# heat1q/libldpc

Hardware: AMD Instinct MI355X
Metric: decoded frames/s (n=1024 code, 50 BP iters, AWGN) (higher is better)
Workload: dtype f64

## Files before the change

include/ldpc_amd.h:

```cpp
#ifndef LDPC_AMD_H
#define LDPC_AMD_H

#include <stdbool.h>
#include <stdint.h>

#ifdef __cplusplus
extern "C" {
#endif

#if defined(__GNUC__)
#pragma GCC visibility push(default)
#endif

typedef struct
{
    bool earlyTerm;
    uint32_t iterations;
    const char *type;
} decoder_param;

typedef struct
{
    uint64_t seed;
    double xRange[3];
    const char *type;
} channel_param;

typedef struct
{
    uint32_t threads;
    uint64_t maxFrames;
    uint64_t fec;
    const char *resultFile;
} simulation_param;

typedef struct
{
    double *fer;
    double *ber;
    double *avg_iter;
    double *time;
    uint64_t *fec;
    uint64_t *frames;
} sim_results_t;

void ldpc_setup(const char *pcFile, const char *genFile, int *n, int *m, int *nct, int *mct);
void simulate(decoder_param decoderParams, channel_param channelParam, simulation_param simParam,
              sim_results_t *results, bool *stopFlag);
int calculate_rank(void);
void encode(uint8_t *infoWord, uint8_t *codeWord);
int decode(decoder_param decoderParams, double *llr, double *llrOut);
void syndrome(uint8_t *word, uint8_t *syndrome);

typedef struct ldpc_hip_ctx ldpc_hip_ctx;

enum
{
    LDPC_HIP_AWGN = 1,
    LDPC_HIP_BSC = 2,
    LDPC_HIP_BEC = 3
};

typedef struct
{
    uint32_t *iters;
    uint32_t *bit_errors;
    uint8_t *hard;
    double *llr_out;
    double *llr_in;
    uint8_t *codeword;
} ldpc_hip_out;

int ldpc_hip_device_count(void);
const char *ldpc_hip_last_error(void);

ldpc_hip_ctx *ldpc_hip_create(const char *pcFile, const char *genFile, int device);
void ldpc_hip_destroy(ldpc_hip_ctx *ctx);
void ldpc_hip_code_info(const ldpc_hip_ctx *ctx, int64_t info[10]);
const char *ldpc_hip_describe(ldpc_hip_ctx *ctx);
void ldpc_hip_set_bec_compat(ldpc_hip_ctx *ctx, int compat);
void ldpc_hip_set_fast_mode(ldpc_hip_ctx *ctx, int mode);

enum
{
    LDPC_HIP_NOISE_REFERENCE = 0,
    LDPC_HIP_NOISE_COUNTER = 1
};
int ldpc_hip_set_noise(ldpc_hip_ctx *ctx, int mode);
int ldpc_hip_philox(ldpc_hip_ctx *ctx, uint64_t seed, uint32_t tag, uint64_t frame, uint32_t first_block, uint64_t n_blocks,
                    uint32_t *out, void *hip_stream);

int ldpc_hip_set_min_sum_correction(ldpc_hip_ctx *ctx, double scale, double offset);

int ldpc_hip_decode_batch(ldpc_hip_ctx *ctx, decoder_param dec, uint64_t n, const double *llr_in,
                          const ldpc_hip_out *out, void *hip_stream);

int ldpc_hip_stream_begin(ldpc_hip_ctx *ctx, int channel, uint64_t seed, double x);
int ldpc_hip_stream_skip(ldpc_hip_ctx *ctx, uint64_t n, void *hip_stream);
int ldpc_hip_stream_decode(ldpc_hip_ctx *ctx, decoder_param dec, uint64_t n, const ldpc_hip_out *out,
                           void *hip_stream);
int ldpc_hip_batch_counters(ldpc_hip_ctx *ctx, const uint32_t *iters, const uint32_t *bit_errors, uint64_t n,
                            uint32_t max_iters, int early_term, int64_t *counters, void *hip_stream);
uint64_t ldpc_hip_stream_frame(const ldpc_hip_ctx *ctx);
uint64_t ldpc_hip_stream_raw_draws(const ldpc_hip_ctx *ctx);
int ldpc_hip_synchronize(ldpc_hip_ctx *ctx, void *hip_stream);

void ldpc_hip_set_profiling(ldpc_hip_ctx *ctx, int on);
float ldpc_hip_last_ms(ldpc_hip_ctx *ctx, int which);

int ldpc_hip_mt64(ldpc_hip_ctx *ctx, uint64_t seed, uint64_t first, uint64_t n, uint64_t *out, void *hip_stream);

int ldpc_hip_selftest_division(ldpc_hip_ctx *ctx, uint64_t n, uint64_t seed, uint64_t *mismatches);

int ldpc_hip_selftest_math(ldpc_hip_ctx *ctx, int fn, uint64_t n, const double *a, const double *b, double *out);

uint64_t ldpc_hip_selftest_chunk_table(uint64_t first_chunk, uint64_t chunks_per_request, uint64_t n_requests, uint64_t gap);
uint64_t ldpc_hip_selftest_shard_table(int world, int rank, uint32_t piece_chunks, uint64_t steps, uint64_t *launches);
uint64_t ldpc_hip_jump_tasks(const ldpc_hip_ctx *ctx);

int ldpc_hip_simulate(ldpc_hip_ctx *ctx, decoder_param dec, channel_param ch, simulation_param sim,
                      sim_results_t *results, uint64_t *totals, bool *stopFlag, int cli_output);

typedef struct ldpc_hip_comm ldpc_hip_comm;

int ldpc_hip_comm_unique_id(uint8_t id[128]);
ldpc_hip_comm *ldpc_hip_comm_create(int rank, int world, int device, const uint8_t id[128]);
ldpc_hip_comm *ldpc_hip_comm_create_shm(int rank, int world, const char *name);
ldpc_hip_comm *ldpc_hip_comm_create_echo(int rank, int world);
void ldpc_hip_comm_destroy(ldpc_hip_comm *comm);
int ldpc_hip_comm_allgather(ldpc_hip_comm *comm, const void *send, void *recv, uint64_t bytes);
void ldpc_hip_fused_plan_info(const ldpc_hip_ctx *ctx, int64_t info[8]);
int ldpc_hip_decode_stages(const ldpc_hip_ctx *ctx, decoder_param dec, int32_t stages[3]);
int ldpc_hip_selftest_layer_plan(ldpc_hip_ctx *ctx, int32_t *step_of_row);
int ldpc_hip_selftest_place(ldpc_hip_comm *comm, uint64_t nct, uint64_t pairs_before, uint64_t frame_pos, uint64_t cap,
                            uint64_t piece_pairs, uint64_t pairs_with_margin, uint64_t status, uint64_t out[5]);
void ldpc_hip_comm_stats(ldpc_hip_comm *comm, double out[4], int reset);
const char *ldpc_hip_comm_describe(ldpc_hip_comm *comm);

uint64_t ldpc_hip_shard_capacity(const ldpc_hip_ctx *ctx, uint64_t target_frames, int world);
int ldpc_hip_stream_decode_sharded(ldpc_hip_ctx *ctx, ldpc_hip_comm *comm, decoder_param dec, uint64_t target_frames,
                                   const ldpc_hip_out *out, uint64_t step[4], void *hip_stream);
int ldpc_hip_simulate_sharded(ldpc_hip_ctx *ctx, ldpc_hip_comm *comm, decoder_param dec, channel_param ch,
                              simulation_param sim, sim_results_t *results, uint64_t *totals, bool *stopFlag,
                              int cli_output);

#if defined(__GNUC__)
#pragma GCC visibility pop
#endif

#ifdef __cplusplus
}
#endif
#endif
```

libldpc_amd/binding.py:

```python
import ctypes as ct
import os

import numpy as np

PKG = os.path.dirname(os.path.abspath(__file__))
LIB_PATH = os.environ.get("LDPC_AMD_LIB") or os.path.join(PKG, "libldpc.so")

AWGN, BSC, BEC = 1, 2, 3
CHANNELS = {"AWGN": AWGN, "BSC": BSC, "BEC": BEC}


class decoder_param(ct.Structure):
    _fields_ = [("earlyTerm", ct.c_bool), ("iterations", ct.c_uint32), ("type", ct.c_char_p)]


class channel_param(ct.Structure):
    _fields_ = [("seed", ct.c_uint64), ("xRange", ct.c_double * 3), ("type", ct.c_char_p)]


class simulation_param(ct.Structure):
    _fields_ = [("threads", ct.c_uint32), ("maxFrames", ct.c_uint64), ("fec", ct.c_uint64),
                ("resultFile", ct.c_char_p)]


class sim_results_t(ct.Structure):
    _fields_ = [("fer", ct.POINTER(ct.c_double)), ("ber", ct.POINTER(ct.c_double)),
                ("avg_iter", ct.POINTER(ct.c_double)), ("time", ct.POINTER(ct.c_double)),
                ("fec", ct.POINTER(ct.c_uint64)), ("frames", ct.POINTER(ct.c_uint64))]


class ldpc_hip_out(ct.Structure):
    _fields_ = [("iters", ct.c_void_p), ("bit_errors", ct.c_void_p), ("hard", ct.c_void_p),
                ("llr_out", ct.c_void_p), ("llr_in", ct.c_void_p), ("codeword", ct.c_void_p)]


_lib = None


def load_library(path=LIB_PATH):
    global _lib
    if _lib is not None and path == LIB_PATH:
        return _lib
    if not os.path.exists(path):
        raise OSError(f"{path} is missing: build the HIP extension first (python -m libldpc_amd.build); "
                      "there is no CPU fallback")
    L = ct.CDLL(path)
    vp, u64, i32 = ct.c_void_p, ct.c_uint64, ct.c_int
    L.ldpc_hip_device_count.restype = i32
    L.ldpc_hip_last_error.restype = ct.c_char_p
    L.ldpc_hip_create.restype = vp
    L.ldpc_hip_create.argtypes = [ct.c_char_p, ct.c_char_p, i32]
    L.ldpc_hip_destroy.argtypes = [vp]
    L.ldpc_hip_code_info.argtypes = [vp, ct.POINTER(ct.c_int64)]
    L.ldpc_hip_set_bec_compat.argtypes = [vp, i32]
    L.ldpc_hip_set_fast_mode.argtypes = [vp, i32]
    L.ldpc_hip_set_noise.restype = i32
    L.ldpc_hip_set_noise.argtypes = [vp, i32]
    L.ldpc_hip_set_min_sum_correction.restype = i32
    L.ldpc_hip_set_min_sum_correction.argtypes = [vp, ct.c_double, ct.c_double]
    L.ldpc_hip_philox.restype = i32
    L.ldpc_hip_philox.argtypes = [vp, u64, ct.c_uint32, u64, ct.c_uint32, u64, vp, vp]
    L.ldpc_hip_decode_batch.restype = i32
    L.ldpc_hip_decode_batch.argtypes = [vp, decoder_param, u64, vp, ct.POINTER(ldpc_hip_out), vp]
    L.ldpc_hip_stream_begin.restype = i32
    L.ldpc_hip_stream_begin.argtypes = [vp, i32, u64, ct.c_double]
    L.ldpc_hip_stream_skip.restype = i32
    L.ldpc_hip_stream_skip.argtypes = [vp, u64, vp]
    L.ldpc_hip_stream_decode.restype = i32
    L.ldpc_hip_stream_decode.argtypes = [vp, decoder_param, u64, ct.POINTER(ldpc_hip_out), vp]
    L.ldpc_hip_stream_frame.restype = u64
    L.ldpc_hip_stream_frame.argtypes = [vp]
    L.ldpc_hip_stream_raw_draws.restype = u64
    L.ldpc_hip_stream_raw_draws.argtypes = [vp]
    L.ldpc_hip_synchronize.restype = i32
    L.ldpc_hip_synchronize.argtypes = [vp, vp]
    L.ldpc_hip_batch_counters.restype = i32
    L.ldpc_hip_batch_counters.argtypes = [vp, vp, vp, u64, ct.c_uint32, i32, vp, vp]
    L.ldpc_hip_selftest_division.restype = i32
    L.ldpc_hip_selftest_division.argtypes = [vp, u64, u64, vp]
    L.ldpc_hip_mt64.restype = i32
    L.ldpc_hip_mt64.argtypes = [vp, u64, u64, u64, vp, vp]
    L.ldpc_hip_set_profiling.argtypes = [vp, i32]
    L.ldpc_hip_last_ms.restype = ct.c_float
    L.ldpc_hip_last_ms.argtypes = [vp, i32]
    L.ldpc_hip_comm_unique_id.restype = i32
    L.ldpc_hip_comm_unique_id.argtypes = [vp]
    L.ldpc_hip_comm_create.restype = vp
    L.ldpc_hip_comm_create.argtypes = [i32, i32, i32, vp]
    L.ldpc_hip_comm_create_shm.restype = vp
    L.ldpc_hip_comm_create_shm.argtypes = [i32, i32, ct.c_char_p]
    L.ldpc_hip_comm_create_echo.restype = vp
    L.ldpc_hip_comm_create_echo.argtypes = [i32, i32]
    L.ldpc_hip_comm_destroy.argtypes = [vp]
    L.ldpc_hip_comm_allgather.restype = i32
    L.ldpc_hip_comm_allgather.argtypes = [vp, vp, vp, u64]
    L.ldpc_hip_fused_plan_info.restype = None
    L.ldpc_hip_fused_plan_info.argtypes = [vp, vp]
    L.ldpc_hip_decode_stages.restype = i32
    L.ldpc_hip_decode_stages.argtypes = [vp, decoder_param, vp]
    L.ldpc_hip_selftest_layer_plan.restype = i32
    L.ldpc_hip_selftest_layer_plan.argtypes = [vp, vp]
    L.ldpc_hip_selftest_place.restype = i32
    L.ldpc_hip_selftest_place.argtypes = [vp, u64, u64, u64, u64, u64, u64, u64, vp]
    L.ldpc_hip_comm_stats.restype = None
    L.ldpc_hip_comm_stats.argtypes = [vp, vp, i32]
    L.ldpc_hip_comm_describe.restype = ct.c_char_p
    L.ldpc_hip_comm_describe.argtypes = [vp]
    L.ldpc_hip_shard_capacity.restype = u64
    L.ldpc_hip_shard_capacity.argtypes = [vp, u64, i32]
    L.ldpc_hip_stream_decode_sharded.restype = i32
    L.ldpc_hip_stream_decode_sharded.argtypes = [vp, vp, decoder_param, u64, ct.POINTER(ldpc_hip_out), vp, vp]
    L.ldpc_hip_simulate_sharded.restype = i32
    L.ldpc_hip_simulate_sharded.argtypes = [vp, vp, decoder_param, channel_param, simulation_param, ct.POINTER(sim_results_t),
                                            vp, ct.POINTER(ct.c_bool), i32]
    L.ldpc_hip_selftest_math.restype = i32
    L.ldpc_hip_selftest_math.argtypes = [vp, i32, u64, vp, vp, vp]
    L.ldpc_hip_selftest_chunk_table.restype = u64
    L.ldpc_hip_selftest_chunk_table.argtypes = [u64, u64, u64, u64]
    L.ldpc_hip_selftest_shard_table.restype = u64
    L.ldpc_hip_selftest_shard_table.argtypes = [i32, i32, ct.c_uint32, u64, vp]
    L.ldpc_hip_jump_tasks.restype = u64
    L.ldpc_hip_jump_tasks.argtypes = [vp]
    L.ldpc_hip_simulate.restype = i32
    L.ldpc_hip_simulate.argtypes = [vp, decoder_param, channel_param, simulation_param, ct.POINTER(sim_results_t),
                                    vp, ct.POINTER(ct.c_bool), i32]
    if path == LIB_PATH:
        _lib = L
    return L


def _ptr(buf):
    if buf is None:
        return None
    if isinstance(buf, np.ndarray):
        assert buf.flags["C_CONTIGUOUS"]
        return buf.ctypes.data
    if hasattr(buf, "data_ptr"):
        assert buf.is_contiguous()
        return buf.data_ptr()
    raise TypeError(f"unsupported buffer type {type(buf)}")


def _dec(early_term, iterations, decoding):
    return decoder_param(bool(early_term), int(iterations), decoding.encode())


class Comm:

    def __init__(self, rank, world, device=0, unique_id=None, shm_name=None, echo=False, lib=LIB_PATH):
        self.lib = load_library(lib)
        self.rank, self.world = int(rank), int(world)
        if echo:
            self.handle = self.lib.ldpc_hip_comm_create_echo(self.rank, self.world)
        elif shm_name is not None:
            self.handle = self.lib.ldpc_hip_comm_create_shm(self.rank, self.world, shm_name.encode())
        else:
            buf = (ct.c_uint8 * 128).from_buffer_copy(bytes(unique_id))
            self.handle = self.lib.ldpc_hip_comm_create(self.rank, self.world, int(device), buf)
        if not self.handle:
            raise RuntimeError("communicator: " + self.lib.ldpc_hip_last_error().decode())

    @staticmethod
    def unique_id(lib=LIB_PATH):
        L = load_library(lib)
        buf = (ct.c_uint8 * 128)()
        if L.ldpc_hip_comm_unique_id(buf) != 0:
            raise RuntimeError("ldpc_hip_comm_unique_id: " + L.ldpc_hip_last_error().decode())
        return bytes(buf)

    def all_gather(self, values):
        v = np.ascontiguousarray(values, np.uint64)
        out = np.zeros((self.world, v.size), np.uint64)
        if self.lib.ldpc_hip_comm_allgather(self.handle, v.ctypes.data, out.ctypes.data, v.nbytes) != 0:
            raise RuntimeError("ldpc_hip_comm_allgather: " + self.lib.ldpc_hip_last_error().decode())
        return out

    def place(self, nct, pairs_before, frame_pos, cap, piece_pairs, pairs_with_margin, status=0):
        out = (ct.c_uint64 * 5)()
        if self.lib.ldpc_hip_selftest_place(self.handle, nct, pairs_before, frame_pos, cap, piece_pairs, pairs_with_margin, status, out) != 0:
            raise RuntimeError("ldpc_hip_selftest_place: " + self.lib.ldpc_hip_last_error().decode())
        return tuple(int(v) for v in out)

    def exchange_stats(self, reset=False):
        out = (ct.c_double * 4)()
        self.lib.ldpc_hip_comm_stats(self.handle, out, int(reset))
        return {"calls": int(out[0]), "min": out[1], "median": out[2], "max": out[3]}

    def describe(self):
        return self.lib.ldpc_hip_comm_describe(self.handle).decode()

    def close(self):
        if getattr(self, "handle", None):
            self.lib.ldpc_hip_comm_destroy(self.handle)
            self.handle = None

    __del__ = close


class HipDecoder:

    OUT_SPEC = {"iters": (np.uint32, False), "bit_errors": (np.uint32, False), "hard": (np.uint8, True),
                "llr_out": (np.float64, True), "llr_in": (np.float64, True), "codeword": (np.uint8, True)}

    def __init__(self, pc_file, gen_file="", device=0, lib=LIB_PATH):
        self.lib = load_library(lib)
        self.ctx = self.lib.ldpc_hip_create(pc_file.encode(), gen_file.encode(), device)
        if not self.ctx:
            raise RuntimeError("ldpc_hip_create: " + self.lib.ldpc_hip_last_error().decode())
        info = (ct.c_int64 * 10)()
        self.lib.ldpc_hip_code_info(self.ctx, info)
        (self.nc, self.mc, self.nnz, self.nct, self.mct, self.kct, self.kc, self.max_degree, lds,
         self.lds_bytes) = list(info)
        self.lds_resident = lds == 1
        self.residency = {0: "memory", 1: "lds", 2: "registers", 3: "registers"}[int(lds)]
        self.register_form = {2: "messages", 3: "totals"}.get(int(lds))

    def close(self):
        if getattr(self, "ctx", None):
            self.lib.ldpc_hip_destroy(self.ctx)
            self.ctx = None

    __del__ = close

    def _check(self, rc, what):
        if rc != 0:
            raise RuntimeError(f"{what}: " + self.lib.ldpc_hip_last_error().decode())

    def _outs(self, n, want, out):
        bufs = dict(out or {})
        for name in want:
            if name not in bufs:
                dt, per_bit = self.OUT_SPEC[name]
                bufs[name] = np.zeros((n, self.nc) if per_bit else (n,), dt)
        s = ldpc_hip_out(*[_ptr(bufs.get(k)) for k in ("iters", "bit_errors", "hard", "llr_out", "llr_in", "codeword")])
        return s, bufs

    def set_bec_compat(self, on):
        self.lib.ldpc_hip_set_bec_compat(self.ctx, int(on))

    def fused_plan(self):
        info = (ct.c_int64 * 8)()
        self.lib.ldpc_hip_fused_plan_info(self.ctx, info)
        return dict(zip(("ok", "n_slots", "vnb", "cnl", "small", "calls_stride", "has_shortened", "table_entries"), [int(v) for v in info]))

    STAGES = ("whole", "ratio-first", "ratio-separate", "list-chain", "llr-redo", "handover-first", "handover-resume")

    def decode_stages(self, early_term=True, iterations=50, decoding="BP"):
        stages = (ct.c_int32 * 3)()
        n = self.lib.ldpc_hip_decode_stages(self.ctx, _dec(early_term, iterations, decoding), stages)
        return [self.STAGES[stages[i]] for i in range(n)]

    def set_fast_mode(self, on):
        self.lib.ldpc_hip_set_fast_mode(self.ctx, int(on))

    NOISE_MODES = {"reference": 0, "counter": 1}

    def set_noise(self, mode):
        m = self.NOISE_MODES.get(mode, mode) if isinstance(mode, str) else int(mode)
        if isinstance(m, str):
            m = -1
        self._check(self.lib.ldpc_hip_set_noise(self.ctx, int(m)), f"ldpc_hip_set_noise({mode!r})")

    def set_min_sum_correction(self, scale=1.0, offset=0.0):
        self._check(self.lib.ldpc_hip_set_min_sum_correction(self.ctx, float(scale), float(offset)),
                    f"ldpc_hip_set_min_sum_correction({scale!r}, {offset!r})")

    def philox(self, seed, tag, frame, first_block, n_blocks):
        out = np.zeros((int(n_blocks), 4), np.uint32)
        self._check(self.lib.ldpc_hip_philox(self.ctx, int(seed), int(tag), int(frame), int(first_block), int(n_blocks),
                                             _ptr(out), None), "ldpc_hip_philox")
        return out

    def decode_batch(self, llr_in, early_term=True, iterations=50, decoding="BP",
                     want=("iters", "hard", "llr_out"), out=None, stream=None):
        n = int(llr_in.shape[0])
        s, bufs = self._outs(n, want, out)
        self._check(self.lib.ldpc_hip_decode_batch(self.ctx, _dec(early_term, iterations, decoding), n, _ptr(llr_in),
                                                   ct.byref(s), stream), "ldpc_hip_decode_batch")
        return bufs

    def stream_begin(self, channel, seed, x):
        ch = CHANNELS[channel] if isinstance(channel, str) else int(channel)
        self._check(self.lib.ldpc_hip_stream_begin(self.ctx, ch, int(seed), float(x)), "ldpc_hip_stream_begin")

    def stream_skip(self, n, stream=None):
        self._check(self.lib.ldpc_hip_stream_skip(self.ctx, int(n), stream), "ldpc_hip_stream_skip")

    def stream_decode(self, n, early_term=True, iterations=50, decoding="BP", want=("iters", "bit_errors"),
                      out=None, stream=None):
        s, bufs = self._outs(int(n), want, out)
        self._check(self.lib.ldpc_hip_stream_decode(self.ctx, _dec(early_term, iterations, decoding), int(n),
                                                    ct.byref(s), stream), "ldpc_hip_stream_decode")
        return bufs

    def shard_capacity(self, target_frames, world):
        return int(self.lib.ldpc_hip_shard_capacity(self.ctx, int(target_frames), int(world)))

    def stream_decode_sharded(self, comm, target_frames, early_term=True, iterations=50, decoding="BP",
                              want=("iters", "bit_errors"), out=None, stream=None):
        cap = self.shard_capacity(target_frames, comm.world)
        s, bufs = self._outs(cap, want, out)
        step = (ct.c_uint64 * 4)()
        self._check(self.lib.ldpc_hip_stream_decode_sharded(self.ctx, comm.handle, _dec(early_term, iterations, decoding),
                                                            int(target_frames), ct.byref(s), step, stream),
                    "ldpc_hip_stream_decode_sharded")
        return bufs, tuple(int(v) for v in step)

    @property
    def stream_frame(self):
        return self.lib.ldpc_hip_stream_frame(self.ctx)

    @property
    def stream_raw_draws(self):
        n = self.lib.ldpc_hip_stream_raw_draws(self.ctx)
        if n == 2**64 - 1:
            raise RuntimeError("ldpc_hip_stream_raw_draws: " + self.lib.ldpc_hip_last_error().decode())
        return n

    @property
    def jump_tasks(self):
        return self.lib.ldpc_hip_jump_tasks(self.ctx)

    def synchronize(self, stream=None):
        self._check(self.lib.ldpc_hip_synchronize(self.ctx, stream), "ldpc_hip_synchronize")

    def set_profiling(self, on=True):
        self.lib.ldpc_hip_set_profiling(self.ctx, int(on))

    def last_ms(self, which=0):
        return float(self.lib.ldpc_hip_last_ms(self.ctx, which))

    def batch_counters(self, iters_ptr, bit_errors_ptr, n, max_iters, early_term, counters_ptr, stream=None):
        self._check(self.lib.ldpc_hip_batch_counters(self.ctx, iters_ptr, bit_errors_ptr, int(n), int(max_iters),
                                                     int(bool(early_term)), counters_ptr, stream), "ldpc_hip_batch_counters")

    def selftest_division(self, n, seed=1):
        bad = ct.c_uint64(0)
        self._check(self.lib.ldpc_hip_selftest_division(self.ctx, int(n), int(seed), ct.byref(bad)),
                    "ldpc_hip_selftest_division")
        return bad.value

    MATH_FNS = ("exp", "log", "boxplus", "ratio_div", "ratio_rho", "ratio_lambda", "e_combine", "exp_clamped", "boxplus_exp",
                "boxplus_log", "cn_ratio3", "cn_ratio4", "cn_ratio5", "cn_ratio6", "cn_ratio8", "cn_llr4", "cn_llr6", "cn_ratio3s", "cn_ratio4s", "cn_ratio6s")

    def selftest_math(self, fn, a, b=None):
        a = np.ascontiguousarray(a, np.float64)
        out = np.empty_like(a)
        n = a.shape[0]
        bb = None if b is None else np.ascontiguousarray(b, np.float64)
        self._check(self.lib.ldpc_hip_selftest_math(self.ctx, self.MATH_FNS.index(fn), n, _ptr(a), _ptr(bb), _ptr(out)),
                    "ldpc_hip_selftest_math")
        return out

    def mt64(self, seed, first, n):
        out = np.zeros(int(n), np.uint64)
        self._check(self.lib.ldpc_hip_mt64(self.ctx, int(seed), int(first), int(n), _ptr(out), None), "ldpc_hip_mt64")
        return out

    def simulate(self, channel, x_range, seed=0, early_term=True, iterations=50, decoding="BP",
                 max_frames=10**10, fec=50, result_file="", cli_output=False, comm=None):
        n_max = max(1, int(np.ceil((x_range[1] - x_range[0]) / x_range[2])) + 2)
        arrs = {k: np.zeros(n_max, np.float64) for k in ("fer", "ber", "avg_iter", "time")}
        arrs["fec"] = np.zeros(n_max, np.uint64)
        arrs["frames"] = np.zeros(n_max, np.uint64)
        res = sim_results_t(*[arrs[k].ctypes.data_as(ct.POINTER(ct.c_double if arrs[k].dtype == np.float64
                                                                 else ct.c_uint64))
                              for k in ("fer", "ber", "avg_iter", "time", "fec", "frames")])
        totals = np.zeros(4 * n_max, np.uint64)
        stop = ct.c_bool(False)
        ch = channel_param(int(seed), (ct.c_double * 3)(*x_range), channel.encode())
        sp = simulation_param(1, int(max_frames), int(fec), result_file.encode())
        if comm is not None:
            nx = self.lib.ldpc_hip_simulate_sharded(self.ctx, comm.handle, _dec(early_term, iterations, decoding), ch, sp,
                                                    ct.byref(res), totals.ctypes.data, ct.byref(stop), int(cli_output))
        else:
            nx = self.lib.ldpc_hip_simulate(self.ctx, _dec(early_term, iterations, decoding), ch, sp, ct.byref(res),
                                            totals.ctypes.data, ct.byref(stop), int(cli_output))
        if nx < 0:
            raise RuntimeError("ldpc_hip_simulate: " + self.lib.ldpc_hip_last_error().decode())
        out = {k: v[:nx] for k, v in arrs.items()}
        out["totals"] = totals[:4 * nx].reshape(nx, 4)
        return out
```

libldpc_amd/csrc/api.cpp:

```cpp
#include "../../include/ldpc_amd.h"

#include <hip/hip_runtime.h>

#include <cstdio>
#include <cstdlib>
#include <cstring>
#include <iostream>
#include <memory>
#include <string>
#include <vector>

#include "engine.hpp"
#include "shard_place.hpp"
#include "sim.hpp"

using namespace ldpc_amd;

struct ldpc_hip_comm
{
    std::unique_ptr<Comm> comm;
    std::string description;
};

struct ldpc_hip_ctx
// ... 292 lines not shown
    return guarded([&] { ctx->eng->decode_llr(to_params(dec), n, llr_in, to_out(out), hip_stream); });
}

int ldpc_hip_stream_begin(ldpc_hip_ctx *ctx, int channel, uint64_t seed, double x)
{
    return guarded([&] { ctx->eng->stream_begin(channel, seed, x, true); });
}

int ldpc_hip_stream_skip(ldpc_hip_ctx *ctx, uint64_t n, void *hip_stream)
{
    return guarded([&] { ctx->eng->stream_skip(n, hip_stream); });
}

int ldpc_hip_stream_decode(ldpc_hip_ctx *ctx, decoder_param dec, uint64_t n, const ldpc_hip_out *out,
                           void *hip_stream)
{
    return guarded([&] { ctx->eng->stream_decode(to_params(dec), n, to_out(out), hip_stream); });
}

uint64_t ldpc_hip_stream_frame(const ldpc_hip_ctx *ctx) { return ctx->eng->stream_frame(); }
uint64_t ldpc_hip_stream_raw_draws(const ldpc_hip_ctx *ctx)
{
    uint64_t n = ~0ull;
    guarded([&] { n = ctx->eng->stream_raw_draws(); });
    return n;
}

int ldpc_hip_synchronize(ldpc_hip_ctx *ctx, void *hip_stream)
{
    return guarded([&] { ctx->eng->synchronize(hip_stream); });
}

void ldpc_hip_set_profiling(ldpc_hip_ctx *ctx, int on)
{
    guarded([&] { ctx->eng->set_profiling(on != 0); });
}

float ldpc_hip_last_ms(ldpc_hip_ctx *ctx, int which) { return ctx->eng->last_ms(which); }

int ldpc_hip_mt64(ldpc_hip_ctx *ctx, uint64_t seed, uint64_t first, uint64_t n, uint64_t *out, void *hip_stream)
{
    return guarded([&] {
        if (ldpc_hip_device_count() <= ctx->eng->device())
            throw std::runtime_error("no usable HIP device (MI355X required)");
        if (hipSetDevice(ctx->eng->device()) != hipSuccess)
            throw std::runtime_error("hipSetDevice failed");
        hipStream_t s = static_cast<hipStream_t>(hip_stream);
        ctx->aux.reset(seed);
        uint64_t done = 0;
        while (done < n)
        {
            const uint64_t k = std::min<uint64_t>(n - done, 64ull << 20);
            const uint64_t *raw = ctx->aux.generate(first + done, k, hip_stream);
            hipPointerAttribute_t attr;
            bool dev = hipPointerGetAttributes(&attr, out) == hipSuccess && attr.type == hipMemoryTypeDevice;
            if (!dev)
                (void)hipGetLastError();
            if (hipMemcpyAsync(out + done, raw, 8 * k, dev ? hipMemcpyDeviceToDevice : hipMemcpyDeviceToHost, s) !=
                    hipSuccess ||
                hipStreamSynchronize(s) != hipSuccess)
                throw std::runtime_error("copy of mt19937_64 words failed");
            done += k;
        }
    });
}

int ldpc_hip_batch_counters(ldpc_hip_ctx *ctx, const uint32_t *iters, const uint32_t *bit_errors, uint64_t n,
                            uint32_t max_iters, int early_term, int64_t *counters, void *hip_stream)
{
    return guarded([&] {
        if (ldpc_hip_device_count() <= ctx->eng->device())
            throw std::runtime_error("no usable HIP device (MI355X required)");
        if (hipSetDevice(ctx->eng->device()) != hipSuccess)
            throw std::runtime_error("hipSetDevice failed");
        if (!iters || !bit_errors || !counters)
            throw std::runtime_error("ldpc_hip_batch_counters: null pointer");
        if (ldpc_amd::launch_batch_counters(iters, bit_errors, n, max_iters, early_term,
                                            reinterpret_cast<long long *>(counters), hip_stream) != hipSuccess)
            throw std::runtime_error("ldpc_hip_batch_counters: launch failed");
    });
}

int ldpc_hip_selftest_division(ldpc_hip_ctx *ctx, uint64_t n, uint64_t seed, uint64_t *mismatches)
{
    return guarded([&] {
        if (ldpc_hip_device_count() <= ctx->eng->device())
            throw std::runtime_error("no usable HIP device (MI355X required)");
        if (hipSetDevice(ctx->eng->device()) != hipSuccess)
            throw std::runtime_error("hipSetDevice failed");
        unsigned long long *d = nullptr, h = 0;
        if (hipMalloc(&d, sizeof h) != hipSuccess || hipMemset(d, 0, sizeof h) != hipSuccess)
            throw std::runtime_error("hipMalloc failed");
        const int rc = ldpc_amd::launch_division_selftest(n, seed, d, nullptr);
        const bool ok = rc == hipSuccess && hipMemcpy(&h, d, sizeof h, hipMemcpyDeviceToHost) == hipSuccess;
        (void)hipFree(d);
        if (!ok)
            throw std::runtime_error("division self-test failed to run");
        *mismatches = h;
    });
}

int ldpc_hip_selftest_math(ldpc_hip_ctx *ctx, int fn, uint64_t n, const double *a, const double *b, double *out)
{
    return guarded([&] {
        if (ldpc_hip_device_count() <= ctx->eng->device())
            throw std::runtime_error("no usable HIP device (MI355X required)");
        if (hipSetDevice(ctx->eng->device()) != hipSuccess)
            throw std::runtime_error("hipSetDevice failed");
        const int w = ldpc_amd::math_selftest_width(fn);
        if (w == 0 || !a || !out)
            throw std::runtime_error("ldpc_hip_selftest_math: unknown function or null buffer");
        const size_t bytes = 8 * n * static_cast<size_t>(w);
        double *da = nullptr, *db = nullptr, *dout = nullptr;
        bool ok = hipMalloc(&da, bytes) == hipSuccess && hipMalloc(&dout, bytes) == hipSuccess &&
                  hipMemcpy(da, a, bytes, hipMemcpyHostToDevice) == hipSuccess;
        if (ok && b)
            ok = hipMalloc(&db, bytes) == hipSuccess && hipMemcpy(db, b, bytes, hipMemcpyHostToDevice) == hipSuccess;
        ok = ok && ldpc_amd::launch_math_selftest(fn, n, da, db ? db : da, dout, nullptr) == hipSuccess &&
             hipMemcpy(out, dout, bytes, hipMemcpyDeviceToHost) == hipSuccess;
        (void)hipFree(da), (void)hipFree(db), (void)hipFree(dout);
        if (!ok)
            throw std::runtime_error("ldpc_hip_selftest_math failed to run");
    });
}

namespace
{
struct SymbolicTable
{
    std::vector<int64_t> row;
    uint64_t tasks = 0, launches = 0;
    explicit SymbolicTable(size_t n) : row(n, -1) {}
    bool apply(const std::vector<StateOp> &ops)
    {
        for (const StateOp &op : ops)
            switch (op.kind)
            {
            case StateOp::kUpload0: row[op.dst] = 0; break;
            case StateOp::kCopy:
                if (row[op.src] < 0)
                    return false;
                row[op.dst] = row[op.src];
                break;
            case StateOp::kJump:
            {
                std::vector<int64_t> src(op.n);
                for (uint32_t i = 0; i < op.n; ++i)
                {
                    src[i] = row[(op.src + i) % op.mod];
                    if (src[i] < 0)
                        return false;
                    for (uint32_t k = 0; k < op.n; ++k)
                        if (k != i && (op.dst + k) % op.mod == (op.src + i) % op.mod)
                            return false;
                }
                for (uint32_t i = 0; i < op.n; ++i)
                    row[(op.dst + i) % op.mod] = src[i] + static_cast<int64_t>(op.stride);
                tasks += op.n, ++launches;
                break;
            }
            }
        return true;
    }
};
}

uint64_t ldpc_hip_selftest_chunk_table(uint64_t first_chunk, uint64_t chunks_per_request, uint64_t n_requests, uint64_t gap)
{
    StateRing t;
    SymbolicTable sym(StateRing::kTotalRows);
    uint64_t c = first_chunk;
    std::vector<StateOp> ops;
    try
    {
        for (uint64_t i = 0; i < n_requests; ++i, c += chunks_per_request + gap)
        {
            ops.clear();
            t.ensure(c, c + chunks_per_request, ops);
            if (!sym.apply(ops))
                return ~0ull;
            for (uint64_t k = c; k < c + chunks_per_request; ++k)
                if (sym.row[k % StateRing::kRows] != static_cast<int64_t>(k))
                    return ~0ull;
            if (gap == 0 && i % 3 != 2)
            {
                ops.clear();
                t.extend_to(c + 3 * chunks_per_request + 2, ops);
                if (!sym.apply(ops))
                    return ~0ull;
                for (uint64_t k = c; k < c + chunks_per_request; ++k)
                    if (sym.row[k % StateRing::kRows] != static_cast<int64_t>(k))
                        return ~0ull;
            }
        }
    }
    catch (const std::exception &e)
    {
        g_err = e.what();
        return ~0ull;
    }
    return sym.tasks;
}

uint64_t ldpc_hip_selftest_shard_table(int world, int rank, uint32_t piece_chunks, uint64_t steps, uint64_t *launches)
{
    StridedTable t;
    SymbolicTable sym(StridedTable::kTotalRows);
    std::vector<StateOp> ops;
    const uint32_t n = piece_chunks + 1;
    const uint64_t stride = static_cast<uint64_t>(world) * piece_chunks;
    uint64_t tasks_after_first = 0, launches_after_first = 0;
    try
    {
        for (uint64_t s = 0; s < steps; ++s)
        {
            const uint64_t first = s * stride + static_cast<uint64_t>(rank) * piece_chunks;
            ops.clear();
            const uint32_t base = t.position(first, n, stride, ops);
            const uint64_t t0 = sym.tasks, l0 = sym.launches;
            if (!sym.apply(ops))
                return ~0ull;
            for (uint32_t i = 0; i < n; ++i)
                if (sym.row[base + i] != static_cast<int64_t>(first + i))
                    return ~0ull;
            if (s % 3 != 2)
            {
                ops.clear();
                t.look_ahead(ops);
                if (!sym.apply(ops))
                    return ~0ull;
                for (uint32_t i = 0; i < n; ++i)
                    if (sym.row[base + i] != static_cast<int64_t>(first + i))
                        return ~0ull;
            }
            if (s > 0)
                tasks_after_first += sym.tasks - t0, launches_after_first += sym.launches - l0;
        }
    }
    catch (const std::exception &e)
    {
        g_err = e.what();
        return ~0ull;
    }
    if (launches)
        *launches = launches_after_first;
    return tasks_after_first;
}

int ldpc_hip_comm_unique_id(uint8_t id[128])
{
    return guarded([&] { rccl_unique_id(id); });
}

ldpc_hip_comm *ldpc_hip_comm_create(int rank, int world, int device, const uint8_t id[128])
{
    ldpc_hip_comm *c = nullptr;
    if (guarded([&] {
            auto p = std::make_unique<ldpc_hip_comm>();
            p->comm = make_rccl_comm(rank, world, device, id);
            c = p.release();
        }) != 0)
        return nullptr;
    return c;
}

ldpc_hip_comm *ldpc_hip_comm_create_shm(int rank, int world, const char *name)
{
    ldpc_hip_comm *c = nullptr;
    if (guarded([&] {
            auto p = std::make_unique<ldpc_hip_comm>();
            p->comm = make_shm_comm(rank, world, name ? name : "/ldpc_amd");
            c = p.release();
        }) != 0)
        return nullptr;
    return c;
}

ldpc_hip_comm *ldpc_hip_comm_create_echo(int rank, int world)
{
    ldpc_hip_comm *c = nullptr;
    if (guarded([&] {
            auto p = std::make_unique<ldpc_hip_comm>();
            p->comm = make_echo_comm(rank, world);
            c = p.release();
        }) != 0)
        return nullptr;
    return c;
}

void ldpc_hip_comm_destroy(ldpc_hip_comm *comm) { delete comm; }

int ldpc_hip_comm_allgather(ldpc_hip_comm *comm, const void *send, void *recv, uint64_t bytes)
{
    return guarded([&] { comm->comm->all_gather(send, recv, bytes); });
}

void ldpc_hip_fused_plan_info(const ldpc_hip_ctx *ctx, int64_t info[8])
{
    const FusedPlan &f = ctx->eng->fused_plan();
    info[0] = f.ok ? 1 : 0, info[1] = f.n_slots, info[2] = f.vnb, info[3] = f.cnl, info[4] = f.wide_exclusive ? 1 : 0;
    info[5] = f.calls_stride, info[6] = f.has_shortened ? 1 : 0, info[7] = static_cast<int64_t>(f.vn_slot.size());
}

int ldpc_hip_decode_stages(const ldpc_hip_ctx *ctx, decoder_param dec, int32_t stages[3])
{
    const StageSeq seq = ctx->eng->stages(to_params(dec));
    for (int i = 0; i < seq.n; ++i)
        stages[i] = static_cast<int32_t>(seq.s[i]);
    return seq.n;
}

int ldpc_hip_selftest_layer_plan(ldpc_hip_ctx *ctx, int32_t *step_of_row)
{
    int n = -1;
    if (guarded([&] {
            const LayerPlan L = build_layer_plan(ctx->eng->code(), ctx->eng->plan());
            if (!L.ok)
                throw std::runtime_error("the layered schedule does not take this code");
            for (size_t i = 0; i < L.step_of_row.size(); ++i)
                step_of_row[i] = L.step_of_row[i];
            n = static_cast<int>(L.steps.size());
        }) != 0)
        return -1;
    return n;
}

int ldpc_hip_selftest_place(ldpc_hip_comm *comm, uint64_t nct, uint64_t pairs_before, uint64_t frame_pos, uint64_t cap,
                            uint64_t piece_pairs, uint64_t pairs_with_margin, uint64_t status, uint64_t out[5])
{
    return guarded([&] {
        const int R = comm->comm->world(), r = comm->comm->rank();
        const uint64_t send[3] = {piece_pairs, pairs_with_margin, status};
        std::vector<uint64_t> all(3 * static_cast<size_t>(R));
        comm->comm->all_gather(send, all.data(), sizeof send);
        const ShardPlacement pl = place_pieces(all.data(), R, r, pairs_before, frame_pos, nct, cap, status ? "status word set by the caller" : "");
        out[0] = pl.first, out[1] = pl.n, out[2] = pl.step_frames, out[3] = pl.pair_start, out[4] = pl.pairs_after;
    });
}

void ldpc_hip_comm_stats(ldpc_hip_comm *comm, double out[4], int reset) { comm->comm->exchange_stats(out, reset != 0); }

const char *ldpc_hip_comm_describe(ldpc_hip_comm *comm)
{
    comm->description = comm->comm->describe();
    return comm->description.c_str();
}

uint64_t ldpc_hip_shard_capacity(const ldpc_hip_ctx *ctx, uint64_t target_frames, int world) { return ctx->eng->shard_capacity(target_frames, world < 1 ? 1 : world); }
uint64_t ldpc_hip_jump_tasks(const ldpc_hip_ctx *ctx) { return ctx->eng->noise_jump_tasks(); }

int ldpc_hip_stream_decode_sharded(ldpc_hip_ctx *ctx, ldpc_hip_comm *comm, decoder_param dec, uint64_t target_frames,
                                   const ldpc_hip_out *out, uint64_t step[4], void *hip_stream)
{
    return guarded([&] {
        const Engine::ShardStep st = ctx->eng->stream_decode_sharded(*comm->comm, to_params(dec), target_frames, to_out(out), hip_stream);
        if (step)
            step[0] = st.step_first, step[1] = st.step_frames, step[2] = st.first, step[3] = st.n;
    });
}

int ldpc_hip_simulate_sharded(ldpc_hip_ctx *ctx, ldpc_hip_comm *comm, decoder_param dec, channel_param ch,
                              simulation_param sim, sim_results_t *results, uint64_t *totals, bool *stopFlag, int cli_output)
{
    int n = -1;
    int rc = guarded([&] {
        SimRequest rq;
        rq.dec = to_params(dec);
        rq.channel = channel_from(ch.type);
        if (!rq.channel)
            throw std::runtime_error("No channel selected.");
        rq.seed = ch.seed;
        for (int i = 0; i < 3; ++i)
            rq.x_range[i] = ch.xRange[i];
        rq.max_frames = sim.maxFrames;
        rq.min_fec = sim.fec;
        rq.result_file = sim.resultFile ? sim.resultFile : "";
        rq.cli_output = cli_output != 0;
        n = run_simulation(*ctx->eng, rq, results, totals, stopFlag, comm ? comm->comm.get() : nullptr);
    });
    return rc == 0 ? n : -1;
}

int ldpc_hip_simulate(ldpc_hip_ctx *ctx, decoder_param dec, channel_param ch, simulation_param sim,
                      sim_results_t *results, uint64_t *totals, bool *stopFlag, int cli_output)
{
    int n = -1;
    int rc = guarded([&] {
        SimRequest rq;
        rq.dec = to_params(dec);
        rq.channel = channel_from(ch.type);
        if (!rq.channel)
            throw std::runtime_error("No channel selected.");
        rq.seed = ch.seed;
        for (int i = 0; i < 3; ++i)
            rq.x_range[i] = ch.xRange[i];
        rq.max_frames = sim.maxFrames;
        rq.min_fec = sim.fec;
        rq.result_file = sim.resultFile ? sim.resultFile : "";
        rq.cli_output = cli_output != 0;
        n = run_simulation(*ctx->eng, rq, results, totals, stopFlag);
    });
    return rc == 0 ? n : -1;
}

}
```

libldpc_amd/csrc/engine.cpp:

```cpp
#include "engine.hpp"
#include "shard_place.hpp"

#include <hip/hip_runtime.h>

#include <algorithm>
#include <chrono>
#include <cmath>
#include <cstdio>
#include <cstdlib>
#include <cstring>
#include <mutex>
#include <stdexcept>

namespace ldpc_amd
{

std::string hip_error_string(int err) { return hipGetErrorString(static_cast<hipError_t>(err)); }

namespace
{
void check(hipError_t e, const char *what)
{
    if (e != hipSuccess)
        throw std::runtime_error(std::string("HIP error in ") + what + ": " + hipGetErrorString(e));
// ... 304 lines not shown
}

uint64_t *MtDevice::ensure_strided(uint64_t first, uint32_t n, uint64_t stride, void *stream)
{
    uint64_t *table = static_cast<uint64_t *>(strided_buf_.reserve(sizeof(uint64_t) * kMtWords * StridedTable::kTotalRows));
    std::vector<StateOp> ops;
    const uint32_t base = strided_.position(first, n, stride, ops);
    for (uint32_t k = 0; k < StridedTable::kSlots; ++k)
        if (strided_pending_[k] && (k == base / StridedTable::kMaxRows || !ops.empty()))
        {
            check(hipStreamWaitEvent(static_cast<hipStream_t>(stream), static_cast<hipEvent_t>(ev_strided_[k]), 0), "wait look-ahead");
            strided_pending_[k] = false;
        }
    apply(ops, table, stream);
    if (!ops.empty())
    {
        if (!ev_main_)
        {
            hipEvent_t e;
            check(hipEventCreateWithFlags(&e, hipEventDisableTiming), "hipEventCreate");
            ev_main_ = e;
        }
        check(hipEventRecord(static_cast<hipEvent_t>(ev_main_), static_cast<hipStream_t>(stream)), "event");
        main_dirty_ = true;
    }
    return table + static_cast<size_t>(base) * kMtWords;
}

void MtDevice::prefetch_strided()
{
    if (!strided_buf_.get())
        return;
    std::vector<StateOp> ops;
    strided_.look_ahead(ops);
    if (ops.empty())
        return;
    if (!jump_stream_)
    {
        hipStream_t js;
        check(hipStreamCreateWithFlags(&js, hipStreamNonBlocking), "hipStreamCreate");
        jump_stream_ = js;
    }
    hipStream_t js = static_cast<hipStream_t>(jump_stream_);
    if (main_dirty_)
    {
        check(hipStreamWaitEvent(js, static_cast<hipEvent_t>(ev_main_), 0), "wait table");
        main_dirty_ = false;
    }
    for (const StateOp &op : ops)
    {
        apply({op}, static_cast<uint64_t *>(strided_buf_.get()), js);
        const uint32_t k = op.dst / StridedTable::kMaxRows;
        if (!ev_strided_[k])
        {
            hipEvent_t e;
            check(hipEventCreateWithFlags(&e, hipEventDisableTiming), "hipEventCreate");
            ev_strided_[k] = e;
        }
        check(hipEventRecord(static_cast<hipEvent_t>(ev_strided_[k]), js), "event");
        strided_pending_[k] = true;
    }
}

const uint64_t *MtStream::generate(uint64_t first, uint64_t count, void *stream, int buffer)
{
    hipStream_t s = static_cast<hipStream_t>(stream);
    if (count == 0)
        count = 1;
    const uint64_t cw = st.chunk_words();
    const uint64_t c_lo = first / cw;
    const uint64_t c_hi = (first + count + cw - 1) / cw;
    if (c_hi - c_lo > StateRing::kWindow)
        throw std::runtime_error("mt19937_64 stream request exceeds the chunk-state window");
    const uint32_t row = st.ensure_ring(c_lo, c_hi, stream);
    const uint32_t n = static_cast<uint32_t>(c_hi - c_lo);
    uint64_t *raw = static_cast<uint64_t *>(raw_[buffer & 1].reserve(sizeof(uint64_t) * cw * n));
    uint32_t words = static_cast<uint32_t>(cw);
    if (n == 1)
    {
        const uint64_t need = (first + count - c_lo * cw + kMtWords - 1) / kMtWords * kMtWords;
        words = static_cast<uint32_t>(std::min<uint64_t>(need, cw));
    }
    check(launch_mt_generate(st.ring(), MtDevice::ring_rows(), row, raw, n, words, words, n == 1 ? 1 : pack_, s), "mt_generate");
    if (first == last_end_ && n > 1)
        st.prefetch_ring(c_hi + 2 * (static_cast<uint64_t>(n) + 1));
    last_end_ = first + count;
    return raw + (first - c_lo * cw);
}

Engine::Engine(const std::string &pc_file, const std::string &gen_file, int device) : device_(device)
{
    code_ = std::make_unique<LdpcCode>(pc_file, gen_file);
    if (code_->min_cn_degree() < 2)
        throw std::runtime_error("check nodes of degree < 2 are not supported (undefined in the reference decoder)");
    plan_ = build_plan(*code_);
    const size_t nc = plan_.nc, nnz = plan_.nnz;
    if (plan_.lds_ok)
    {
        residency_ = Residency::kLds;
        fused_plan_ = build_fused_plan(*code_, plan_);
        const size_t cu_lds = 160 * 1024, with_llr = plan_.lds_bytes, without = plan_.lds_bytes - 8 * nc;
        if (cu_lds / without > cu_lds / with_llr && plan_.vn_work_stride <= 8 && !plan_.has_isolated_vn && plan_.nc <= plan_.nnz &&
            !plan_.vn_packed.empty())
            lds_llr_mode_ = 2;
        return;
    }
    for (int r = 0; r < code_->H.rows && !shared6_; ++r)
        shared6_ = code_->H.rptr[r + 1] - code_->H.rptr[r] == 6;
    struct Tile { int nt, kc, maxd; };
    for (Tile t : {Tile{1024, 4, 6}, Tile{1024, 8, 4}, Tile{1024, 2, 8}, Tile{512, 8, 6}, Tile{512, 16, 4}, Tile{512, 4, 8}})
    {
        reg_plan_ = build_reg_plan(*code_, plan_, t.nt, t.kc, t.maxd, t.nt == 512 ? 80 * 1024 : 160 * 1024);
        if (reg_plan_.ok)
            break;
    }
    if (reg_plan_.ok)
    {
        reg2_plan_ = build_reg2_plan(*code_, plan_, 1024, 4, 6, 4, 4);
        residency_ = reg2_plan_.ok ? Residency::kRegTotals : Residency::kRegMessages;
        noise_.set_pack(4), noise_.st.set_default_chunk_blocks(2240);
    }
    else if (plan_.hbm_ok)
    {
        residency_ = Residency::kMemory;
        const uint64_t per_frame = 8ull * nnz + 8ull * nc + nnz;
        const uint64_t frames_per_cu = std::clamp<uint64_t>((224ull << 20) / (256 * per_frame), 1, 8);
        mem_occ_lds_ = frames_per_cu >= 8 ? 0 : static_cast<uint32_t>((160 * 1024) / (frames_per_cu + 1) + 1024) & ~15u;
    }
}

Engine::~Engine()
{
    for (void *p : owned_)
        (void)hipFree(p);
    for (auto &q : prof_pending_)
        for (void *e : q)
            prof_free_.push_back(e);
    for (void *e : prof_free_)
        if (e)
            (void)hipEventDestroy(static_cast<hipEvent_t>(e));
    for (int i = 0; i < 2; ++i)
    {
        if (ev_pairs_ready_[i])
            (void)hipEventDestroy(static_cast<hipEvent_t>(ev_pairs_ready_[i]));
        if (ev_pairs_free_[i])
            (void)hipEventDestroy(static_cast<hipEvent_t>(ev_pairs_free_[i]));
    }
    if (rng_stream_)
        (void)hipStreamDestroy(static_cast<hipStream_t>(rng_stream_));
    if (pin_in_ev_)
        (void)hipEventDestroy(static_cast<hipEvent_t>(pin_in_ev_));
}

void Engine::set_profiling(bool on) { profiling_ = on; }

void Engine::bind_device()
{
    if (!device_checked_)
    {
        int n = 0;
        hipError_t e = hipGetDeviceCount(&n);
        if (e != hipSuccess || n <= device_)
        {
            (void)hipGetLastError();
            throw std::runtime_error("no usable HIP device (MI355X required): " + std::string(hipGetErrorString(e)));
        }
        device_checked_ = true;
    }
    check(hipSetDevice(device_), "hipSetDevice");
}

void Engine::prof_mark(int which, void *stream)
{
    if (!profiling_)
        return;
    auto &q = prof_pending_[which];
    if (q.size() >= 8192 && q.size() % 2 == 0)
    {
        prof_free_.insert(prof_free_.end(), q.begin(), q.end());
        q.clear();
    }
    void *e;
    if (prof_free_.empty())
    {
        hipEvent_t ev;
        check(hipEventCreate(&ev), "hipEventCreate");
        e = ev;
    }
    else
    {
        e = prof_free_.back();
        prof_free_.pop_back();
    }
    check(hipEventRecord(static_cast<hipEvent_t>(e), static_cast<hipStream_t>(stream)), "event");
    q.push_back(e);
}

float Engine::last_ms(int which)
{
    if (which == 2 || which == 3)
    {
        const int k = which - 2;
        const float v = host_n_[k] ? static_cast<float>(host_ms_[k] / static_cast<double>(host_n_[k])) : 0.f;
        host_ms_[k] = 0, host_n_[k] = 0;
        return v;
    }
    bind_device();
    auto &q = prof_pending_[which ? 1 : 0];
    double sum = 0;
    size_t spans = 0;
    for (size_t i = 0; i + 1 < q.size(); i += 2)
    {
        hipEvent_t a = static_cast<hipEvent_t>(q[i]), b = static_cast<hipEvent_t>(q[i + 1]);
        float ms = 0.f;
        if (hipEventSynchronize(b) == hipSuccess && hipEventElapsedTime(&ms, a, b) == hipSuccess)
            sum += ms, ++spans;
        else
            (void)hipGetLastError();
    }
    for (void *e : q)
        prof_free_.push_back(e);
    q.clear();
    return spans ? static_cast<float>(sum / spans) : 0.f;
}

void Engine::upload_plan()
{
    bind_device();
    if (dev_.cn_blocks)
        return;
    auto up = [&](const void *src, size_t bytes) -> void * {
        void *d = nullptr;
        check(hipMalloc(&d, std::max<size_t>(bytes, 16)), "hipMalloc plan");
        owned_.push_back(d);
        if (bytes)
            check(hipMemcpy(d, src, bytes, hipMemcpyHostToDevice), "upload plan");
        return d;
    };
    const Plan &p = plan_;
    dev_.nc = p.nc, dev_.mc = p.mc, dev_.nnz = p.nnz, dev_.nct = p.nct;
    dev_.n_bitpos = p.n_bitpos;
    dev_.n_cn_blocks = static_cast<int>(p.cn_blocks.size());
    dev_.n_vn_blocks = static_cast<int>(p.vn_blocks.size());
    dev_.cn_work_stride = p.cn_work_stride, dev_.vn_work_stride = p.vn_work_stride;
#define UP(field, vec) dev_.field = static_cast<decltype(dev_.field)>(up(vec.data(), vec.size() * sizeof(vec[0])))
    UP(cn_blocks, p.cn_blocks);
    UP(vn_blocks, p.vn_blocks);
    UP(vn_slot, p.vn_slot);
    UP(cn_work, p.cn_work);
    UP(cn_work_desc, p.cn_work_desc);
    UP(vn_work_desc, p.vn_work_desc);
    if (!p.vn_packed.empty())
        UP(vn_packed, p.vn_packed);
    else
        dev_.vn_packed = nullptr;
    dev_.cn_desc_stride = p.cn_desc_stride;
    UP(vn_work, p.vn_work);
    UP(col_rank, p.col_rank);
    UP(rank_col, p.rank_col);
    UP(tx_rank, p.tx_rank);
    UP(rank_kind, p.rank_kind);
    UP(rank_slot0, p.rank_slot0);
    UP(bit_pos, code_->bit_pos);
#undef UP
    if (reg_plan_.ok)
    {
        const RegPlan &r = reg_plan_;
        dev_reg_.nt = r.nt, dev_reg_.kc = r.kc, dev_reg_.maxd = r.maxd, dev_reg_.rounds = r.rounds;
        dev_reg_.mb_doubles = r.mb_doubles;
        dev_reg_.cn_edge = static_cast<const uint32_t *>(up(r.cn_edge.data(), r.cn_edge.size() * 4));
        dev_reg_.cn_deg = static_cast<const uint8_t *>(up(r.cn_deg.data(), r.cn_deg.size()));
        dev_reg_.cn_cnt = static_cast<const uint8_t *>(up(r.cn_cnt.data(), r.cn_cnt.size()));
        dev_reg_.vn_blocks = static_cast<const RegVnBlock *>(up(r.vn_blocks.data(), r.vn_blocks.size() * sizeof(RegVnBlock)));
        dev_reg_.round_first = static_cast<const uint32_t *>(up(r.round_first.data(), r.round_first.size() * 4));
    }
    if (reg2_plan_.ok)
    {
        const Reg2Plan &r = reg2_plan_;
        dev_reg2_.nt = r.nt, dev_reg2_.kc = r.kc, dev_reg2_.maxd = r.maxd, dev_reg2_.nv0 = r.nv0, dev_reg2_.nv1 = r.nv1;
        dev_reg2_.neutral = r.neutral, dev_reg2_.lds_entries = r.lds_entries;
        dev_reg2_.uniform_cn = r.uniform_cn ? 1 : 0;
        dev_reg2_.uniform_vn = r.uniform_vn ? 1 : 0;
        std::memcpy(dev_reg2_.vn_affine, r.vn_affine, sizeof r.vn_affine);
        dev_reg2_.edge_w = static_cast<const uint32_t *>(up(r.edge_w.data(), r.edge_w.size() * 4));
        dev_reg2_.cn_deg = static_cast<const uint8_t *>(up(r.cn_deg.data(), r.cn_deg.size()));
        dev_reg2_.vn_blocks = static_cast<const Reg2VnBlock *>(up(r.vn_blocks.data(), r.vn_blocks.size() * sizeof(Reg2VnBlock)));
        dev_reg2_.vn_rank = static_cast<const uint32_t *>(up(r.vn_rank.data(), r.vn_rank.size() * 4));
    }
    if (fused_plan_.ok)
    {
        const FusedPlan &f = fused_plan_;
        dev_fused_.n_slots = f.n_slots, dev_fused_.vnb = f.vnb, dev_fused_.cnl = f.cnl, dev_fused_.calls_stride = f.calls_stride;
        dev_fused_.has_shortened = f.has_shortened ? 1 : 0;
        dev_fused_.need_lambda = f.need_lambda ? 1 : 0;
        dev_fused_.wide_exclusive = f.wide_exclusive ? 1 : 0;
        std::memcpy(dev_fused_.vn_prog, f.vn_prog, sizeof f.vn_prog);
        dev_fused_.lds_bytes = static_cast<uint32_t>(std::max<size_t>(8 * static_cast<size_t>(f.n_slots), 16 * (static_cast<size_t>(std::max(p.nc, p.nct)) + 2)) + 15) & ~15u;
        dev_fused_.leaf_calls = static_cast<const FusedCall *>(up(f.leaf_calls.data(), f.leaf_calls.size() * sizeof(FusedCall)));
        dev_fused_.calls = static_cast<const FusedCall *>(up(f.calls.data(), f.calls.size() * sizeof(FusedCall)));
        dev_fused_.vn_desc = static_cast<const uint32_t *>(up(f.vn_desc.data(), f.vn_desc.size() * 4));
        dev_fused_.vn_slot = static_cast<const uint32_t *>(up(f.vn_slot.data(), f.vn_slot.size() * 4));
        dev_fused_.lane_tab = static_cast<const uint32_t *>(up(f.lane_tab.data(), f.lane_tab.size() * 4));
        dev_fused_.ho_map = static_cast<const uint32_t *>(up(f.ho_map.data(), f.ho_map.size() * 4));
    }
    if (code_->has_G())
    {
        std::vector<uint32_t> cp(code_->G.cptr.begin(), code_->G.cptr.end()), cr(code_->G.crow.begin(), code_->G.crow.end());
        g_col_ptr_ = static_cast<const uint32_t *>(up(cp.data(), cp.size() * 4));
        g_col_row_ = static_cast<const uint32_t *>(up(cr.data(), cr.size() * 4));
        const int kc = code_->kc(), words = (kc + 63) / 64;
        if (kc > 0 && words <= 4 && code_->G.rows <= kc)
        {
            std::vector<uint64_t> mask(static_cast<size_t>(p.nc) * words, 0);
            for (int j = 0; j < code_->G.cols && j < p.nc; ++j)
                for (int q = code_->G.cptr[j]; q < code_->G.cptr[j + 1]; ++q)
                {
                    const int r = code_->G.crow[q];
                    mask[static_cast<size_t>(j) * words + r / 64] ^= 1ull << (r % 64);
                }
            g_mask_ = static_cast<const uint64_t *>(up(mask.data(), mask.size() * 8));
        }
    }
    dev_.lds_bytes = static_cast<uint32_t>(p.lds_bytes);
}

void Engine::synchronize(void *stream)
{
    bind_device();
    check(hipStreamSynchronize(static_cast<hipStream_t>(stream)), "sync");
}

uint64_t Engine::max_sub_batch() const
{
    const uint64_t kMaxSlabs = std::max<uint64_t>(4, 476ull * 2240 / noise_.st.chunk_blocks());
    const uint64_t pairs_per_frame = std::max<uint64_t>(1, (static_cast<uint64_t>(plan_.nct) + 1) / 2 + 1);
    const uint64_t by_noise = std::max<uint64_t>(1, (kMaxSlabs - 2) * noise_.st.chunk_trials() * 3 / 4 / pairs_per_frame);
    if (residency_ == Residency::kLds || register_resident())
        return std::min<uint64_t>(1u << 17, by_noise);
    const uint64_t per_frame = 8ull * plan_.nnz + 8ull * plan_.nc + plan_.nnz;
    return std::max<uint64_t>(1, std::min<uint64_t>({1u << 17, (8ull << 30) / per_frame, by_noise}));
}

void Engine::ensure_layer_plan()
{
    if (layer_plan_.ok || !layer_plan_.steps.empty())
        return;
    layer_plan_ = build_layer_plan(*code_, plan_);
    if (!layer_plan_.ok)
        return;
    const size_t nc = plan_.nc;
    std::vector<uint32_t> steps;
    for (const LayerStep &l : layer_plan_.steps)
        steps.push_back(l.off), steps.push_back(static_cast<uint32_t>(l.count) | static_cast<uint32_t>(l.degree) << 16);
    std::vector<uint32_t> vn4(layer_plan_.steps.size() * 4 * kWaveSize, 0);
    for (size_t si = 0; si < layer_plan_.steps.size(); ++si)
        for (int j = 0; j < layer_plan_.steps[si].degree; ++j)
            for (int l = 0; l < kWaveSize; ++l)
                vn4[(si * 4 + j / 2) * kWaveSize + l] |=
                    static_cast<uint32_t>(layer_plan_.vn[layer_plan_.steps[si].off + static_cast<size_t>(j) * kWaveSize + l]) << (16 * (j & 1));
    void *d_steps = nullptr, *d_vn = nullptr;
    check(hipMalloc(&d_steps, steps.size() * 4), "hipMalloc layer plan");
    owned_.push_back(d_steps);
    check(hipMalloc(&d_vn, vn4.size() * 4), "hipMalloc layer plan");
    owned_.push_back(d_vn);
    check(hipMemcpy(d_steps, steps.data(), steps.size() * 4, hipMemcpyHostToDevice), "upload layer plan");
    check(hipMemcpy(d_vn, vn4.data(), vn4.size() * 4, hipMemcpyHostToDevice), "upload layer plan");
    dev_layer_.steps = static_cast<const uint32_t *>(d_steps);
    dev_layer_.vn4 = static_cast<const uint32_t *>(d_vn);
    dev_layer_.n_steps = static_cast<uint32_t>(layer_plan_.steps.size());
    dev_layer_.slots = layer_plan_.slots;
    const size_t tot_bytes = 4 * ((nc + 3) & ~size_t(3));
    dev_layer_.region_bytes = static_cast<uint32_t>((std::max(8 * nc, tot_bytes + 4 * size_t(layer_plan_.slots)) + 15) & ~size_t(15));
    dev_layer_.region_bytes_half = static_cast<uint32_t>((std::max(8 * nc, tot_bytes + 2 * size_t(layer_plan_.slots)) + 15) & ~size_t(15));
}

void Engine::finish_batch(OutStage &st, const BatchOut &out, uint64_t n, const uint8_t *codeword, int noise_buffer, void *stream)
{
    hipStream_t s = static_cast<hipStream_t>(stream);
    const size_t nc = plan_.nc;
    prof_mark(0, s);
    if (noise_buffer >= 0)
        noise_raw_release(noise_buffer, stream);
    if (out.codeword)
    {
        if (codeword)
            check(hipMemcpyAsync(out.codeword, codeword, n * nc,
                                 is_device_ptr(out.codeword) ? hipMemcpyDeviceToDevice : hipMemcpyDeviceToHost, s),
                  "codeword out");
        else if (is_device_ptr(out.codeword))
            check(hipMemsetAsync(out.codeword, 0, n * nc, s), "codeword out");
        else
            std::memset(out.codeword, 0, n * nc);
    }
    st.flush(s, &pin_out_);
}

static void set_stage_lists(DecodeArgs &a, Stage st, uint32_t *in, uint32_t *out, uint64_t n)
{
    const bool reads = stage_reads_list(st), writes = stage_writes_list(st);
    a.redo_count_in = reads ? in : nullptr, a.redo_list_in = reads ? in + 1 : nullptr;
    a.redo_iter_in = st == Stage::kHandoverResume ? in + 1 + n : nullptr;
    a.redo_count = writes ? out : nullptr, a.redo_list = writes ? out + 1 : nullptr;
    a.redo_iter = st == Stage::kHandoverFirst ? out + 1 + n : nullptr;
}

void Engine::run_decode(DecodeArgs &a, const DecParams &p, const BatchOut &out, uint64_t n, void *stream)
{
    hipStream_t s = static_cast<hipStream_t>(stream);
    const size_t nc = plan_.nc, nnz = plan_.nnz;
    OutStage st;
    a.plan = dev_;
    a.iterations = p.iterations;
    a.early_term = p.early_term;
    a.n_frames = n;
    a.iters = st.route(out.iters, stage_iters_, 4 * n);
    a.bit_errors = st.route(out.bit_errors, stage_be_, 4 * n);
    a.hard = st.route(out.hard, stage_hard_, n * nc);
    a.llr_out = st.route(out.llr_out, stage_llr_out_, 8 * n * nc);
    a.llr_in_dump = st.route(out.llr_in, stage_llr_in_, 8 * n * nc);
    a.ms_correct = p.min_sum && !(ms_scale == 1.0 && ms_offset == 0.0);
    a.ms_scale = ms_scale, a.ms_offset = ms_offset;
    prof_mark(0, s);
    const bool fast = fast_mode && !p.min_sum;
    const auto launch = [&](Stage stage) {
        if (fast && fast_mode == 1)
        {
            if (!fast_mode_supported(dev_, plan_.max_cn_degree) || plan_.has_isolated_vn)
                throw std::runtime_error("fast mode: this code is outside what the binary32 kernel takes (check nodes up to degree 8, "
                                         "nc <= 8192, LDS-resident, no isolated variable node)");
            a.ws_hb = static_cast<uint8_t *>(ws_hb_.reserve(n * nc));
            check(launch_decode_fast(a, plan_.max_cn_degree, s), "decode (fast mode, binary32)");
            return;
        }
        if (fast)
        {
            ensure_layer_plan();
            const bool half = fast_mode == 3;
            if (!layer_plan_.ok || plan_.has_isolated_vn || (half ? dev_layer_.region_bytes_half : dev_layer_.region_bytes) > 160 * 1024)
                throw std::runtime_error("layered mode: this code is outside what the layered kernel takes (check nodes of degree 2..8, at "
                                         "most 65535 columns, totals and messages of one frame within 160 KB of LDS, no isolated variable node)");
            check(launch_decode_layered(a, dev_layer_, half, s), half ? "decode (layered, binary16 messages)" : "decode (layered, binary32 messages)");
            return;
        }
        switch (residency_)
        {
        case Residency::kLds:
            if (fused_plan_.ok && stage == Stage::kRatioFirst)
                check(launch_decode_fused(a, dev_fused_, stage, s), "decode (fused form)");
            else if (fused_plan_.ok && stage == Stage::kHandoverFirst)
                check(launch_decode_fused(a, dev_fused_, stage, s), "decode (fused form, hand-over)");
            else if (fused_plan_.ok && stage == Stage::kWhole && p.min_sum && !p.early_term && p.iterations > 0)
                check(launch_decode_fused(a, dev_fused_, stage, s), "decode (min-sum, fused plan)");
            else
                check(launch_decode_lds(a, stage, p.min_sum, plan_.max_cn_degree, lds_llr_mode_, s), "decode (LDS-resident)");
            break;
        case Residency::kRegTotals:
        case Residency::kRegMessages:
            a.ws_llr = static_cast<double *>(ws_llr_.reserve(8 * n * nc));
            a.ws_hb = static_cast<uint8_t *>(ws_hb_.reserve(n * nc));
            if (residency_ == Residency::kRegTotals)
            {
                a.ws_scr = static_cast<double *>(ws_scr_.reserve(8 * n * static_cast<uint64_t>(reg2_plan_.nv0 + reg2_plan_.nv1) * reg2_plan_.nt));
                check(launch_decode_reg2(a, dev_reg2_, stage, p.min_sum, s), "decode (register-resident, totals form)");
            }
            else
                check(launch_decode_reg(a, dev_reg_, stage, p.min_sum, s), "decode (register-resident)");
            break;
        case Residency::kMemory:
            a.ws_msg = static_cast<double *>(ws_msg_.reserve(8 * n * nnz));
            a.ws_llr = static_cast<double *>(ws_llr_.reserve(8 * n * nc));
            a.ws_hb = static_cast<uint8_t *>(ws_hb_.reserve(n * nnz));
            a.ws_scr = plan_.max_cn_degree > kMaxCnDegree ? static_cast<double *>(ws_scr_.reserve(16 * n * nnz)) : nullptr;
            check(launch_decode_mem(a, stage, p.min_sum, plan_.max_cn_degree, mem_occ_lds_, s), "decode (memory-resident)");
            break;
        case Residency::kNone:
            throw std::runtime_error("code not supported by any decoder instantiation");
        }
    };
    const StageSeq seq = stages(p);
    uint32_t *list_in = nullptr;
    for (int i = 0; i < seq.n; ++i)
    {
        const Stage stage = seq.s[i];
        uint32_t *list_out = nullptr;
        if (stage_writes_list(stage))
        {
            list_out = static_cast<uint32_t *>(i == 0 ? redo_.reserve(4 * (2 * n + 1)) : redo2_.reserve(4 * (n + 1)));
            check(hipMemsetAsync(list_out, 0, 4, s), "redo count");
        }
        set_stage_lists(a, stage, list_in, list_out, n);
        if (stage == Stage::kHandoverFirst)
            a.ws_handover = static_cast<double *>(ws_msg_.reserve(8 * n * nnz));
        if (stage == Stage::kHandoverResume)
            a.handover_llr = fused_plan_.ok ? 1 : 0;
#ifdef LDPC_AMD_PHASE_TRACE
        uint64_t *tr = nullptr;
        const char *trace_file = i == 0 && stage != Stage::kWhole ? std::getenv("LDPC_AMD_PHASE_TRACE") : nullptr;
        if (trace_file)
        {
            check(hipMalloc(&tr, 2048 * 32 * 8), "trace");
            check(hipMemset(tr, 0, 2048 * 32 * 8), "trace");
            a.phase_trace = tr;
        }
#endif
        launch(stage);
#ifdef LDPC_AMD_PHASE_TRACE
        if (tr)
        {
            std::vector<uint64_t> h(2048 * 32);
            check(hipDeviceSynchronize(), "sync");
            check(hipMemcpy(h.data(), tr, 2048 * 32 * 8, hipMemcpyDeviceToHost), "trace");
            if (FILE *f = std::fopen(trace_file, "wb"))
            {
                std::fwrite(h.data(), 8, h.size(), f);
                std::fclose(f);
            }
            (void)hipFree(tr);
            a.phase_trace = nullptr;
        }
#endif
        const size_t pinned = st.pinned_bytes();
        if (i == 0 && stage == Stage::kRatioFirst && n <= 16 && pinned && pinned <= OutStage::kPinnedLimit && a.mode == kModeLlr &&
            st.flush(s, &pin_out_, list_out) == 0)
        {
            st.items.clear();
            break;
        }
        list_in = list_out;
    }
    set_stage_lists(a, Stage::kWhole, nullptr, nullptr, n);
    a.ws_handover = nullptr, a.handover_llr = 0;
    finish_batch(st, out, n, a.codeword, a.mode == kModeAwgn ? a.pairs_buffer : -1, stream);
}

void Engine::run_bsc(DecodeArgs &a, const DecParams &p, const BatchOut &out, uint64_t n, uint64_t raw_first, void *stream)
{
    a.mode = kModeBsc;
    int raw_buffer = 0;
    a.raw = noise_raw_async(raw_first, n * static_cast<uint64_t>(plan_.nct), stream, raw_buffer);
    a.eps = x_, a.delta = delta_;
    a.shorten_llr = delta_;
    run_decode(a, p, out, n, stream);
    noise_raw_release(raw_buffer, stream);
}

void Engine::run_bec(const DecParams &p, const BatchOut &out, uint64_t n, const uint8_t *codeword, uint64_t raw_first, void *stream,
                     const uint64_t *ctr_frame0)
{
    hipStream_t s = static_cast<hipStream_t>(stream);
    const size_t nc = plan_.nc;
    const uint64_t nct = static_cast<uint64_t>(plan_.nct);
    const size_t state = static_cast<size_t>((plan_.nnz + 15) / 16) * 16 + 2 * ((nc + 15) / 16) * 16;
    OutStage st;
    BecArgs a{};
    a.ws = state > 160 * 1024 ? static_cast<uint8_t *>(ws_msg_.reserve(n * state)) : nullptr;
    a.plan = dev_;
    a.iterations = p.iterations;
    a.early_term = p.early_term;
    a.deg1_compat = bec_deg1_compat;
    a.n_frames = n;
    int raw_buffer = -1;
    if (ctr_frame0)
    {
        a.counter = 1;
        a.ctr_key[0] = static_cast<uint32_t>(ctr_seed_), a.ctr_key[1] = static_cast<uint32_t>(ctr_seed_ >> 32);
        a.ctr_frame0 = *ctr_frame0;
    }
    else
        a.raw = noise_raw_async(raw_first, n * nct, stream, raw_buffer);
    a.eps = x_;
    a.codeword = codeword;
    a.iters = st.route(out.iters, stage_iters_, 4 * n);
    a.bit_errors = st.route(out.bit_errors, stage_be_, 4 * n);
    a.hard = st.route(out.hard, stage_hard_, n * nc);
    a.llr_out = st.route(out.llr_out, stage_llr_out_, 8 * n * nc);
    a.llr_in_dump = st.route(out.llr_in, stage_llr_in_, 8 * n * nc);
    prof_mark(0, s);
    check(launch_bec(a, s), "bec");
    finish_batch(st, out, n, codeword, raw_buffer, stream);
}

uint8_t *Engine::encoder_prologue(uint64_t frames_kept, bool sharded, void *stream)
{
    const int kc = code_->kc();
    if (kc <= 0 || code_->G.rows > kc)
        throw std::runtime_error("generator matrix does not match the code (rows > nc - mc)");
    if (sharded && static_cast<size_t>((kc + 63) / 64) * 8 > Comm::kMaxBytes)
        throw std::runtime_error("sharded encoding: more than 2048 information bits per frame do not fit the exchange");
    hipStream_t s = static_cast<hipStream_t>(stream);
    const size_t nc = plan_.nc;
    uint8_t *prev = static_cast<uint8_t *>(cw_run_.reserve(nc));
    if (!cw_run_valid_)
    {
        check(hipMemsetAsync(prev, 0, nc, s), "codeword reset");
        cw_run_valid_ = true;
    }
    check(hipMemcpyAsync(cw_before_.reserve(nc), prev, nc, hipMemcpyDeviceToDevice, s), "codeword snapshot");
    last_enc_n_ = frames_kept;
    return prev;
}

const uint8_t *Engine::encode_frames(uint64_t n, bool want_codewords, void *stream)
{
    if (!code_->has_G() || n == 0)
        return nullptr;
    hipStream_t s = static_cast<hipStream_t>(stream);
// ... 710 lines not shown
```

libldpc_amd/csrc/kernels.hpp:

```cpp
#pragma once

#include <cstddef>
#include <cstdint>

#include "plan.hpp"

namespace ldpc_amd
{

struct DevPlan
{
    int nc, mc, nnz, nct;
    int n_bitpos;
    int n_cn_blocks, n_vn_blocks;
    int cn_work_stride, vn_work_stride;
    const CnBlock *cn_blocks;
    const VnBlock *vn_blocks;
    const uint32_t *vn_slot;
    const uint32_t *cn_work;
    const uint32_t *vn_work;
    const CnBlock *cn_work_desc;
    int cn_desc_stride;
    const uint32_t *vn_work_desc;
    const uint32_t *vn_packed;
    const uint32_t *col_rank;
    const uint32_t *rank_col;
    const uint32_t *tx_rank;
    const uint8_t *rank_kind;
    const uint32_t *rank_slot0;
    const int *bit_pos;
    uint32_t lds_bytes;
};

enum ChannelMode : int
{
    kModeLlr = 0,
    kModeAwgn = 1,
    kModeBsc = 2,
    kModeAwgnCtr = 3,
    kModeBscCtr = 4,
};

struct DecodeArgs
{
    DevPlan plan;
    uint32_t iterations;
    int early_term;
    int mode;
    uint64_t n_frames;
    const double *llr_in;
    const uint64_t *pairs;
    const uint64_t *slab_cum;
    uint64_t slab_words;
    uint32_t n_slabs;
    float slab_pairs_inv;
    uint64_t pair_origin;
    uint64_t normal_base;
    int pairs_buffer;
    double sigma, sigma2;
    double inv_sigma2;
    double shorten_llr;
    const uint64_t *raw;
    double eps, delta;
    const uint8_t *codeword;
    uint32_t *iters;
    uint32_t *bit_errors;
    uint8_t *hard;
    double *llr_out;
    double *llr_in_dump;
    double *ws_msg;
    double *ws_llr;
    uint8_t *ws_hb;
    double *ws_scr;
    uint32_t *redo_list;
    uint32_t *redo_count;
    int ratio_separate;
    const uint32_t *redo_list_in;
    const uint32_t *redo_count_in;
    uint32_t *redo_iter;
    const uint32_t *redo_iter_in;
    double *ws_handover;
    int handover_llr;
    uint64_t *phase_trace;
    uint32_t ctr_key[2];
    uint64_t ctr_frame0;
    int ms_correct;
    double ms_scale, ms_offset;
};
static_assert(sizeof(DecodeArgs) == 512 && offsetof(DecodeArgs, plan) == 0 && offsetof(DecodeArgs, iterations) == 168 &&
                  offsetof(DecodeArgs, redo_list) == 392 && offsetof(DecodeArgs, ratio_separate) == 408 &&
                  offsetof(DecodeArgs, redo_list_in) == 416 && offsetof(DecodeArgs, ms_correct) == 488 &&
                  offsetof(DecodeArgs, ms_offset) == 504,
              "DecodeArgs: layout changed");

enum class Stage : int
{
    kWhole,
    kRatioFirst,
    kRatioSeparate,
    kListChain,
    kLlrRedo,
    kHandoverFirst,
    kHandoverResume,
};
constexpr bool stage_writes_list(Stage s) { return s == Stage::kRatioFirst || s == Stage::kRatioSeparate || s == Stage::kHandoverFirst; }
constexpr bool stage_reads_list(Stage s)
{
    return s == Stage::kRatioSeparate || s == Stage::kListChain || s == Stage::kLlrRedo || s == Stage::kHandoverResume;
}
constexpr bool stage_is_handover(Stage s) { return s == Stage::kHandoverFirst || s == Stage::kHandoverResume; }
inline bool stage_args_ok(const DecodeArgs &a, Stage s)
{
    if (stage_writes_list(s) && (!a.redo_list || !a.redo_count))
        return false;
    if (stage_reads_list(s) && (!a.redo_list_in || !a.redo_count_in))
        return false;
    if (stage_is_handover(s) && (!a.ws_handover || !(s == Stage::kHandoverFirst ? a.redo_iter : a.redo_iter_in)))
        return false;
    return s == Stage::kWhole || (a.iterations > 0 && stage_is_handover(s) == !a.early_term);
}

struct DevRegPlan
{
    int nt, kc, maxd, rounds;
    uint32_t mb_doubles;
    const uint32_t *cn_edge;
    const uint8_t *cn_deg;
    const uint8_t *cn_cnt;
    const RegVnBlock *vn_blocks;
    const uint32_t *round_first;
};

struct DevReg2Plan
{
    int nt, kc, maxd, nv0, nv1;
    uint32_t neutral, lds_entries;
    int uniform_cn;
    int uniform_vn;
    uint32_t vn_affine[2][6];
    const uint32_t *edge_w;
    const uint8_t *cn_deg;
    const Reg2VnBlock *vn_blocks;
    const uint32_t *vn_rank;
};

struct DevFusedPlan
{
    int n_slots, vnb, cnl, calls_stride;
    int has_shortened;
    int need_lambda;
    int wide_exclusive;
    uint32_t vn_prog[kDecodeWaves];
    uint32_t lds_bytes;
    const FusedCall *leaf_calls;
    const FusedCall *calls;
    const uint32_t *vn_desc;
    const uint32_t *vn_slot;
    const uint32_t *lane_tab;
    const uint32_t *ho_map;
};
int launch_decode_fused(const DecodeArgs &a, const DevFusedPlan &f, Stage stage, void *stream);

struct BecArgs
{
    DevPlan plan;
    uint32_t iterations;
    int early_term;
    int deg1_compat;
    uint64_t n_frames;
    const uint64_t *raw;
    double eps;
    const uint8_t *symbols;
    const uint8_t *codeword;
    uint32_t *iters;
    uint32_t *bit_errors;
    uint8_t *hard;
    double *llr_out;
    double *llr_in_dump;
    uint8_t *ws;
    int counter;
    uint32_t ctr_key[2];
    uint64_t ctr_frame0;
};

bool bec_sliced_fits(const DevPlan &p);
int launch_bec_sliced(const BecArgs &a, void *stream);

int launch_decode_lds(const DecodeArgs &a, Stage stage, bool min_sum, int max_cn_degree, int llr_mode, void *stream);
int launch_decode_mem(const DecodeArgs &a, Stage stage, bool min_sum, int max_cn_degree, uint32_t occupancy_lds, void *stream);
int launch_decode_reg(const DecodeArgs &a, const DevRegPlan &r, Stage stage, bool min_sum, void *stream);
int launch_decode_reg2(const DecodeArgs &a, const DevReg2Plan &r, Stage stage, bool min_sum, void *stream);
bool fast_mode_supported(const DevPlan &p, int max_cn_degree);
int launch_decode_fast(const DecodeArgs &a, int max_cn_degree, void *stream);
struct DevLayerPlan
{
    const uint32_t *steps;
    const uint32_t *vn4;
    uint32_t n_steps, slots;
    uint32_t region_bytes, region_bytes_half;
};
int launch_decode_layered(const DecodeArgs &a, const DevLayerPlan &L, bool half_messages, void *stream);
int launch_bec(const BecArgs &a, void *stream);

constexpr int kMtN = 312;
constexpr uint32_t kBlockTrials = kMtN / 2;
int launch_mt_generate(const uint64_t *ring, uint32_t ring_rows, uint32_t first_row, uint64_t *out, uint32_t n_chunks,
                       uint32_t chunk_words, uint32_t last_words, int pack, void *stream);
int launch_mt_jump(uint64_t *ring, uint32_t ring_rows, uint32_t src_first, uint32_t dst_first, const uint64_t *poly,
                   uint32_t n_tasks, int groups, void *stream);
constexpr uint32_t kJumpPolyWords = 320;

struct NormalsArgs
{
    const uint64_t *ring;
    uint32_t ring_rows, first_row;
    uint32_t n_chunks;
    uint32_t blocks;
    uint32_t last_blocks;
    int pack;
    uint64_t *raw;
    uint64_t *lookback;
    uint64_t *slabs;
    uint64_t slab_words;
    uint32_t *counts;
    int write_normals;
    uint32_t locate_chunk, locate_rank;
    uint64_t *locate_out;
};
constexpr uint32_t kSlabBlock = 2048;
inline uint64_t normals_lookback_words(uint32_t n_chunks, uint32_t blocks)
{
    return static_cast<uint64_t>(n_chunks) * ((static_cast<uint64_t>(kBlockTrials) * blocks + kSlabBlock - 1) / kSlabBlock + 1);
}
int launch_mt_normals(const NormalsArgs &a, void *stream);

struct NormalsResult
{
    uint64_t total;
    uint64_t piece;
    uint64_t next_k;
    uint32_t next_slab;
    uint32_t enough;
};
int launch_normals_finish(const uint32_t *counts, uint32_t n, uint32_t n_piece, uint32_t n_full, uint64_t need, uint64_t target,
                          uint64_t *cum, NormalsResult *result, void *stream);

struct EncodeArgs
{
    int nc, kc, words;
    const uint32_t *g_col_ptr;
    const uint32_t *g_col_row;
    int g_cols;
    const uint64_t *info_raw;
    uint64_t *prefix;
    const uint8_t *cw_prev;
    uint8_t *codeword;
    uint8_t *cw_last;
    uint64_t n_frames;
    const uint64_t *base;
    const uint64_t *g_mask;
};
int launch_encode(const EncodeArgs &a, void *stream);
int launch_encode_prefix(const EncodeArgs &a, void *stream);
int launch_encode_codewords(const EncodeArgs &a, void *stream, bool only_last);

int launch_philox(uint64_t seed, uint32_t tag, uint64_t frame, uint32_t first_block, uint64_t n_blocks, uint32_t *out, void *stream);
int launch_encode_info_counter(uint64_t seed, uint64_t frame0, uint64_t n, int kc, int words, uint64_t *prefix, void *stream);

int launch_batch_counters(const uint32_t *iters, const uint32_t *bit_errors, uint64_t n, uint32_t max_iters, int early_term,
                          long long *counters, void *stream);

int launch_division_selftest(uint64_t n, uint64_t seed, unsigned long long *mismatches, void *stream);

enum MathFn : int
{
    kMathExp = 0,
    kMathLog,
    kMathBoxplus,
    kMathRatioDiv,
    kMathRatioRho,
    kMathRatioLambda,
    kMathECombine,
    kMathExpClamped,
    kMathBoxplusExp,
    kMathBoxplusLog,
    kMathCnRatio3,
    kMathCnRatio4,
    kMathCnRatio5,
    kMathCnRatio6,
    kMathCnRatio8,
    kMathCnLlr4,
    kMathCnLlr6,
    kMathCnRatio3s,
    kMathCnRatio4s,
    kMathCnRatio6s,
    kMathCount
};
int math_selftest_width(int fn);
int launch_math_selftest(int fn, uint64_t n, const double *a, const double *b, double *out, void *stream);

}
```

libldpc_amd/csrc/kernels_fused.hip:

```cpp
#include <hip/hip_runtime.h>

#include <algorithm>

#include "device_cn.hpp"
#include "device_math.hpp"
#include "device_philox.hpp"
#include "fused_rule.h"
#include "kernels.hpp"

#ifndef LDPC_AMD_DECODE_PRIO
#define LDPC_AMD_DECODE_PRIO 3
#endif
#ifndef LDPC_AMD_FUSED_WAVES
#define LDPC_AMD_FUSED_WAVES 6
#endif

namespace ldpc_amd
{

namespace
{

constexpr int kThreads = kDecodeWaves * kWaveSize;

__device__ __forceinline__ uint32_t hi_word(double x) { return static_cast<uint32_t>(dm_bits(x) >> 32); }
__device__ __forceinline__ double with_sign(double mag, uint32_t sign_hi)
{
    return dm_from_bits(dm_bits(mag) | (static_cast<uint64_t>(sign_hi) << 32));
}
__device__ __forceinline__ double *at(char *msg, uint32_t byte_off) { return reinterpret_cast<double *>(msg + byte_off); }

struct Track
{
    uint32_t hmax, hmin, pmax;
};
__device__ __forceinline__ void track(Track &t, double a)
{
    t.hmax = max(t.hmax, hi_word(a));
    t.hmin = min(t.hmin, hi_word(a));
}
__device__ __forceinline__ void track2(Track &t, double a, double b)
{
    t.hmax = max(max(t.hmax, hi_word(a)), hi_word(b));
    t.hmin = min(min(t.hmin, hi_word(a)), hi_word(b));
}

template <int D, bool LEAF, unsigned FLIP, bool TWO, bool WANT_TOT, bool SHARED = true>
__device__ __forceinline__ uint32_t cnf_call(char *msg, uint32_t off0, uint32_t off1, uint32_t cnt0, int lane, double rho0, double rho1,
                                             uint32_t prev0, uint32_t prev1, uint32_t &lb0, uint32_t &lb1, Track &t, double &tot0,
                                             double &tot1)
{
    constexpr int M = D - (LEAF ? 1 : 0);
    const uint32_t stride = TWO ? kWaveSize * 8u : cnt0 * 8u;
    char *p0 = msg + off0 + lane * 8, *p1 = msg + off1 + lane * 8;
    double v0[D], v1[D];
    uint32_t par0 = prev0, par1 = prev1;
#pragma unroll
    for (int k = 0; k < M; ++k)
    {
        const double x = *at(p0, k * stride);
        par0 ^= hi_word(x);
        v0[k] = __builtin_fabs(x);
    }
    if constexpr (TWO)
    {
#pragma unroll
        for (int k = 0; k < M; ++k)
        {
            const double x = *at(p1, k * stride);
            par1 ^= hi_word(x);
            v1[k] = __builtin_fabs(x);
        }
    }
    if constexpr (LEAF)
        v0[M] = rho0, v1[M] = rho1;
    auto node = [&](double(&v)[D], uint32_t &lb, double &tot) {
        uint32_t h;
        if constexpr (D == 2)
            h = dm_cnf2(v, FLIP);
        else if constexpr (D == 3)
            h = dm_cnf3(v, FLIP, LEAF, SHARED, &lb, WANT_TOT ? &tot : nullptr);
        else
            h = dm_cnf4(v, FLIP, LEAF, SHARED, &lb, WANT_TOT ? &tot : nullptr);
        t.pmax = max(t.pmax, h);
    };
    node(v0, lb0, tot0);
    if constexpr (TWO)
        node(v1, lb1, tot1);
#pragma unroll
    for (int k = 0; k < M; ++k)
        *at(p0, k * stride) = v0[k];
    if constexpr (TWO)
    {
#pragma unroll
        for (int k = 0; k < M; ++k)
            *at(p1, k * stride) = v1[k];
        return par0 | par1;
    }
    return par0;
}

constexpr unsigned cls_key(int d, int leaf, int nm) { return static_cast<unsigned>(d) | (static_cast<unsigned>(leaf) << 3) | ((((1u << nm) - 1u) << (d - leaf - nm)) << 4); }
constexpr unsigned cls_flip(int d, int leaf, int nm) { return ((1u << nm) - 1u) << (d - leaf - nm); }

__device__ __forceinline__ void vn2_pair(char *msg, uint32_t packed_a, uint32_t packed_b, double ra, double rb, Track &t, uint32_t &sga,
                                         uint32_t &sgb, double &ta, double &tb)
{
    asm volatile("" : "+v"(packed_a), "+v"(packed_b));
    const uint32_t a0 = packed_a & 0xFFFFu, a1 = packed_a >> 16, b0 = packed_b & 0xFFFFu, b1 = packed_b >> 16;
    const double ca0 = __builtin_fabs(*at(msg, a0)), ca1 = __builtin_fabs(*at(msg, a1));
    const double cb0 = __builtin_fabs(*at(msg, b0)), cb1 = __builtin_fabs(*at(msg, b1));
    const double oa0 = ra * ca1, oa1 = ra * ca0, ob0 = rb * cb1, ob1 = rb * cb0;
    ta = oa0 * ca0, tb = ob0 * cb0;
    sga = ta <= 1.0 ? 0x80000000u : 0u, sgb = tb <= 1.0 ? 0x80000000u : 0u;
    track2(t, oa0, oa1);
    track2(t, ob0, ob1);
    *at(msg, a0) = with_sign(oa0, sga), *at(msg, a1) = with_sign(oa1, sga);
    *at(msg, b0) = with_sign(ob0, sgb), *at(msg, b1) = with_sign(ob1, sgb);
}

__device__ __forceinline__ void vn2_one(char *msg, uint32_t packed_a, double ra, Track &t, uint32_t &sga, double &ta)
{
    asm volatile("" : "+v"(packed_a));
    const uint32_t a0 = packed_a & 0xFFFFu, a1 = packed_a >> 16;
    const double ca0 = __builtin_fabs(*at(msg, a0)), ca1 = __builtin_fabs(*at(msg, a1));
    const double oa0 = ra * ca1, oa1 = ra * ca0;
    ta = oa0 * ca0;
    sga = ta <= 1.0 ? 0x80000000u : 0u;
    track2(t, oa0, oa1);
    *at(msg, a0) = with_sign(oa0, sga), *at(msg, a1) = with_sign(oa1, sga);
}

template <int DV, bool TWICE>
__device__ __forceinline__ double vn_wide(char *msg, const uint32_t (&packed)[8], double lam, Track &t, uint32_t &sg)
{
    uint32_t pk[(DV + 1) / 2];
#pragma unroll
    for (int i = 0; i < (DV + 1) / 2; ++i)
    {
        pk[i] = packed[i];
        asm volatile("" : "+v"(pk[i]));
    }
    auto slot = [&](int p) { return at(msg, (p & 1) ? pk[p >> 1] >> 16 : pk[p >> 1] & 0xFFFFu); };
    double c[DV];
#pragma unroll
    for (int p = 0; p < DV; ++p)
        c[p] = __builtin_fabs(*slot(p));
    if constexpr (TWICE)
    {
#pragma unroll
        for (int i = 0; i < (DV + 1) / 2; ++i)
            asm volatile("" : "+v"(pk[i]));
    }
    double prod = lam;
#pragma unroll
    for (int p = 0; p < DV; ++p)
    {
        prod *= c[p];
        if (DV > 3 && p % 3 == 2)
            track(t, prod);
    }
    sg = prod >= 1.0 ? 0x80000000u : 0u;
    const double tot = with_sign(dm_ratio_div(1.0, prod), sg);
    uint32_t nmax = 0u, nmin = 0xFFFFFFFFu;
#pragma unroll
    for (int p = 0; p + 1 < DV; p += 2)
    {
        const double o0 = tot * c[p], o1 = tot * c[p + 1];
        nmax = max(max(nmax, hi_word(o0)), hi_word(o1));
        nmin = min(min(nmin, hi_word(o0)), hi_word(o1));
        *slot(p) = o0, *slot(p + 1) = o1;
    }
    if constexpr (DV % 2 == 1)
    {
        const double o = tot * c[DV - 1];
        nmax = max(nmax, hi_word(o)), nmin = min(nmin, hi_word(o));
        *slot(DV - 1) = o;
    }
    t.hmax = max(t.hmax, nmax & 0x7FFFFFFFu);
    t.hmin = min(t.hmin, nmin & 0x7FFFFFFFu);
    return prod;
}

__device__ __forceinline__ double vn_table(char *msg, const uint32_t *tbl, int lane, int count, int degree, double lam, Track &t, uint32_t &sg)
{
    double prod = lam;
    for (int p = 0; p < degree; ++p)
    {
        prod *= __builtin_fabs(*at(msg, tbl[p * count + lane]));
        if (degree > 3 && p % 3 == 2)
            track(t, prod);
    }
    sg = prod >= 1.0 ? 0x80000000u : 0u;
    const double tot = dm_ratio_div(1.0, prod);
    for (int p = 0; p < degree; ++p)
    {
        double *m = at(msg, tbl[p * count + lane]);
        const double o = tot * __builtin_fabs(*m);
        track(t, o);
        *m = with_sign(o, sg);
    }
    return prod;
}

__device__ __forceinline__ int wave_sum(int v)
{
#pragma unroll
    for (int o = 32; o > 0; o >>= 1)
        v += __shfl_xor(v, o, 64);
    return v;
}

struct AwgnFrame
{
    const uint64_t *p0;
    uint32_t t1, t2, d1, d2;
    bool ok;
};
__device__ __forceinline__ AwgnFrame awgn_frame(const DecodeArgs &a, uint64_t frame, int nct)
{
    AwgnFrame f;
    const uint64_t g0 = a.normal_base + frame * static_cast<uint64_t>(nct);
    const uint64_t q_lo = g0 >> 1, q_hi = (g0 + nct - 1) >> 1;
    const auto cum = uniform_table(a.slab_cum);
    const uint64_t rel_lo = q_lo - a.pair_origin, rel_hi = q_hi - a.pair_origin;
    uint32_t j0 = static_cast<uint32_t>(static_cast<float>(rel_lo) * a.slab_pairs_inv);
    j0 = j0 < a.n_slabs ? j0 : a.n_slabs - 1;
    uint32_t jb = j0 > 0 ? j0 - 1 : 0;
    uint64_t c0 = cum[jb], c1 = cum[jb + 1], c2 = cum[jb + 2], c3 = cum[jb + 3];
    if (!(c0 <= rel_lo && rel_hi < c3))
    {
        while (j0 > 0 && rel_lo < cum[j0])
            --j0;
        while (j0 + 1 < a.n_slabs && rel_lo >= cum[j0 + 1])
            ++j0;
        jb = j0;
        c0 = cum[jb], c1 = cum[jb + 1], c2 = cum[jb + 2], c3 = cum[jb + 3];
    }
    f.ok = c0 <= rel_lo && rel_hi < c3;
    auto threshold = [&](uint64_t c) -> uint32_t {
        if (c <= rel_lo)
            return 0u;
        const uint64_t dlt = c - rel_lo;
        return dlt > 0x3FFFFFFFull ? 0x7FFFFFFFu : static_cast<uint32_t>(2 * dlt - (g0 & 1));
    };
    f.t1 = threshold(c1), f.t2 = threshold(c2);
    f.p0 = a.pairs + (static_cast<uint64_t>(jb) * a.slab_words + g0 - 2 * (a.pair_origin + c0));
    f.d1 = static_cast<uint32_t>(a.slab_words - 2 * (c1 - c0));
    f.d2 = static_cast<uint32_t>(a.slab_words - 2 * (c2 - c1));
    return f;
}

template <int NK, typename Put>
__device__ __forceinline__ bool stage_channel(const DecodeArgs &a, const DevFusedPlan &F, uint64_t frame, int tid, Put &&put)
{
    const DevPlan &P = a.plan;
    const int nc = P.nc, nct = P.nct;
    const uint8_t *cw = a.codeword ? a.codeword + frame * nc : nullptr;
    const bool given = a.mode == kModeLlr;
    const int n_stage = given ? nc : nct;
    bool ok = true;
    double *dump = a.llr_in_dump ? a.llr_in_dump + frame * nc : nullptr;
    if (dump && !given)
        for (int r = tid; r < nc; r += kThreads)
            if (const uint8_t k = P.rank_kind[r]; k != 0)
                dump[P.rank_col[r]] = k == 2 ? a.shorten_llr : 0.0;
    if (given)
    {
        const double *in = a.llr_in + frame * nc;
        for (int s = tid; s < n_stage; s += kThreads)
        {
            const double L = in[s];
            if (dump)
                dump[s] = L;
            put(s, L);
        }
    }
    else if (counter_mode<NK>(a))
    {
        const bool awgn = a.mode == kModeAwgnCtr;
        const uint64_t f = a.ctr_frame0 + frame;
        for (int b = tid; 4 * b < n_stage; b += kThreads)
        {
            const uint4 w = philox_block(a.ctr_key[0], a.ctr_key[1], f, static_cast<uint32_t>(b), awgn ? kTagAwgn : kTagDraw);
            float2 p0{0.f, 0.f}, p1{0.f, 0.f};
            if (awgn)
                p0 = box_muller(w.x, w.y), p1 = box_muller(w.z, w.w);
#pragma unroll
            for (int k = 0; k < 4; ++k)
            {
                const int i = 4 * b + k;
                if (i >= n_stage)
                    break;
                int xb = 0, col = 0;
                if (cw || dump)
                    col = P.bit_pos[i];
                if (cw)
                    xb = static_cast<int>(cw[col]);
                double L;
                if (awgn)
                {
                    const double noise = static_cast<double>(pick_normal(p0, p1, k)) * a.sigma + 0.0;
                    const double xs = cw ? static_cast<double>(1 - 2 * xb) : 1.0;
                    const double y = noise + xs;
                    L = dm_div_by(2 * y, a.sigma2, a.inv_sigma2);
                }
                else
                {
                    const int y = xb ^ (counter_hit(word_of(w, k), a.eps) ? 1 : 0);
                    L = a.delta * static_cast<double>(1 - 2 * y);
                }
                if (dump)
                    dump[col] = L;
                put(i, L);
            }
        }
    }
    else if (a.mode == kModeAwgn)
    {
        const AwgnFrame f = awgn_frame(a, frame, nct);
        ok = f.ok;
        if (f.ok)
            for (int i = tid; i < n_stage; i += kThreads)
            {
                const uint32_t ui = static_cast<uint32_t>(i);
                const uint32_t off = ui + (ui >= f.t1 ? f.d1 : 0u) + (ui >= f.t2 ? f.d2 : 0u);
                const uint64_t w = __builtin_nontemporal_load(f.p0 + off);
                int xb = 0;
                int col = 0;
                if (cw || dump)
                    col = P.bit_pos[i];
                if (cw)
                    xb = static_cast<int>(cw[col]);
                const double noise = dm_from_bits(w) * a.sigma + 0.0;
                const double xs = cw ? static_cast<double>(1 - 2 * xb) : 1.0;
                const double y = noise + xs;
                const double L = dm_div_by(2 * y, a.sigma2, a.inv_sigma2);
                if (dump)
                    dump[col] = L;
                put(i, L);
            }
    }
    else
    {
        const uint64_t *raw = a.raw + frame * static_cast<uint64_t>(nct);
        for (int i = tid; i < n_stage; i += kThreads)
        {
            int xb = 0, col = 0;
            if (cw || dump)
                col = P.bit_pos[i];
            if (cw)
                xb = static_cast<int>(cw[col]);
            const int flip = canonical(raw[i]) < a.eps;
            const int y = xb ^ flip;
            const double L = a.delta * static_cast<double>(1 - 2 * y);
            if (dump)
                dump[col] = L;
            put(i, L);
        }
    }
    if (tid == kThreads - 1 && F.has_shortened && !given)
        put(n_stage, a.shorten_llr);
    return ok;
}

template <bool WANT_LLR, int VNB, int CNL, bool EXCL, bool HO = false, int NK = kNoiseStream>
__device__ __forceinline__ void fused_body(const DecodeArgs &a, const DevFusedPlan &F)
{
    extern __shared__ double lds[];
    __shared__ int misc[4];
    __shared__ int votes[2][kDecodeWaves];
    const DevPlan &P = a.plan;
    const int nc = P.nc, nct = P.nct;
    const uint64_t frame = blockIdx.x;
    char *msg = reinterpret_cast<char *>(lds);
    const int tid = threadIdx.x;
    const int lane = tid & 63;
    const int wave = __builtin_amdgcn_readfirstlane(tid >> 6);
    __builtin_amdgcn_s_setprio(LDPC_AMD_DECODE_PRIO);
    const uint8_t *cw = a.codeword ? a.codeword + frame * nc : nullptr;
    if (tid == 0)
        misc[0] = 0;
    Track t{DM_BOX_LO_WORD, DM_BOX_LO_WORD, 0u};

    const bool given = a.mode == kModeLlr;
    const int n_stage = given ? nc : nct;
    double2 *stage = reinterpret_cast<double2 *>(lds);
    {
        const bool need_lambda = F.need_lambda != 0 || given;
        auto put = [&](int s, double L) {
            if (!(__builtin_fabs(L) <= DM_RATIO_LLR_LIMIT))
                t.hmax = 0xFFFFFFFFu;
            stage[s] = double2{need_lambda ? dm_exp_clamped(0.0 - L) : 1.0, dm_exp_clamped(L)};
        };
        if (!stage_channel<NK>(a, F, frame, tid, put))
            t.hmax = 0xFFFFFFFFu;
        if (tid == kThreads - 1)
            stage[n_stage + 1] = double2{1.0, 1.0};
    }

    const uint32_t *tab = F.lane_tab + (static_cast<uint32_t>(wave) * kFusedLaneRows) * kWaveSize + lane;
    const auto my_vdesc = uniform_table(F.vn_desc + wave * kFusedVnSlots * 4);
    const uint32_t vn_prog = F.vn_prog[wave];
    auto vn_cnt = [&](int w) { return my_vdesc[4 * w] & 0xFFFFu; };
    auto vn_deg = [&](int w) { return my_vdesc[4 * w] >> 16; };
    static_assert(!EXCL || VNB == 4, "the shared layout is written for four slots");
    const bool is_wide = (vn_prog & 0xFu) == kFusedVnWide;
    uint32_t my_idx[VNB + 1], wide_idx[8], vn_entry[VNB], leaf_entry[2 * CNL];
    if constexpr (EXCL)
    {
#pragma unroll
        for (int i = 0; i < 4; ++i)
            wide_idx[i] = tab[((is_wide ? 8 : 0) + i) * kWaveSize];
#pragma unroll
        for (int i = 4; i < 8; ++i)
            wide_idx[i] = tab[(8 + i) * kWaveSize];
    }
    else
    {
#pragma unroll
        for (int w = 0; w < VNB; ++w)
            my_idx[w] = tab[w * kWaveSize];
#pragma unroll
        for (int i = 0; i < 8; ++i)
            wide_idx[i] = tab[(8 + i) * kWaveSize];
    }
    my_idx[VNB] = 0;
    const uint32_t none_entry = static_cast<uint32_t>(n_stage + 1) * 16u;
#pragma unroll
    for (int w = 0; w < VNB; ++w)
    {
        if (given)
        {
            const uint32_t cwd = tab[(24 + w) * kWaveSize];
            vn_entry[w] = cwd == kFusedNone ? none_entry : (cwd & 0x3FFFFFFFu) * 16u;
        }
        else
            vn_entry[w] = tab[(16 + w) * kWaveSize];
    }
#pragma unroll
    for (int c = 0; c < 2 * CNL; ++c)
    {
        if (given)
        {
            const uint32_t cwd = tab[(36 + c) * kWaveSize];
            leaf_entry[c] = cwd == kFusedNone ? none_entry : (cwd & 0x3FFFFFFFu) * 16u;
        }
        else
            leaf_entry[c] = tab[(32 + c) * kWaveSize];
    }
    __syncthreads();

    double my_val[VNB + 1];
    double leaf_rho[2 * CNL];
    double first_v2c[VNB];
    my_val[VNB] = 1.0;
#pragma unroll
    for (int w = 0; w < VNB; ++w)
    {
        const double2 e = *reinterpret_cast<const double2 *>(msg + vn_entry[w]);
        first_v2c[w] = e.y;
        my_val[w] = vn_deg(w) == 2 ? e.y : e.x;
    }
#pragma unroll
    for (int c = 0; c < 2 * CNL; ++c)
        leaf_rho[c] = reinterpret_cast<const double2 *>(msg + leaf_entry[c])->y;
    __syncthreads();
    auto idx_at = [&](int w) { return EXCL ? wide_idx[w] : my_idx[w]; };
#pragma unroll
    for (int w = 0; w < VNB; ++w)
    {
        const int cnt = vn_cnt(w), deg = vn_deg(w);
        if (lane >= cnt)
            continue;
        if (deg == 2)
        {
            *at(msg, idx_at(w) & 0xFFFFu) = first_v2c[w];
            *at(msg, idx_at(w) >> 16) = first_v2c[w];
        }
        else if (w == 0 && deg <= 15)
        {
#pragma unroll
            for (int q = 0; q < 15; ++q)
                if (q < deg)
                    *at(msg, (wide_idx[q >> 1] >> (16 * (q & 1))) & 0xFFFFu) = first_v2c[w];
        }
        else if constexpr (!EXCL)
        {
            const uint32_t *idx = F.vn_slot + my_vdesc[4 * w + 1] + lane;
            for (int p = 0; p < deg; ++p)
                *at(msg, idx[p * cnt]) = first_v2c[w];
        }
    }
    if constexpr (EXCL)
        if (!is_wide)
        {
            wide_idx[4] = static_cast<uint32_t>(dm_bits(my_val[1])), wide_idx[5] = hi_word(my_val[1]);
            wide_idx[6] = static_cast<uint32_t>(dm_bits(my_val[2])), wide_idx[7] = hi_word(my_val[2]);
        }
    auto val_at = [&](int w) {
        if constexpr (EXCL)
        {
            if (w == 1)
                return dm_from_bits(wide_idx[4] | (static_cast<uint64_t>(wide_idx[5]) << 32));
            if (w == 2)
                return dm_from_bits(wide_idx[6] | (static_cast<uint64_t>(wide_idx[7]) << 32));
        }
        return my_val[w];
    };
    __syncthreads();

    const auto my_leaf_calls = uniform_table(reinterpret_cast<const uint32_t *>(F.leaf_calls + wave * kFusedLeafCalls));
    const auto my_calls = uniform_table(reinterpret_cast<const uint32_t *>(F.calls + wave * F.calls_stride));
    double *out_llr = WANT_LLR ? a.llr_out + frame * nc : nullptr;
    uint32_t leaf_bits = 0;
    uint32_t vn_bits = 0;
    [[maybe_unused]] double leaf_tot[2 * CNL];
    uint32_t I = 0;
    uint32_t bad = 0, new_leaf_bits = 0, bits = 0;
    [[maybe_unused]] int32_t ho_key = 0;
    auto leaf_calls_now = my_leaf_calls;
    auto vdesc_now = my_vdesc;
    uint32_t prog = vn_prog;
    auto refresh_tables = [&] {
        leaf_calls_now = my_leaf_calls;
        vdesc_now = my_vdesc;
        prog = vn_prog;
        asm volatile("" : "+s"(leaf_calls_now), "+s"(vdesc_now), "+s"(prog));
    };
    auto cn_pass = [&] {
        bad = 0, new_leaf_bits = 0;
#pragma unroll
        for (int c = 0; c < CNL; ++c)
        {
            const uint32_t offs = leaf_calls_now[4 * c], cnts = leaf_calls_now[4 * c + 1], cls = leaf_calls_now[4 * c + 2];
            const uint32_t cnt0 = cnts & 0xFFFFu;
            if (cnt0 == 0)
                continue;
            const bool two = (cnts >> 16) != 0;
            uint32_t lb0 = 0, lb1 = 0;
            const uint32_t prev0 = leaf_bits << (31 - 2 * c), prev1 = leaf_bits << (30 - 2 * c);
            double tot0 = 1.0, tot1 = 1.0;
            uint32_t par = 0;
#define LDPC_LEAF_CLASS(D, NM)                                                                                                                 \
    case cls_key(D, 1, NM):                                                                                                                    \
        if (two)                                                                                                                               \
            par = cnf_call<D, true, cls_flip(D, 1, NM), true, WANT_LLR, !HO>(msg, offs & 0xFFFFu, offs >> 16, cnt0, lane, leaf_rho[2 * c],          \
                                                                        leaf_rho[2 * c + 1], prev0, prev1, lb0, lb1, t, tot0, tot1);           \
        else if (lane < static_cast<int>(cnt0))                                                                                                \
            par = cnf_call<D, true, cls_flip(D, 1, NM), false, WANT_LLR, !HO>(msg, offs & 0xFFFFu, 0, cnt0, lane, leaf_rho[2 * c],                  \
                                                                         leaf_rho[2 * c + 1], prev0, prev1, lb0, lb1, t, tot0, tot1);          \
        break;
            switch (cls)
            {
                LDPC_LEAF_CLASS(3, 0)
                LDPC_LEAF_CLASS(3, 1)
                LDPC_LEAF_CLASS(3, 2)
                LDPC_LEAF_CLASS(4, 0)
                LDPC_LEAF_CLASS(4, 1)
                LDPC_LEAF_CLASS(4, 2)
                LDPC_LEAF_CLASS(4, 3)
            default: break;
            }
#undef LDPC_LEAF_CLASS
            bad |= par;
            new_leaf_bits |= (lb0 << (2 * c)) | (lb1 << (2 * c + 1));
            if constexpr (WANT_LLR)
                leaf_tot[2 * c] = tot0, leaf_tot[2 * c + 1] = tot1;
        }
        for (int c = 0; c < F.calls_stride; ++c)
        {
            const uint32_t offs = my_calls[4 * c], cnts = my_calls[4 * c + 1], cls = my_calls[4 * c + 2];
            const uint32_t cnt0 = cnts & 0xFFFFu;
            if (cnt0 == 0)
                break;
            const bool two = (cnts >> 16) != 0;
            uint32_t lb0, lb1;
            double tot0, tot1;
            uint32_t par = 0;
#define LDPC_CLASS(D, NM)                                                                                                                      \
    case cls_key(D, 0, NM):                                                                                                                    \
        if (two)                                                                                                                               \
            par = cnf_call<D, false, cls_flip(D, 0, NM), true, false, !HO>(msg, offs & 0xFFFFu, offs >> 16, cnt0, lane, 0.0, 0.0, 0u, 0u, lb0, lb1, \
                                                                      t, tot0, tot1);                                                          \
        else if (lane < static_cast<int>(cnt0))                                                                                                \
            par = cnf_call<D, false, cls_flip(D, 0, NM), false, false, !HO>(msg, offs & 0xFFFFu, 0, cnt0, lane, 0.0, 0.0, 0u, 0u, lb0, lb1, t,      \
                                                                       tot0, tot1);                                                            \
        break;
            switch (cls)
            {
                LDPC_CLASS(2, 0)
                LDPC_CLASS(2, 1)
                LDPC_CLASS(2, 2)
                LDPC_CLASS(3, 0)
                LDPC_CLASS(3, 1)
                LDPC_CLASS(3, 2)
                LDPC_CLASS(3, 3)
                LDPC_CLASS(4, 0)
                LDPC_CLASS(4, 1)
                LDPC_CLASS(4, 2)
                LDPC_CLASS(4, 3)
                LDPC_CLASS(4, 4)
            default: break;
            }
#undef LDPC_CLASS
            bad |= par;
        }
    };
    auto commit_leaves = [&] {
        leaf_bits = new_leaf_bits;
        if constexpr (WANT_LLR)
        {
#pragma unroll
            for (int c = 0; c < 2 * CNL; ++c)
                if (const uint32_t cwd = tab[(36 + c) * kWaveSize]; cwd != kFusedNone)
                    out_llr[cwd & 0x3FFFFFFFu] = 0.0 - dm_log(leaf_tot[c]);
        }
    };
    auto vn_pass = [&] {
        bits = 0;
        auto note = [&](int w, uint32_t sg) { bits |= (sg >> 31) << w; };
        auto note_total = [&](double total) {
            if constexpr (HO)
            {
                const int32_t k = dm_handover_key(total);
                ho_key = k > ho_key ? k : ho_key;
            }
        };
        [[maybe_unused]] auto put_llr = [&](int w, double llr) {
            if constexpr (WANT_LLR)
                out_llr[tab[(24 + w) * kWaveSize] & 0x3FFFFFFFu] = llr;
        };
        auto one = [&](int w, uint32_t kind) {
            const uint32_t d0 = vdesc_now[4 * w];
            const int cnt = static_cast<int>(d0 & 0xFFFFu), deg = static_cast<int>(d0 >> 16);
            if (lane >= cnt)
                return;
            uint32_t sg;
            if (kind == kFusedVnPair || kind == kFusedVn2)
            {
                double tt;
                vn2_one(msg, idx_at(w), val_at(w), t, sg, tt);
                note_total(tt);
                put_llr(w, dm_log(tt));
            }
            else
            {
                double prod = 1.0;
                if (w == 0 && kind == kFusedVnWide)
                    switch (deg)
                    {
#define LDPC_VN(DV) \
    case DV: prod = vn_wide<DV, EXCL>(msg, wide_idx, my_val[0], t, sg); break;
                        LDPC_VN(3) LDPC_VN(4) LDPC_VN(5) LDPC_VN(6) LDPC_VN(7) LDPC_VN(8) LDPC_VN(9)
                        LDPC_VN(10) LDPC_VN(11) LDPC_VN(12) LDPC_VN(13) LDPC_VN(14) LDPC_VN(15)
#undef LDPC_VN
                    default: sg = 0; break;
                    }
                else if constexpr (!EXCL)
                    prod = vn_table(msg, F.vn_slot + vdesc_now[4 * w + 1], lane, cnt, deg, val_at(w), t, sg);
                else
                    sg = 0;
                note_total(prod);
                put_llr(w, 0.0 - dm_log(prod));
            }
            note(w, sg);
        };
#pragma unroll
        for (int w = 0; w < VNB; w += 2)
        {
            const uint32_t k01 = (prog >> (4 * w)) & 0xFFu;
            if (k01 == (kFusedVnPair | (kFusedVnPair << 4)))
            {
                uint32_t sga, sgb;
                double ta, tb;
                vn2_pair(msg, idx_at(w), idx_at(w + 1), val_at(w), val_at(w + 1), t, sga, sgb, ta, tb);
                note(w, sga), note(w + 1, sgb);
                note_total(ta), note_total(tb);
                put_llr(w, dm_log(ta)), put_llr(w + 1, dm_log(tb));
            }
            else
            {
                if (k01 & 0xFu)
                    one(w, k01 & 0xFu);
                if (k01 >> 4)
                    one(w + 1, k01 >> 4);
            }
        }
        vn_bits = bits;
    };
    if constexpr (HO)
    {
        auto post_vote = [&](uint32_t pass) {
            const int wave_vote = ((__ballot(dm_box_escaped(t.hmax, t.hmin)) != 0) << 1) | ((__ballot(DM_HANDOVER_DUE(ho_key)) != 0) << 2);
            if (lane == 0)
                votes[pass & 1][wave] = wave_vote;
        };
        post_vote(0);
        __syncthreads();
        for (;;)
        {
            int any = 0;
#pragma unroll
            for (int w = 0; w < kDecodeWaves; ++w)
                any |= votes[I & 1][w];
            if (any & 2)
            {
                if (tid == 0)
                {
                    const uint32_t pos = atomicAdd(a.redo_count, 1u);
                    a.redo_list[pos] = static_cast<uint32_t>(frame);
                    a.redo_iter[pos] = 0xFFFFFFFFu;
                }
                return;
            }
            if (I == a.iterations)
                break;
            refresh_tables();
            if (any & 4)
            {
                if (tid == 0)
                {
                    const uint32_t pos = atomicAdd(a.redo_count, 1u);
                    a.redo_list[pos] = static_cast<uint32_t>(frame);
                    a.redo_iter[pos] = I;
                    misc[1] = static_cast<int>(pos);
                }
                __syncthreads();
                double *dst = a.ws_handover + static_cast<uint64_t>(static_cast<uint32_t>(misc[1])) * P.nnz;
                auto ho_call = [&](uint32_t offs, uint32_t cnts, uint32_t cls, int leaf_slot) {
                    const int D = static_cast<int>(cls & 7u), leaf = static_cast<int>((cls >> 3) & 1u), M = D - leaf;
                    for (int h = 0; h < 2; ++h)
                    {
                        const uint32_t off = h ? offs >> 16 : offs & 0xFFFFu, cnt = h ? cnts >> 16 : cnts & 0xFFFFu;
                        if (static_cast<uint32_t>(lane) >= cnt)
                            continue;
                        double v[4] = {1.0, 1.0, 1.0, 1.0};
#pragma unroll
                        for (int k = 0; k < 4; ++k)
                            if (k < M)
                                v[k] = __builtin_fabs(*at(msg, off + (k * cnt + lane) * 8u));
                        const double rl = leaf ? leaf_rho[(2 * leaf_slot + h) & (2 * CNL - 1)] : 1.0;
                        uint32_t lb = 0;
                        if (D == 2)
                            dm_cnf2(v, 0u);
                        else if (D == 3)
                        {
                            if (leaf)
                                v[2] = rl;
                            dm_cnf3(v, 0u, 0, 0, &lb, nullptr);
                        }
                        else
                        {
                            if (leaf)
                                v[3] = rl;
                            dm_cnf4(v, 0u, 0, 0, &lb, nullptr);
                        }
#pragma unroll
                        for (int k = 0; k < 4; ++k)
                            if (k < M)
                                dst[F.ho_map[off / 8u + k * cnt + lane]] = 0.0 - dm_log(v[k]);
                        if (leaf)
                            dst[tab[(40 + ((2 * leaf_slot + h) & 3)) * kWaveSize]] = 0.0 - dm_log(D == 3 ? v[2] : v[3]);
                    }
                };
                for (int c = 0; c < CNL; ++c)
                    if ((leaf_calls_now[4 * c + 1] & 0xFFFFu) != 0)
                        ho_call(leaf_calls_now[4 * c], leaf_calls_now[4 * c + 1], leaf_calls_now[4 * c + 2], c);
                for (int c = 0; c < F.calls_stride; ++c)
                {
                    if ((my_calls[4 * c + 1] & 0xFFFFu) == 0)
                        break;
                    ho_call(my_calls[4 * c], my_calls[4 * c + 1], my_calls[4 * c + 2], 0);
                }
                return;
            }
            cn_pass();
            commit_leaves();
            __syncthreads();
            vn_pass();
            post_vote(I + 1);
            __syncthreads();
            ++I;
        }
    }
    else
    for (;;)
    {
        refresh_tables();
        cn_pass();
        const int ph = I & 1;
        const bool esc = dm_box_escaped(t.hmax, t.hmin) || t.pmax >= DM_FUSED_P_HI;
        const int wave_vote = (__ballot((bad & 0x80000000u) != 0) != 0) | ((__ballot(esc) != 0) << 1);
        if (lane == 0)
            votes[ph][wave] = wave_vote;
        __syncthreads();
        int any = 0;
#pragma unroll
        for (int w = 0; w < kDecodeWaves; ++w)
            any |= votes[ph][w];
        if (any & 2)
        {
            if (tid == 0)
            {
                const uint32_t pos = atomicAdd(a.redo_count, 1u);
                a.redo_list[pos] = static_cast<uint32_t>(frame);
            }
            return;
        }
        if (I > 0 && a.early_term && !(any & 1))
        {
            --I;
            break;
        }
        if (I == a.iterations)
            break;
        commit_leaves();

        vn_pass();
        __syncthreads();
        ++I;
    }

    if (tid == 0 && a.iters)
        a.iters[frame] = I;
    uint8_t *hard = a.hard ? a.hard + frame * nc : nullptr;
    int err = 0;
    if (hard || a.bit_errors)
    {
        int lane_now = lane;
        asm volatile("" : "+v"(lane_now));
        const uint32_t *tab = F.lane_tab + (static_cast<uint32_t>(wave) * kFusedLaneRows) * kWaveSize + lane_now;
        auto account = [&](uint32_t cwd, uint32_t bit) {
            if (cwd == kFusedNone)
                return;
            const uint32_t col = cwd & 0x3FFFFFFFu;
            if (hard)
                hard[col] = static_cast<uint8_t>(bit);
            if (cwd & kFusedCounted)
                err += static_cast<int>(bit) != (cw ? static_cast<int>(cw[col]) : 0);
        };
#pragma unroll
        for (int w = 0; w < VNB; ++w)
            account(tab[(24 + w) * kWaveSize], (vn_bits >> w) & 1u);
#pragma unroll
        for (int c = 0; c < 2 * CNL; ++c)
            account(tab[(36 + c) * kWaveSize], (leaf_bits >> c) & 1u);
    }
    if (a.bit_errors)
    {
        err = wave_sum(err);
        if (lane == 0 && err)
            atomicAdd(&misc[0], err);
        __syncthreads();
        if (tid == 0)
            a.bit_errors[frame] = static_cast<uint32_t>(misc[0]);
    }
}

template <int D, bool LEAF, bool TWO, bool CORR = false>
__device__ __forceinline__ void cnms_call(char *msg, uint32_t off0, uint32_t off1, uint32_t cnt0, int lane, double &lv0, double &lv1,
                                          double L0, double L1, double &out0, double &out1, MsCorr c = MsCorr{1.0, 0.0})
{
    constexpr int M = D - (LEAF ? 1 : 0);
    const uint32_t stride = TWO ? kWaveSize * 8u : cnt0 * 8u;
    char *p0 = msg + off0 + lane * 8, *p1 = msg + off1 + lane * 8;
    double v0[D], v1[D];
#pragma unroll
    for (int k = 0; k < M; ++k)
        v0[k] = *at(p0, k * stride);
    if constexpr (TWO)
    {
#pragma unroll
        for (int k = 0; k < M; ++k)
            v1[k] = *at(p1, k * stride);
    }
    if constexpr (LEAF)
        v0[M] = lv0, v1[M] = lv1;
    cn_core<D, true, CORR>(v0, c);
    if constexpr (TWO)
        cn_core<D, true, CORR>(v1, c);
#pragma unroll
    for (int k = 0; k < M; ++k)
        *at(p0, k * stride) = v0[k];
    if constexpr (TWO)
    {
#pragma unroll
        for (int k = 0; k < M; ++k)
            *at(p1, k * stride) = v1[k];
    }
    if constexpr (LEAF)
    {
        out0 = L0 + v0[M];
        lv0 = out0 - v0[M];
        if constexpr (TWO)
        {
            out1 = L1 + v1[M];
            lv1 = out1 - v1[M];
        }
    }
}

__device__ __forceinline__ void vnms2_pair(char *msg, uint32_t packed_a, uint32_t packed_b, double La, double Lb, double &oa, double &ob)
{
    asm volatile("" : "+v"(packed_a), "+v"(packed_b));
    const uint32_t a0 = packed_a & 0xFFFFu, a1 = packed_a >> 16, b0 = packed_b & 0xFFFFu, b1 = packed_b >> 16;
    const double ca0 = *at(msg, a0), ca1 = *at(msg, a1), cb0 = *at(msg, b0), cb1 = *at(msg, b1);
    oa = La + ca0, ob = Lb + cb0;
    oa += ca1, ob += cb1;
    *at(msg, a0) = oa - ca0, *at(msg, a1) = oa - ca1;
    *at(msg, b0) = ob - cb0, *at(msg, b1) = ob - cb1;
}

__device__ __forceinline__ double vnms2_one(char *msg, uint32_t packed_a, double La)
{
    asm volatile("" : "+v"(packed_a));
    const uint32_t a0 = packed_a & 0xFFFFu, a1 = packed_a >> 16;
    const double ca0 = *at(msg, a0), ca1 = *at(msg, a1);
    double oa = La + ca0;
    oa += ca1;
    *at(msg, a0) = oa - ca0, *at(msg, a1) = oa - ca1;
    return oa;
}

template <int DV>
__device__ __forceinline__ double vnms_wide(char *msg, const uint32_t (&packed)[8], double L)
{
    uint32_t pk[(DV + 1) / 2];
    auto opaque = [&] {
#pragma unroll
        for (int i = 0; i < (DV + 1) / 2; ++i)
        {
            pk[i] = packed[i];
            asm volatile("" : "+v"(pk[i]));
        }
    };
    auto slot = [&](int p) { return at(msg, (p & 1) ? pk[p >> 1] >> 16 : pk[p >> 1] & 0xFFFFu); };
    opaque();
    double c[DV];
#pragma unroll
    for (int p = 0; p < DV; ++p)
        c[p] = *slot(p);
    double out = L;
#pragma unroll
    for (int p = 0; p < DV; ++p)
        out += c[p];
    opaque();
#pragma unroll
    for (int p = 0; p < DV; ++p)
        *slot(p) = out - c[p];
    return out;
}

__device__ __forceinline__ double vnms_table(char *msg, const uint32_t *tbl, int lane, int count, int degree, double L)
{
    double out = L;
    for (int p = 0; p < degree; ++p)
        out += *at(msg, tbl[p * count + lane]);
    for (int p = 0; p < degree; ++p)
    {
        double *m = at(msg, tbl[p * count + lane]);
        *m = out - *m;
    }
    return out;
}

template <bool WANT_LLR, int VNB, int CNL, int NK = kNoiseStream, bool CORR = false>
__device__ __forceinline__ void fused_ms_body(const DecodeArgs &a, const DevFusedPlan &F)
{
    [[maybe_unused]] const MsCorr corr{a.ms_scale, a.ms_offset};
    extern __shared__ double lds[];
    __shared__ int misc[4];
    const DevPlan &P = a.plan;
    const int nc = P.nc, nct = P.nct;
    const uint64_t frame = blockIdx.x;
    char *msg = reinterpret_cast<char *>(lds);
    const int tid = threadIdx.x;
    const int lane = tid & 63;
    const int wave = __builtin_amdgcn_readfirstlane(tid >> 6);
    __builtin_amdgcn_s_setprio(LDPC_AMD_DECODE_PRIO);
    const uint8_t *cw = a.codeword ? a.codeword + frame * nc : nullptr;
    if (tid == 0)
        misc[0] = 0;

    const bool given = a.mode == kModeLlr;
    const int n_stage = given ? nc : nct;
    double2 *stage = reinterpret_cast<double2 *>(lds);
    bool addressed = stage_channel<NK>(a, F, frame, tid, [&](int s, double L) { stage[s].x = L; });
    if (tid == kThreads - 1)
        stage[n_stage + 1].x = 0.0;
    const uint32_t *tab = F.lane_tab + (static_cast<uint32_t>(wave) * kFusedLaneRows) * kWaveSize + lane;
    const auto my_vdesc = uniform_table(F.vn_desc + wave * kFusedVnSlots * 4);
    const uint32_t vn_prog = F.vn_prog[wave];
    uint32_t my_idx[VNB], wide_idx[8], vn_entry[VNB], leaf_entry[2 * CNL];
#pragma unroll
    for (int w = 0; w < VNB; ++w)
        my_idx[w] = tab[w * kWaveSize];
#pragma unroll
    for (int i = 0; i < 8; ++i)
        wide_idx[i] = tab[(8 + i) * kWaveSize];
    const uint32_t none_entry = static_cast<uint32_t>(n_stage + 1) * 16u;
    auto entry_of = [&](int mode_row, int col_row) {
        if (given)
        {
            const uint32_t cwd = tab[col_row * kWaveSize];
            return cwd == kFusedNone ? none_entry : (cwd & 0x3FFFFFFFu) * 16u;
        }
        return tab[mode_row * kWaveSize];
    };
#pragma unroll
    for (int w = 0; w < VNB; ++w)
        vn_entry[w] = entry_of(16 + w, 24 + w);
#pragma unroll
    for (int c = 0; c < 2 * CNL; ++c)
        leaf_entry[c] = entry_of(32 + c, 36 + c);
    __syncthreads();
    double my_L[VNB], leaf_L[2 * CNL], leaf_v2c[2 * CNL];
#pragma unroll
    for (int w = 0; w < VNB; ++w)
        my_L[w] = *at(msg, vn_entry[w]);
#pragma unroll
    for (int c = 0; c < 2 * CNL; ++c)
        leaf_L[c] = leaf_v2c[c] = *at(msg, leaf_entry[c]);
    __syncthreads();
#pragma unroll
    for (int w = 0; w < VNB; ++w)
    {
        const uint32_t d0 = my_vdesc[4 * w];
        const int cnt = static_cast<int>(d0 & 0xFFFFu), deg = static_cast<int>(d0 >> 16);
        if (lane >= cnt)
            continue;
        if (deg == 2)
            *at(msg, my_idx[w] & 0xFFFFu) = my_L[w], *at(msg, my_idx[w] >> 16) = my_L[w];
        else if (w == 0 && deg <= 15)
        {
#pragma unroll
            for (int q = 0; q < 15; ++q)
                if (q < deg)
                    *at(msg, (wide_idx[q >> 1] >> (16 * (q & 1))) & 0xFFFFu) = my_L[w];
        }
        else
        {
            const uint32_t *idx = F.vn_slot + my_vdesc[4 * w + 1];
            for (int p = 0; p < deg; ++p)
                *at(msg, idx[p * cnt + lane]) = my_L[w];
        }
    }
    __syncthreads();

    const auto my_leaf_calls = uniform_table(reinterpret_cast<const uint32_t *>(F.leaf_calls + wave * kFusedLeafCalls));
    const auto my_calls = uniform_table(reinterpret_cast<const uint32_t *>(F.calls + wave * F.calls_stride));
    double *out_llr = WANT_LLR ? a.llr_out + frame * nc : nullptr;
    uint32_t leaf_bits = 0, vn_bits = 0;
    for (uint32_t I = 0; I < a.iterations; ++I)
    {
        const bool last = I + 1 == a.iterations;
        auto leaf_calls_now = my_leaf_calls;
        auto vdesc_now = my_vdesc;
        uint32_t prog = vn_prog;
        asm volatile("" : "+s"(leaf_calls_now), "+s"(vdesc_now), "+s"(prog));
        uint32_t lbits = 0;
#pragma unroll
        for (int c = 0; c < CNL; ++c)
        {
            const uint32_t offs = leaf_calls_now[4 * c], cnts = leaf_calls_now[4 * c + 1], cls = leaf_calls_now[4 * c + 2];
            const uint32_t cnt0 = cnts & 0xFFFFu;
            if (cnt0 == 0)
                continue;
            const bool two = (cnts >> 16) != 0;
            double o0 = 1.0, o1 = 1.0;
#define LDPC_MS_LEAF(D)                                                                                                                   \
    case D:                                                                                                                               \
        if (two)                                                                                                                          \
            cnms_call<D, true, true, CORR>(msg, offs & 0xFFFFu, offs >> 16, cnt0, lane, leaf_v2c[2 * c], leaf_v2c[2 * c + 1],          \
                                           leaf_L[2 * c], leaf_L[2 * c + 1], o0, o1, corr);                                               \
        else if (lane < static_cast<int>(cnt0))                                                                                           \
            cnms_call<D, true, false, CORR>(msg, offs & 0xFFFFu, 0, cnt0, lane, leaf_v2c[2 * c], leaf_v2c[2 * c + 1], leaf_L[2 * c],      \
                                            leaf_L[2 * c + 1], o0, o1, corr);                                                             \
        break;
            switch (cls & 7u)
            {
                LDPC_MS_LEAF(3)
                LDPC_MS_LEAF(4)
            default: break;
            }
#undef LDPC_MS_LEAF
            lbits |= (o0 <= 0 ? 1u : 0u) << (2 * c) | (o1 <= 0 ? 1u : 0u) << (2 * c + 1);
            if constexpr (WANT_LLR)
                if (last)
                {
                    if (const uint32_t cwd = tab[(36 + 2 * c) * kWaveSize]; cwd != kFusedNone)
                        out_llr[cwd & 0x3FFFFFFFu] = o0;
                    if (const uint32_t cwd = tab[(37 + 2 * c) * kWaveSize]; cwd != kFusedNone)
                        out_llr[cwd & 0x3FFFFFFFu] = o1;
                }
        }
        leaf_bits = lbits;
        for (int c = 0; c < F.calls_stride; ++c)
        {
            const uint32_t offs = my_calls[4 * c], cnts = my_calls[4 * c + 1], cls = my_calls[4 * c + 2];
            const uint32_t cnt0 = cnts & 0xFFFFu;
            if (cnt0 == 0)
                break;
            const bool two = (cnts >> 16) != 0;
            double d0 = 0.0, d1 = 0.0, d2 = 0.0, d3 = 0.0;
#define LDPC_MS(D)                                                                                                        \
    case D:                                                                                                               \
        if (two)                                                                                                          \
            cnms_call<D, false, true, CORR>(msg, offs & 0xFFFFu, offs >> 16, cnt0, lane, d0, d1, 0.0, 0.0, d2, d3, corr); \
        else if (lane < static_cast<int>(cnt0))                                                                           \
            cnms_call<D, false, false, CORR>(msg, offs & 0xFFFFu, 0, cnt0, lane, d0, d1, 0.0, 0.0, d2, d3, corr);         \
        break;
            switch (cls & 7u)
            {
                LDPC_MS(2)
                LDPC_MS(3)
                LDPC_MS(4)
            default: break;
            }
#undef LDPC_MS
        }
        __syncthreads();

        uint32_t bits = 0;
        [[maybe_unused]] auto put_llr = [&](int w, double llr) {
            if constexpr (WANT_LLR)
                if (last)
                    out_llr[tab[(24 + w) * kWaveSize] & 0x3FFFFFFFu] = llr;
        };
        auto one = [&](int w, uint32_t kind) {
            const uint32_t d0 = vdesc_now[4 * w];
            const int cnt = static_cast<int>(d0 & 0xFFFFu), deg = static_cast<int>(d0 >> 16);
            if (lane >= cnt)
                return;
            double out = 1.0;
            if (kind == kFusedVnPair || kind == kFusedVn2)
                out = vnms2_one(msg, my_idx[w], my_L[w]);
            else if (w == 0 && kind == kFusedVnWide)
                switch (deg)
                {
#define LDPC_VN(DV) \
    case DV: out = vnms_wide<DV>(msg, wide_idx, my_L[0]); break;
                    LDPC_VN(3) LDPC_VN(4) LDPC_VN(5) LDPC_VN(6) LDPC_VN(7) LDPC_VN(8) LDPC_VN(9)
                    LDPC_VN(10) LDPC_VN(11) LDPC_VN(12) LDPC_VN(13) LDPC_VN(14) LDPC_VN(15)
#undef LDPC_VN
                default: break;
                }
            else
                out = vnms_table(msg, F.vn_slot + vdesc_now[4 * w + 1], lane, cnt, deg, my_L[w]);
            bits |= (out <= 0 ? 1u : 0u) << w;
            put_llr(w, out);
        };
#pragma unroll
        for (int w = 0; w < VNB; w += 2)
        {
            const uint32_t k01 = (prog >> (4 * w)) & 0xFFu;
            if (w + 1 < VNB && k01 == (kFusedVnPair | (kFusedVnPair << 4)))
            {
                double oa, ob;
                vnms2_pair(msg, my_idx[w], my_idx[w + 1], my_L[w], my_L[w + 1], oa, ob);
                bits |= (oa <= 0 ? 1u : 0u) << w | (ob <= 0 ? 1u : 0u) << (w + 1);
                put_llr(w, oa), put_llr(w + 1, ob);
            }
            else
            {
                if (k01 & 0xFu)
                    one(w, k01 & 0xFu);
                if (w + 1 < VNB && (k01 >> 4))
                    one(w + 1, k01 >> 4);
            }
        }
        vn_bits = bits;
        __syncthreads();
    }

    if (tid == 0 && a.iters)
        a.iters[frame] = a.iterations;
    uint8_t *hard = a.hard ? a.hard + frame * nc : nullptr;
    int err = 0;
    if (hard || a.bit_errors)
    {
        auto account = [&](uint32_t cwd, uint32_t bit) {
            if (cwd == kFusedNone)
                return;
            const uint32_t col = cwd & 0x3FFFFFFFu;
            if (hard)
                hard[col] = static_cast<uint8_t>(bit);
            if (cwd & kFusedCounted)
                err += static_cast<int>(bit) != (cw ? static_cast<int>(cw[col]) : 0);
        };
#pragma unroll
        for (int w = 0; w < VNB; ++w)
            account(tab[(24 + w) * kWaveSize], (vn_bits >> w) & 1u);
#pragma unroll
        for (int c = 0; c < 2 * CNL; ++c)
            account(tab[(36 + c) * kWaveSize], (leaf_bits >> c) & 1u);
    }
    if (a.bit_errors)
    {
        err = wave_sum(err);
        if (lane == 0 && err)
            atomicAdd(&misc[0], err);
        __syncthreads();
        if (tid == 0)
            a.bit_errors[frame] = addressed ? static_cast<uint32_t>(misc[0]) : 0xFFFFFFFFu;
    }
}

template <bool WANT_LLR, int VNB, int CNL>
__global__ __launch_bounds__(kThreads) void decode_fused_ms_kernel(const DecodeArgs a, const DevFusedPlan f)
{
    fused_ms_body<WANT_LLR, VNB, CNL>(a, f);
}

__global__ __launch_bounds__(kThreads) __attribute__((amdgpu_waves_per_eu(LDPC_AMD_FUSED_WAVES, LDPC_AMD_FUSED_WAVES))) void
decode_fused_small(const DecodeArgs a, const DevFusedPlan f)
{
    fused_body<false, 4, 1, true>(a, f);
}

template <bool WANT_LLR, int VNB, int CNL>
__global__ __launch_bounds__(kThreads) void decode_fused_ho_kernel(const DecodeArgs a, const DevFusedPlan f)
{
    fused_body<WANT_LLR, VNB, CNL, false, true>(a, f);
}

__global__ __launch_bounds__(kThreads) __attribute__((amdgpu_waves_per_eu(5, 5))) void
decode_fused_ho_small(const DecodeArgs a, const DevFusedPlan f)
{
    fused_body<false, 4, 1, true, true>(a, f);
}

template <bool WANT_LLR, int VNB, int CNL>
__global__ __launch_bounds__(kThreads) void decode_fused_kernel(const DecodeArgs a, const DevFusedPlan f)
{
    fused_body<WANT_LLR, VNB, CNL, false>(a, f);
}

__global__ __launch_bounds__(kThreads) __attribute__((amdgpu_waves_per_eu(LDPC_AMD_FUSED_WAVES, LDPC_AMD_FUSED_WAVES))) void
decode_ctr_fused_small(const DecodeArgs a, const DevFusedPlan f)
{
    fused_body<false, 4, 1, true, false, kNoiseCounter>(a, f);
}

template <bool WANT_LLR, int VNB, int CNL>
__global__ __launch_bounds__(kThreads) void decode_ctr_fused_kernel(const DecodeArgs a, const DevFusedPlan f)
{
    fused_body<WANT_LLR, VNB, CNL, false, false, kNoiseCounter>(a, f);
}

__global__ __launch_bounds__(kThreads) __attribute__((amdgpu_waves_per_eu(5, 5))) void
decode_ctr_fused_ho_small(const DecodeArgs a, const DevFusedPlan f)
{
    fused_body<false, 4, 1, true, true, kNoiseCounter>(a, f);
}

template <bool WANT_LLR, int VNB, int CNL>
__global__ __launch_bounds__(kThreads) void decode_ctr_fused_ho_kernel(const DecodeArgs a, const DevFusedPlan f)
{
    fused_body<WANT_LLR, VNB, CNL, false, true, kNoiseCounter>(a, f);
}

template <bool WANT_LLR, int VNB, int CNL>
__global__ __launch_bounds__(kThreads) void decode_ctr_fused_ms_kernel(const DecodeArgs a, const DevFusedPlan f)
{
    fused_ms_body<WANT_LLR, VNB, CNL, kNoiseCounter>(a, f);
}

template <bool WANT_LLR, int VNB, int CNL, int NK>
__global__ __launch_bounds__(kThreads) void decode_fused_msc_kernel(const DecodeArgs a, const DevFusedPlan f)
{
    fused_ms_body<WANT_LLR, VNB, CNL, NK, true>(a, f);
}

using FusedKernel = void (*)(const DecodeArgs, const DevFusedPlan);

template <bool WANT_LLR, int VNB, int CNL>
FusedKernel fused_kernel_of(Stage stage, bool counter, bool ms_correct, [[maybe_unused]] bool exclusive)
{
    constexpr bool kHasSmall = !WANT_LLR && VNB == 4 && CNL == 1;
    switch (stage)
    {
    case Stage::kRatioFirst:
        if constexpr (kHasSmall)
            if (exclusive)
                return counter ? decode_ctr_fused_small : decode_fused_small;
        return counter ? decode_ctr_fused_kernel<WANT_LLR, VNB, CNL> : decode_fused_kernel<WANT_LLR, VNB, CNL>;
    case Stage::kHandoverFirst:
        if constexpr (kHasSmall)
            if (exclusive)
                return counter ? decode_ctr_fused_ho_small : decode_fused_ho_small;
        return counter ? decode_ctr_fused_ho_kernel<WANT_LLR, VNB, CNL> : decode_fused_ho_kernel<WANT_LLR, VNB, CNL>;
    case Stage::kWhole:
        if (ms_correct)
            return counter ? decode_fused_msc_kernel<WANT_LLR, VNB, CNL, kNoiseCounter> : decode_fused_msc_kernel<WANT_LLR, VNB, CNL, kNoiseStream>;
        return counter ? decode_ctr_fused_ms_kernel<WANT_LLR, VNB, CNL> : decode_fused_ms_kernel<WANT_LLR, VNB, CNL>;
    default:
        return nullptr;
    }
}

}

int launch_decode_fused(const DecodeArgs &a, const DevFusedPlan &f, Stage stage, void *stream)
{
    if (a.n_frames == 0)
        return hipSuccess;
    if (!stage_args_ok(a, stage) || (stage == Stage::kWhole && (a.early_term || a.iterations == 0)))
        return hipErrorInvalidValue;
    if (f.vnb > kFusedVnSlots || f.cnl > kFusedLeafCalls)
        return hipErrorInvalidValue;
    const bool counter = a.mode == kModeAwgnCtr || a.mode == kModeBscCtr, exclusive = f.wide_exclusive != 0;
    FusedKernel k = nullptr;
    if (f.vnb <= 4 && f.cnl <= 1)
        k = a.llr_out ? fused_kernel_of<true, 4, 1>(stage, counter, a.ms_correct, exclusive)
                      : fused_kernel_of<false, 4, 1>(stage, counter, a.ms_correct, exclusive);
    else
        k = a.llr_out ? fused_kernel_of<true, kFusedVnSlots, kFusedLeafCalls>(stage, counter, a.ms_correct, exclusive)
                      : fused_kernel_of<false, kFusedVnSlots, kFusedLeafCalls>(stage, counter, a.ms_correct, exclusive);
    if (!k)
        return hipErrorInvalidValue;
    hipError_t e = hipFuncSetAttribute(reinterpret_cast<const void *>(k), hipFuncAttributeMaxDynamicSharedMemorySize, static_cast<int>(f.lds_bytes));
    if (e != hipSuccess)
        return e;
    hipLaunchKernelGGL(k, dim3(static_cast<unsigned>(a.n_frames)), dim3(kThreads), f.lds_bytes, static_cast<hipStream_t>(stream), a, f);
    return hipGetLastError();
}

}
```

libldpc_amd/csrc/plan.cpp:

```cpp
#include "plan.hpp"

#include "fused_rule.h"

#include <algorithm>
#include <cstdio>
#include <cstdlib>
#include <map>
#include <numeric>
#include <stdexcept>

namespace ldpc_amd
{

namespace
{
void deal(const std::vector<int> &cost, std::vector<uint32_t> &work, int &stride)
{
    std::vector<int> order(cost.size());
    std::iota(order.begin(), order.end(), 0);
    std::stable_sort(order.begin(), order.end(), [&](int a, int b) { return cost[a] > cost[b]; });
    std::vector<std::vector<uint32_t>> lists(kDecodeWaves);
    std::vector<long> load(kDecodeWaves, 0);
    for (int b : order)
    {
        int w = static_cast<int>(std::min_element(load.begin(), load.end()) - load.begin());
        lists[w].push_back(static_cast<uint32_t>(b));
        load[w] += cost[b];
    }
    stride = 1;
    for (auto &l : lists)
        stride = std::max(stride, static_cast<int>(l.size()));
    work.assign(static_cast<size_t>(kDecodeWaves) * stride, 0xFFFF);
    for (int w = 0; w < kDecodeWaves; ++w)
        std::copy(lists[w].begin(), lists[w].end(), work.begin() + static_cast<size_t>(w) * stride);
}
}

Plan build_plan(const LdpcCode &code)
{
    Plan p;
    const SparseGF2 &H = code.H;
    p.nc = code.nc(), p.mc = code.mc(), p.nnz = code.nnz(), p.nct = code.nct();
    p.max_cn_degree = code.max_cn_degree();
    p.max_vn_degree = code.max_vn_degree();

    std::vector<int> rows(p.mc);
    std::iota(rows.begin(), rows.end(), 0);
    auto rdeg = [&](int r) { return H.rptr[r + 1] - H.rptr[r]; };
    std::stable_sort(rows.begin(), rows.end(), [&](int a, int b) { return rdeg(a) < rdeg(b); });
    p.edge_slot.assign(p.nnz, 0);
    p.cn_rank_row.assign(rows.begin(), rows.end());
    uint32_t slot = 0;
    std::vector<int> cn_cost;
    for (int i = 0; i < p.mc;)
    {
        int d = rdeg(rows[i]), j = i;
        while (j < p.mc && j - i < kWaveSize && rdeg(rows[j]) == d)
            ++j;
        CnBlock b{slot, static_cast<uint16_t>(j - i), static_cast<uint16_t>(d)};
        for (int l = 0; l < j - i; ++l)
            for (int k = 0; k < d; ++k)
                p.edge_slot[H.redge[H.rptr[rows[i + l]] + k]] = slot + k * (j - i) + l;
        slot += static_cast<uint32_t>(d) * (j - i);
        p.cn_blocks.push_back(b);
        cn_cost.push_back(10 * d + 15 * (d - 2));
        i = j;
    }

    std::vector<int> cols(p.nc);
    std::iota(cols.begin(), cols.end(), 0);
    auto cdeg = [&](int c) { return H.cptr[c + 1] - H.cptr[c]; };
    std::stable_sort(cols.begin(), cols.end(), [&](int a, int b) { return cdeg(a) > cdeg(b); });
    p.rank_col.resize(p.nc), p.col_rank.resize(p.nc);
    for (int r = 0; r < p.nc; ++r)
    {
        p.rank_col[r] = static_cast<uint32_t>(cols[r]);
        p.col_rank[cols[r]] = static_cast<uint32_t>(r);
    }
    std::vector<int> vn_cost;
    int vn_cost_a = 2, vn_cost_b = 2;
    if (const char *e = std::getenv("LDPC_AMD_VN_COST"))
        std::sscanf(e, "%d,%d", &vn_cost_a, &vn_cost_b);
    for (int i = 0; i < p.nc;)
    {
        int d = cdeg(cols[i]), j = i;
        while (j < p.nc && j - i < kWaveSize && cdeg(cols[j]) == d)
            ++j;
        VnBlock b{static_cast<uint32_t>(p.vn_slot.size()), static_cast<uint32_t>(i), static_cast<uint16_t>(j - i),
                  static_cast<uint16_t>(d)};
        for (int k = 0; k < d; ++k)
            for (int l = 0; l < j - i; ++l)
                p.vn_slot.push_back(p.edge_slot[H.cedge[H.cptr[cols[i + l]] + k]]);
        p.vn_blocks.push_back(b);
        vn_cost.push_back(vn_cost_a * d + vn_cost_b);
        i = j;
    }
    p.has_isolated_vn = p.nc > 0 && cdeg(cols[p.nc - 1]) == 0;
    p.rank_slot0.assign(p.nc, kNoSlot);
    for (int r = 0; r < p.nc; ++r)
        if (cdeg(cols[r]) > 0)
            p.rank_slot0[r] = p.edge_slot[H.cedge[H.cptr[cols[r]]]];
    if (p.vn_slot.empty())
        p.vn_slot.push_back(0);

    deal(cn_cost, p.cn_work, p.cn_work_stride);
    deal(vn_cost, p.vn_work, p.vn_work_stride);
    p.vn_work_desc.assign(static_cast<size_t>(kDecodeWaves) * (p.vn_work_stride + 1) * 4, 0);
    for (int w = 0; w < kDecodeWaves; ++w)
        for (int i = 0; i < p.vn_work_stride; ++i)
            if (uint32_t b = p.vn_work[static_cast<size_t>(w) * p.vn_work_stride + i]; b != 0xFFFF)
            {
                uint32_t *d = &p.vn_work_desc[(static_cast<size_t>(w) * (p.vn_work_stride + 1) + i) * 4];
                const VnBlock &vb = p.vn_blocks[b];
                d[0] = vb.idx_off, d[1] = vb.first, d[2] = vb.count | (static_cast<uint32_t>(vb.degree) << 16);
            }
    p.cn_desc_stride = (p.cn_work_stride + 1) / 2 * 2 + 2;
    p.cn_work_desc.assign(static_cast<size_t>(kDecodeWaves) * p.cn_desc_stride, CnBlock{0, 0, 0});
    for (int w = 0; w < kDecodeWaves; ++w)
        for (int i = 0; i < p.cn_work_stride; ++i)
            if (uint32_t b = p.cn_work[static_cast<size_t>(w) * p.cn_work_stride + i]; b != 0xFFFF)
                p.cn_work_desc[static_cast<size_t>(w) * p.cn_desc_stride + i] = p.cn_blocks[b];

    p.rank_kind.assign(p.nc, 0);
    for (int c : code.puncture)
        if (c >= 0 && c < p.nc)
            p.rank_kind[p.col_rank[c]] = 1;
    for (int c : code.shorten)
        if (c >= 0 && c < p.nc)
            p.rank_kind[p.col_rank[c]] = 2;
    p.n_bitpos = static_cast<int>(code.bit_pos.size());
    p.nct = std::min(p.nct, p.n_bitpos);
    p.tx_rank.resize(code.bit_pos.size());
    for (size_t i = 0; i < code.bit_pos.size(); ++i)
    {
        p.tx_rank[i] = p.col_rank[code.bit_pos[i]];
        if (static_cast<int>(i) >= p.nct)
            p.rank_kind[p.tx_rank[i]] = 3;
    }
    p.rank_kind.resize((static_cast<size_t>(p.nc) + 7) / 8 * 8, 0);

    if (p.nnz < 65536 && p.vn_work_stride <= 8)
    {
        p.vn_packed.assign(static_cast<size_t>(kDecodeWaves) * kVnPackedRows * kWaveSize, 0);
        std::vector<uint32_t> rank_tx(p.nc, kVnSrcZero);
        for (int i = 0; i < p.nct; ++i)
            rank_tx[p.tx_rank[i]] = static_cast<uint32_t>(i);
        for (int w = 0; w < kDecodeWaves; ++w)
        {
            uint32_t *rows = &p.vn_packed[static_cast<size_t>(w) * kVnPackedRows * kWaveSize];
            std::fill(rows + 16 * kWaveSize, rows + 32 * kWaveSize, kVnSrcZero);
            for (int i = 0; i < p.vn_work_stride; ++i)
            {
                const uint32_t bi = p.vn_work[static_cast<size_t>(w) * p.vn_work_stride + i];
                if (bi == 0xFFFF)
                    continue;
                const VnBlock &vb = p.vn_blocks[bi];
                auto slot = [&](int edge, int lane) { return p.vn_slot[vb.idx_off + static_cast<size_t>(edge) * vb.count + lane]; };
                for (int l = 0; l < vb.count; ++l)
                {
                    if (vb.degree >= 1 && vb.degree <= 2)
                        rows[i * kWaveSize + l] = slot(0, l) | (slot(vb.degree - 1, l) << 16);
                    else if (i == 0 && vb.degree <= 16)
                        for (int q = 0; q < vb.degree; ++q)
                            rows[(8 + q / 2) * kWaveSize + l] |= slot(q, l) << (16 * (q & 1));
                    const uint32_t r = vb.first + l;
                    const uint8_t kind = p.rank_kind[r];
                    rows[(16 + i) * kWaveSize + l] = kind == 2 ? kVnSrcShortened : (kind == 0 ? rank_tx[r] : kVnSrcZero);
                    rows[(24 + i) * kWaveSize + l] = p.rank_col[r];
                }
            }
        }
    }

    p.lds_bytes = static_cast<size_t>(8) * p.nnz + static_cast<size_t>(8) * p.nc + ((p.nnz + 15) / 16) * 16 + 16;
    p.lds_ok = code.min_cn_degree() >= 2 && p.max_cn_degree <= kMaxLdsCnDegree && p.lds_bytes <= 160 * 1024 &&
               p.cn_blocks.size() < 0xFFFF && p.vn_blocks.size() < 0xFFFF;
    p.hbm_ok = code.min_cn_degree() >= 2 && p.cn_blocks.size() < 0xFFFF && p.vn_blocks.size() < 0xFFFF;
    return p;
}

RegPlan build_reg_plan(const LdpcCode &code, const Plan &plan, int nt, int kc, int maxd, uint32_t lds_budget)
{
    RegPlan r;
    r.nt = nt, r.kc = kc, r.maxd = maxd;
    const int kRegWaves = nt / kWaveSize, kRegThreads = nt;
    const SparseGF2 &H = code.H;
    const int n_cb = static_cast<int>(plan.cn_blocks.size());
    if (code.min_cn_degree() < 2 || plan.max_cn_degree > maxd || n_cb > kc * kRegWaves || plan.nnz >= (1 << 28))
        return r;
    const uint32_t cap = ((lds_budget - 256) / 9) & ~63u;
    std::vector<uint32_t> block_round(plan.vn_blocks.size()), block_off(plan.vn_blocks.size());
    uint32_t fill = 0, round = 0, peak = 0;
    r.round_first.push_back(0);
    for (size_t b = 0; b < plan.vn_blocks.size(); ++b)
    {
        const VnBlock &vb = plan.vn_blocks[b];
        const uint32_t need = static_cast<uint32_t>(vb.degree) * vb.count;
        if (need > cap)
            return r;
        if (fill + need > cap)
        {
            ++round;
            fill = 0;
            r.round_first.push_back(static_cast<uint32_t>(b));
        }
        block_round[b] = round;
        block_off[b] = fill;
        fill += need;
        peak = std::max(peak, fill);
        r.vn_blocks.push_back(RegVnBlock{vb.first, block_off[b], vb.count, vb.degree});
    }
    r.round_first.push_back(static_cast<uint32_t>(plan.vn_blocks.size()));
    r.rounds = static_cast<int>(round) + 1;
    if (r.rounds > 15)
        return r;
    r.mb_doubles = (peak + 63) & ~63u;

    std::vector<uint32_t> edge_mb(plan.nnz);
    for (size_t b = 0; b < plan.vn_blocks.size(); ++b)
    {
        const VnBlock &vb = plan.vn_blocks[b];
        for (int l = 0; l < vb.count; ++l)
        {
            const int col = static_cast<int>(plan.rank_col[vb.first + l]);
            for (int p = 0; p < vb.degree; ++p)
                edge_mb[H.cedge[H.cptr[col] + p]] = (block_round[b] << 28) | (block_off[b] + p * vb.count + l);
        }
    }
    r.cn_edge.assign(static_cast<size_t>(kc) * maxd * kRegThreads, kRegNoEdge);
    r.cn_deg.assign(static_cast<size_t>(kc) * kRegWaves, 0);
    r.cn_cnt.assign(static_cast<size_t>(kc) * kRegWaves, 0);
    int rank = 0;
    for (int bi = 0; bi < n_cb; ++bi)
    {
        const CnBlock &cb = plan.cn_blocks[bi];
        const int k = bi / kRegWaves, wave = bi % kRegWaves;
        r.cn_deg[k * kRegWaves + wave] = static_cast<uint8_t>(cb.degree);
        r.cn_cnt[k * kRegWaves + wave] = static_cast<uint8_t>(cb.count);
        for (int l = 0; l < cb.count; ++l, ++rank)
        {
            const int row = static_cast<int>(plan.cn_rank_row[rank]);
            const int tid = wave * kWaveSize + l;
            for (int j = 0; j < cb.degree; ++j)
                r.cn_edge[(static_cast<size_t>(k) * maxd + j) * kRegThreads + tid] = edge_mb[H.redge[H.rptr[row] + j]];
        }
    }
    r.ok = true;
    return r;
}

Reg2Plan build_reg2_plan(const LdpcCode &code, const Plan &plan, int nt, int kc, int maxd, int nv0, int nv1)
{
    Reg2Plan r;
    r.nt = nt, r.kc = kc, r.maxd = maxd, r.nv0 = nv0, r.nv1 = nv1;
    const int W = nt / kWaveSize, NT = nt;
    const SparseGF2 &H = code.H;
    const int n_cb = static_cast<int>(plan.cn_blocks.size()), n_vb = static_cast<int>(plan.vn_blocks.size());
    if (code.min_cn_degree() < 2 || plan.max_cn_degree > maxd || n_cb > kc * W || plan.has_isolated_vn || kc * maxd > 64 ||
        n_vb > W * (nv0 + nv1) || plan.nnz == 0)
        return r;
    for (const VnBlock &vb : plan.vn_blocks)
        if (vb.degree < 2)
            return r;
    const int cap[2] = {W * nv0, W * nv1};
    std::vector<int> rb[2];
    long ent[2] = {0, 0};
    for (int b = 0; b < n_vb; ++b)
    {
        const bool ok0 = static_cast<int>(rb[0].size()) < cap[0], ok1 = static_cast<int>(rb[1].size()) < cap[1];
        const int rd = (ok0 && (!ok1 || ent[0] * cap[1] <= ent[1] * cap[0])) ? 0 : 1;
        rb[rd].push_back(b);
        ent[rd] += static_cast<long>(plan.vn_blocks[b].degree) * plan.vn_blocks[b].count;
    }
    const uint32_t c0_area = static_cast<uint32_t>(rb[1].size()) * kWaveSize;
    uint32_t e0 = 0, e1 = c0_area;
    r.vn_blocks.assign(static_cast<size_t>(W) * (nv0 + nv1), Reg2VnBlock{0, 0, 0, 0, 0});
    r.vn_rank.assign(static_cast<size_t>(W) * (nv0 + nv1) * kWaveSize, kNoSlot);
    std::vector<uint32_t> edge_gather(plan.nnz), edge_scatter(plan.nnz);
    std::vector<uint8_t> edge_round(plan.nnz);
    std::vector<Reg2VnBlock *> placed[2];
    std::vector<size_t> placed_pos[2];
    for (int rd = 0; rd < 2; ++rd)
        for (size_t q = 0; q < rb[rd].size(); ++q)
        {
            const VnBlock &vb = plan.vn_blocks[rb[rd][q]];
            const size_t pos = (q / W + (rd ? nv0 : 0)) * W + q % W;
            Reg2VnBlock &o = r.vn_blocks[pos];
            o.count = vb.count, o.degree = vb.degree;
            if (rd == 0)
            {
                o.p0_off = e0, o.prest_off = e0 + vb.count;
                o.tot_off = static_cast<uint32_t>(q) * kWaveSize;
                e0 += static_cast<uint32_t>(vb.degree) * vb.count;
            }
            else
            {
                o.p0_off = static_cast<uint32_t>(q) * kWaveSize, o.tot_off = o.p0_off;
                o.prest_off = e1;
                e1 += static_cast<uint32_t>(vb.degree - 1) * vb.count;
            }
            placed[rd].push_back(&o);
            placed_pos[rd].push_back(pos);
        }
    r.e_max = (std::max(e0, e1) + 31u) & ~31u;
    const uint32_t n_tot0 = static_cast<uint32_t>(rb[0].size()) * kWaveSize;
    const uint32_t tot_base = r.e_max + n_tot0 <= kReg2TrashEntry ? r.e_max : kReg2TrashEntry + kWaveSize;
    r.neutral = std::max(tot_base + n_tot0, kReg2TrashEntry + 1);
    r.lds_entries = r.neutral + 2;
    if (r.e_max > kReg2TrashEntry || static_cast<size_t>(r.lds_entries) * 8 + 64 > 160 * 1024)
        return r;
    for (Reg2VnBlock *o : placed[0])
        o->tot_off += tot_base;

    struct Slot { uint32_t rd, q, lane; };
    const int max_deg = plan.max_vn_degree;
    std::vector<std::vector<std::vector<Slot>>> free_slots(max_deg + 1, std::vector<std::vector<Slot>>(64));
    for (int rd = 0; rd < 2; ++rd)
        for (size_t q = rb[rd].size(); q-- > 0;)
        {
            const VnBlock &vb = plan.vn_blocks[rb[rd][q]];
            for (uint32_t l = vb.count; l-- > 0;)
                free_slots[vb.degree][rd * 32 + l % 32].push_back(Slot{static_cast<uint32_t>(rd), static_cast<uint32_t>(q), l});
        }
    const uint32_t n_gg = static_cast<uint32_t>(kc) * maxd * W * 2, n_sg = static_cast<uint32_t>(kc) * maxd * W * 4;
    std::vector<uint32_t> edge_gg(plan.nnz), edge_sg(plan.nnz);
    {
        int crank = 0;
        for (int bi = 0; bi < n_cb; ++bi)
        {
            const CnBlock &cb = plan.cn_blocks[bi];
            for (int l = 0; l < cb.count; ++l, ++crank)
            {
                const int row = static_cast<int>(plan.cn_rank_row[crank]);
                for (int j = 0; j < cb.degree; ++j)
                {
                    const int e = H.redge[H.rptr[row] + j];
                    const uint32_t inst = static_cast<uint32_t>(bi) * maxd + j;
                    edge_gg[e] = inst * 2 + l / 32;
                    edge_sg[e] = inst * 4 + l / 16;
                }
            }
        }
    }
    std::vector<uint16_t> g_cnt(static_cast<size_t>(n_gg) * 32, 0), s_cnt(static_cast<size_t>(n_sg) * 2 * 16, 0);
    for (size_t g = 0; g < s_cnt.size(); g += 16)
        s_cnt[g + kReg2TrashEntry % 16] = 1;
    std::vector<uint32_t> order(plan.nc);
    std::iota(order.begin(), order.end(), 0u);
    uint64_t rng = 0x9E3779B97F4A7C15ull;
    for (size_t i = order.size(); i > 1; --i)
    {
        rng ^= rng >> 12, rng ^= rng << 25, rng ^= rng >> 27;
        std::swap(order[i - 1], order[(rng * 0x2545F4914F6CDD1Dull >> 33) % i]);
    }
    std::vector<Slot> rank_slot(plan.nc);
    for (uint32_t rank : order)
    {
        const int col = static_cast<int>(plan.rank_col[rank]);
        const int d = H.cptr[col + 1] - H.cptr[col];
        long best = -1;
        int best_class = -1;
        for (int cls = 0; cls < 64; ++cls)
        {
            if (free_slots[d][cls].empty())
                continue;
            const int rd = cls / 32, colour = cls % 32;
            long cost = 0;
            for (int p = 0; p < d; ++p)
            {
                const int e = H.cedge[H.cptr[col] + p];
                cost += 4l * g_cnt[static_cast<size_t>(edge_gg[e]) * 32 + colour] +
                        s_cnt[(static_cast<size_t>(edge_sg[e]) * 2 + rd) * 16 + colour % 16];
            }
            cost = cost * 4096 + static_cast<long>(4096 - free_slots[d][cls].size());
            if (best < 0 || cost < best)
                best = cost, best_class = cls;
        }
        if (best_class < 0)
            return r;
        const Slot sl = free_slots[d][best_class].back();
        free_slots[d][best_class].pop_back();
        rank_slot[rank] = sl;
        for (int p = 0; p < d; ++p)
        {
            const int e = H.cedge[H.cptr[col] + p];
            ++g_cnt[static_cast<size_t>(edge_gg[e]) * 32 + best_class % 32];
            ++s_cnt[(static_cast<size_t>(edge_sg[e]) * 2 + best_class / 32) * 16 + (best_class % 32) % 16];
        }
    }
    for (uint32_t rank = 0; rank < static_cast<uint32_t>(plan.nc); ++rank)
    {
        const Slot sl = rank_slot[rank];
        const Reg2VnBlock &o = *placed[sl.rd][sl.q];
        r.vn_rank[placed_pos[sl.rd][sl.q] * kWaveSize + sl.lane] = rank;
        const int col = static_cast<int>(plan.rank_col[rank]);
        const int d = H.cptr[col + 1] - H.cptr[col];
        for (int p = 0; p < d; ++p)
        {
            const int e = H.cedge[H.cptr[col] + p];
            edge_gather[e] = o.tot_off + sl.lane;
            edge_scatter[e] = p == 0 ? o.p0_off + sl.lane : o.prest_off + static_cast<uint32_t>(p - 1) * o.count + sl.lane;
            edge_round[e] = static_cast<uint8_t>(sl.rd);
        }
    }
    r.edge_w.assign(static_cast<size_t>(kc) * maxd * NT, (r.neutral << 3) | 2u);
    r.cn_deg.assign(static_cast<size_t>(kc) * W, 0), r.cn_cnt.assign(static_cast<size_t>(kc) * W, 0);
    int rank = 0;
    for (int bi = 0; bi < n_cb; ++bi)
    {
        const CnBlock &cb = plan.cn_blocks[bi];
        const int k = bi / W, wave = bi % W;
        r.cn_deg[k * W + wave] = static_cast<uint8_t>(cb.degree);
        r.cn_cnt[k * W + wave] = static_cast<uint8_t>(cb.count);
        for (int l = 0; l < cb.count; ++l, ++rank)
        {
            const int row = static_cast<int>(plan.cn_rank_row[rank]);
            const int tid = wave * kWaveSize + l;
            for (int j = 0; j < cb.degree; ++j)
            {
                const int e = H.redge[H.rptr[row] + j], s = k * maxd + j;
                r.edge_w[static_cast<size_t>(s) * NT + tid] = (edge_gather[e] << 3) | (edge_scatter[e] << 18) | edge_round[e];
            }
        }
    }
    r.uniform_cn = std::all_of(r.cn_deg.begin(), r.cn_deg.end(), [&](uint8_t d) { return d == maxd; });
    r.uniform_vn = nv0 >= 2 && nv1 >= 2;
    for (int rd = 0; rd < 2 && r.uniform_vn; ++rd)
    {
        const int nvr = rd ? nv1 : nv0;
        auto blk = [&](int q) -> const Reg2VnBlock & { return r.vn_blocks[static_cast<size_t>(q / W + (rd ? nv0 : 0)) * W + q % W]; };
        const Reg2VnBlock &b0 = blk(0), &b1 = blk(1);
        uint32_t *af = r.vn_affine[rd];
        af[0] = b0.p0_off, af[1] = b1.p0_off - b0.p0_off, af[2] = b0.prest_off, af[3] = b1.prest_off - b0.prest_off;
        af[4] = b0.tot_off, af[5] = b1.tot_off - b0.tot_off;
        for (int q = 0; q < nvr * W && r.uniform_vn; ++q)
        {
            const Reg2VnBlock &b = blk(q);
            r.uniform_vn = b.count == kWaveSize && b.degree == 3 && b.p0_off == af[0] + af[1] * q && b.prest_off == af[2] + af[3] * q &&
                           b.tot_off == af[4] + af[5] * q;
        }
    }
    r.ok = true;
    return r;
}

FusedPlan build_fused_plan(const LdpcCode &code, const Plan &plan)
{
    FusedPlan f;
    const SparseGF2 &H = code.H;
    if (!plan.lds_ok || plan.has_isolated_vn || H.rows <= 0 ||
        !dm_fused_applies(H.rows, H.cols, H.rptr.data(), H.rcol.data(), H.cptr.data()))
        return f;
    const int W = kDecodeWaves;
    auto cdeg = [&](int c) { return H.cptr[c + 1] - H.cptr[c]; };

    struct Row
    {
        int row, order[4];
    };
    std::map<unsigned, std::vector<Row>> by_class;
    for (int i = 0; i < H.rows; ++i)
    {
        Row r{i, {0, 0, 0, 0}};
        unsigned flip;
        int leaf;
        const int d = H.rptr[i + 1] - H.rptr[i];
        if (!dm_fused_row_order(d, H.rcol.data() + H.rptr[i], H.cptr.data(), r.order, &flip, &leaf))
            return f;
        by_class[dm_fused_class(d, flip, leaf)].push_back(r);
    }
    struct Block
    {
        unsigned cls;
        uint32_t off;
        std::vector<Row> rows;
    };
    std::vector<Block> blocks;
    f.edge_slot.assign(plan.nnz, kNoSlot);
    uint32_t slot = 0;
    for (auto &[cls, rows] : by_class)
    {
        const int d = static_cast<int>(cls & 7u), leaf = static_cast<int>((cls >> 3) & 1u), m = d - leaf;
        for (size_t i = 0; i < rows.size(); i += kWaveSize)
        {
            Block b{cls, slot, {}};
            b.rows.assign(rows.begin() + i, rows.begin() + std::min(rows.size(), i + kWaveSize));
            const uint32_t cnt = static_cast<uint32_t>(b.rows.size());
            for (uint32_t l = 0; l < cnt; ++l)
                for (int k = 0; k < m; ++k)
                    f.edge_slot[H.redge[H.rptr[b.rows[l].row] + b.rows[l].order[k]]] = slot + k * cnt + l;
            slot += static_cast<uint32_t>(m) * cnt;
            blocks.push_back(std::move(b));
        }
    }
    f.n_slots = static_cast<int>(slot);
    if (f.n_slots > DM_FUSED_MAX_SLOTS)
        return f;
    f.ho_map.assign(static_cast<size_t>(f.n_slots), 0);
    for (int e = 0; e < plan.nnz; ++e)
        if (f.edge_slot[e] != kNoSlot)
            f.ho_map[f.edge_slot[e]] = plan.edge_slot[e];

    struct Call
    {
        int b0, b1;
        int cost;
        bool leaf;
    };
    auto class_cost = [](unsigned cls) {
        const int d = static_cast<int>(cls & 7u), leaf = static_cast<int>((cls >> 3) & 1u);
        return d == 2 ? 12 : (d == 3 ? (leaf ? 28 : 30) : (leaf ? 45 : 50));
    };
    std::vector<Call> calls;
    for (size_t b = 0; b < blocks.size();)
    {
        const bool pair = b + 1 < blocks.size() && blocks[b + 1].cls == blocks[b].cls && blocks[b].rows.size() == kWaveSize &&
                          blocks[b + 1].rows.size() == kWaveSize;
        const bool leaf = (blocks[b].cls >> 3) & 1u;
        calls.push_back(Call{static_cast<int>(b), pair ? static_cast<int>(b + 1) : -1, class_cost(blocks[b].cls) * (pair ? 2 : 1) + 4, leaf});
        b += pair ? 2 : 1;
    }
    std::vector<std::vector<int>> w_leaf(W), w_rest(W);
    std::vector<long> load(W, 0);
    {
        std::vector<int> order(calls.size());
        std::iota(order.begin(), order.end(), 0);
        std::stable_sort(order.begin(), order.end(), [&](int a, int b) { return calls[a].cost > calls[b].cost; });
        int n_leaf = 0;
        for (const Call &c : calls)
            n_leaf += c.leaf;
        const int leaf_cap = (n_leaf + W - 1) / W;
        if (leaf_cap > kFusedLeafCalls)
            return f;
        for (int ci : order)
            if (calls[ci].leaf)
            {
                int best = -1;
                for (int w = 0; w < W; ++w)
                    if (static_cast<int>(w_leaf[w].size()) < leaf_cap && (best < 0 || load[w] < load[best]))
                        best = w;
                w_leaf[best].push_back(ci);
                load[best] += calls[ci].cost;
            }
        for (int ci : order)
            if (!calls[ci].leaf)
            {
                const int w = static_cast<int>(std::min_element(load.begin(), load.end()) - load.begin());
                w_rest[w].push_back(ci);
                load[w] += calls[ci].cost;
            }
        f.cnl = leaf_cap;
    }
    auto describe = [&](const Call &c) {
        const Block &b0 = blocks[c.b0];
        FusedCall d{b0.off * 8u, static_cast<uint32_t>(b0.rows.size()), b0.cls, 0};
        if (c.b1 >= 0)
        {
            d.offs |= (blocks[c.b1].off * 8u) << 16;
            d.cnts |= static_cast<uint32_t>(blocks[c.b1].rows.size()) << 16;
        }
        return d;
    };
    f.leaf_calls.assign(static_cast<size_t>(W) * kFusedLeafCalls, FusedCall{0, 0, 0, 0});
    f.calls_stride = 1;
    for (int w = 0; w < W; ++w)
        f.calls_stride = std::max(f.calls_stride, static_cast<int>(w_rest[w].size()) + 1);
    f.calls.assign(static_cast<size_t>(W) * f.calls_stride, FusedCall{0, 0, 0, 0});
    for (int w = 0; w < W; ++w)
    {
        for (size_t i = 0; i < w_leaf[w].size(); ++i)
            f.leaf_calls[static_cast<size_t>(w) * kFusedLeafCalls + i] = describe(calls[w_leaf[w][i]]);
        for (size_t i = 0; i < w_rest[w].size(); ++i)
            f.calls[static_cast<size_t>(w) * f.calls_stride + i] = describe(calls[w_rest[w][i]]);
    }

    std::vector<int> cols;
    for (int c = 0; c < H.cols; ++c)
        if (cdeg(c) >= 2)
            cols.push_back(c);
    std::stable_sort(cols.begin(), cols.end(), [&](int a, int b) { return cdeg(a) > cdeg(b); });
    struct VBlock
    {
        int degree;
        std::vector<int> cols;
    };
    std::vector<VBlock> vblocks;
    for (size_t i = 0; i < cols.size();)
    {
        size_t j = i;
        while (j < cols.size() && j - i < kWaveSize && cdeg(cols[j]) == cdeg(cols[i]))
            ++j;
        vblocks.push_back(VBlock{cdeg(cols[i]), std::vector<int>(cols.begin() + i, cols.begin() + j)});
        i = j;
    }
    std::vector<std::vector<int>> w_vn(W);
    {
        std::vector<int> order(vblocks.size());
        std::iota(order.begin(), order.end(), 0);
        auto cost = [&](int b) { return vblocks[b].degree == 2 ? 13 : 5 * vblocks[b].degree + 8; };
        std::stable_sort(order.begin(), order.end(), [&](int a, int b) { return cost(a) > cost(b); });
        std::vector<long> vload(W, 0);
        for (int b : order)
        {
            int best = -1;
            for (int w = 0; w < W; ++w)
                if (static_cast<int>(w_vn[w].size()) < kFusedVnSlots - 1 && (best < 0 || vload[w] < vload[best]))
                    best = w;
            if (best < 0)
                for (int w = 0; w < W; ++w)
                    if (static_cast<int>(w_vn[w].size()) < kFusedVnSlots && (best < 0 || vload[w] < vload[best]))
                        best = w;
            if (best < 0)
                return f;
            w_vn[best].push_back(b);
            vload[best] += cost(b);
        }
    }
    std::vector<uint32_t> col_entry(H.cols, static_cast<uint32_t>(plan.nct) + 1u), col_word(H.cols);
    for (int c = 0; c < H.cols; ++c)
        col_word[c] = static_cast<uint32_t>(c);
    for (int i = 0; i < static_cast<int>(code.bit_pos.size()); ++i)
    {
        if (i < plan.nct)
            col_entry[code.bit_pos[i]] = static_cast<uint32_t>(i);
        col_word[code.bit_pos[i]] |= kFusedCounted;
    }
    for (int c : code.shorten)
        if (c >= 0 && c < H.cols && plan.rank_kind[plan.col_rank[c]] == 2)
            col_entry[c] = static_cast<uint32_t>(plan.nct);
    f.has_shortened = !code.shorten.empty();
    for (int c = 0; c < H.cols; ++c)
        if (cdeg(c) >= 3 && col_entry[c] <= static_cast<uint32_t>(plan.nct))
            f.need_lambda = true;

    f.vn_desc.assign(static_cast<size_t>(W) * kFusedVnSlots * 4, 0);
    f.lane_tab.assign(static_cast<size_t>(W) * kFusedLaneRows * kWaveSize, 0);
    f.vnb = 1;
    for (int w = 0; w < W; ++w)
    {
        uint32_t *tab = &f.lane_tab[static_cast<size_t>(w) * kFusedLaneRows * kWaveSize];
        for (int r = 16; r < 24; ++r)
            std::fill(tab + r * kWaveSize, tab + (r + 1) * kWaveSize, (static_cast<uint32_t>(plan.nct) + 1u) * 16u);
        for (int r = 32; r < 36; ++r)
            std::fill(tab + r * kWaveSize, tab + (r + 1) * kWaveSize, (static_cast<uint32_t>(plan.nct) + 1u) * 16u);
        for (int r = 24; r < 32; ++r)
            std::fill(tab + r * kWaveSize, tab + (r + 1) * kWaveSize, kFusedNone);
        for (int r = 36; r < 40; ++r)
            std::fill(tab + r * kWaveSize, tab + (r + 1) * kWaveSize, kFusedNone);
        for (int r = 40; r < 44; ++r)
            std::fill(tab + r * kWaveSize, tab + (r + 1) * kWaveSize, 0u);
        std::vector<int> &mine = w_vn[w];
        std::stable_sort(mine.begin(), mine.end(), [&](int a, int b) { return vblocks[a].degree > vblocks[b].degree; });
        std::vector<int> slots;
        for (int b : mine)
        {
            if (vblocks[b].degree == 2 && slots.size() % 2 == 1 && !slots.empty() && slots.back() >= 0 && vblocks[slots.back()].degree != 2 &&
                mine.size() + 1 <= static_cast<size_t>(kFusedVnSlots))
                slots.push_back(-1);
            slots.push_back(b);
        }
        if (static_cast<int>(slots.size()) > kFusedVnSlots)
            return f;
        f.vnb = std::max(f.vnb, static_cast<int>(slots.size()));
        for (size_t sw = 0; sw < slots.size(); ++sw)
        {
            if (slots[sw] < 0)
                continue;
            const VBlock &vb = vblocks[slots[sw]];
            const uint32_t cnt = static_cast<uint32_t>(vb.cols.size());
            uint32_t *d = &f.vn_desc[(static_cast<size_t>(w) * kFusedVnSlots + sw) * 4];
            d[0] = cnt | (static_cast<uint32_t>(vb.degree) << 16);
            d[1] = static_cast<uint32_t>(f.vn_slot.size());
            auto eslot = [&](int l, int p) { return f.edge_slot[H.cedge[H.cptr[vb.cols[l]] + p]] * 8u; };
            const bool in_regs = vb.degree == 2 || (sw == 0 && vb.degree <= 15);
            f.vn_prog[w] |= (vb.degree == 2 ? (cnt == kWaveSize ? kFusedVnPair : kFusedVn2) : (in_regs ? kFusedVnWide : kFusedVnTable)) << (4 * sw);
            if (!in_regs)
                for (int p = 0; p < vb.degree; ++p)
                    for (uint32_t l = 0; l < cnt; ++l)
                        f.vn_slot.push_back(eslot(static_cast<int>(l), p));
            for (uint32_t l = 0; l < cnt; ++l)
            {
                if (vb.degree == 2)
                    tab[sw * kWaveSize + l] = eslot(l, 0) | (eslot(l, 1) << 16);
                else if (in_regs)
                    for (int q = 0; q < vb.degree; ++q)
                        tab[(8 + q / 2) * kWaveSize + l] |= eslot(l, q) << (16 * (q & 1));
                tab[(16 + sw) * kWaveSize + l] = col_entry[vb.cols[l]] * 16u;
                tab[(24 + sw) * kWaveSize + l] = col_word[vb.cols[l]];
            }
        }
        for (size_t c = 0; c < w_leaf[w].size(); ++c)
            for (int h = 0; h < 2; ++h)
            {
                const int bi = h == 0 ? calls[w_leaf[w][c]].b0 : calls[w_leaf[w][c]].b1;
                if (bi < 0)
                    continue;
                const Block &b = blocks[bi];
                const int d = static_cast<int>(b.cls & 7u);
                for (size_t l = 0; l < b.rows.size(); ++l)
                {
                    const int col = H.rcol[H.rptr[b.rows[l].row] + b.rows[l].order[d - 1]];
                    tab[(32 + 2 * c + h) * kWaveSize + l] = col_entry[col] * 16u;
                    tab[(36 + 2 * c + h) * kWaveSize + l] = col_word[col];
                    tab[(40 + 2 * c + h) * kWaveSize + l] = plan.edge_slot[H.redge[H.rptr[b.rows[l].row] + b.rows[l].order[d - 1]]];
                }
            }
    }
    if (f.vn_slot.empty())
        f.vn_slot.push_back(0);
    f.wide_exclusive = true;
    for (int w = 0; w < W; ++w)
    {
        if ((f.vn_prog[w] & 0xFu) == kFusedVnWide && (f.vn_prog[w] >> 4) != 0)
            f.wide_exclusive = false;
        for (int sw = 0; sw < kFusedVnSlots; ++sw)
            if (((f.vn_prog[w] >> (4 * sw)) & 0xFu) == kFusedVnTable)
                f.wide_exclusive = false;
    }
    f.ok = true;
    return f;
}

LayerPlan build_layer_plan(const LdpcCode &code, const Plan &plan)
{
    LayerPlan L;
    const SparseGF2 &H = code.H;
    if (H.cols > 0xFFFF || code.max_cn_degree() > kMaxLdsCnDegree || code.min_cn_degree() < 2)
        return L;
    struct Open
    {
        int degree;
        std::vector<int> rows;
        std::vector<uint8_t> used;
    };
    std::vector<Open> open;
    for (int i = 0; i < H.rows; ++i)
    {
        const int deg = H.rptr[i + 1] - H.rptr[i];
        Open *dst = nullptr;
        for (Open &o : open)
        {
            if (o.degree != deg || static_cast<int>(o.rows.size()) >= kWaveSize)
                continue;
            bool clash = false;
            for (int p = H.rptr[i]; p < H.rptr[i + 1] && !clash; ++p)
                clash = o.used[H.rcol[p]] != 0;
            if (!clash)
            {
                dst = &o;
                break;
            }
        }
        if (!dst)
        {
            open.push_back({deg, {}, std::vector<uint8_t>(H.cols, 0)});
            dst = &open.back();
        }
        dst->rows.push_back(i);
        for (int p = H.rptr[i]; p < H.rptr[i + 1]; ++p)
            dst->used[H.rcol[p]] = 1;
    }
    L.step_of_row.assign(H.rows, -1);
    for (size_t si = 0; si < open.size(); ++si)
        for (int i : open[si].rows)
            L.step_of_row[i] = static_cast<int>(si);
    for (const Open &o : open)
    {
        LayerStep st{static_cast<uint32_t>(L.vn.size()), static_cast<uint16_t>(o.rows.size()), static_cast<uint16_t>(o.degree)};
        L.vn.resize(L.vn.size() + static_cast<size_t>(o.degree) * kWaveSize, 0);
        for (size_t l = 0; l < o.rows.size(); ++l)
        {
            const int i = o.rows[l];
            for (int j = 0; j < o.degree; ++j)
                L.vn[st.off + static_cast<size_t>(j) * kWaveSize + l] = static_cast<uint16_t>(plan.col_rank[H.rcol[H.rptr[i] + j]]);
        }
        L.steps.push_back(st);
    }
    L.slots = static_cast<uint32_t>(L.vn.size());
    L.ok = !L.steps.empty();
    return L;
}

}
```

libldpc_amd/csrc/plan.hpp:

```cpp
#pragma once

#include <cstdint>
#include <vector>

#include "code.hpp"

namespace ldpc_amd
{

constexpr int kWaveSize = 64;
constexpr int kMaxLdsCnDegree = 8;
constexpr int kMaxCnDegree = 16;
constexpr uint32_t kNoSlot = 0xFFFFFFFFu;
constexpr int kDecodeWaves = 4;

struct CnBlock
{
    uint32_t off;
    uint16_t count;
    uint16_t degree;
};

constexpr int kVnPackedRows = 32;
constexpr uint32_t kVnSrcZero = 0xFFFFFFFFu, kVnSrcShortened = 0xFFFFFFFEu;

struct VnBlock
{
    uint32_t idx_off;
    uint32_t first;
    uint16_t count;
    uint16_t degree;
};

struct Plan
{
    int nc = 0, mc = 0, nnz = 0, nct = 0;
    int n_bitpos = 0;
    int max_cn_degree = 0, max_vn_degree = 0;
    std::vector<CnBlock> cn_blocks;
    std::vector<VnBlock> vn_blocks;
    std::vector<uint32_t> vn_slot;
    std::vector<uint32_t> cn_work;
    std::vector<uint32_t> vn_work;
    int cn_work_stride = 0, vn_work_stride = 0;
    std::vector<CnBlock> cn_work_desc;
    int cn_desc_stride = 0;
    std::vector<uint32_t> vn_work_desc;
    std::vector<uint32_t> vn_packed;
    std::vector<uint32_t> col_rank;
    std::vector<uint32_t> rank_col;
    std::vector<uint32_t> tx_rank;
    std::vector<uint8_t> rank_kind;
    std::vector<uint32_t> rank_slot0;
    std::vector<uint32_t> edge_slot;
    std::vector<uint32_t> cn_rank_row;
    size_t lds_bytes = 0;
    bool lds_ok = false;
    bool hbm_ok = false;
    bool has_isolated_vn = false;
};

constexpr uint32_t kRegNoEdge = 0xFFFFFFFFu;

struct RegVnBlock
{
    uint32_t first;
    uint32_t mb_off;
    uint16_t count;
    uint16_t degree;
};

struct RegPlan
{
    bool ok = false;
    int nt = 0;
    int kc = 0, maxd = 0;
    int rounds = 0;
    uint32_t mb_doubles = 0;
    std::vector<uint32_t> cn_edge;
    std::vector<uint8_t> cn_deg;
    std::vector<uint8_t> cn_cnt;
    std::vector<RegVnBlock> vn_blocks;
    std::vector<uint32_t> round_first;
};


constexpr uint32_t kReg2TrashEntry = 16384;

struct Reg2VnBlock
{
    uint32_t p0_off;
    uint32_t prest_off;
    uint32_t tot_off;
    uint16_t count;
    uint16_t degree;
};

struct Reg2Plan
{
    bool ok = false;
    int nt = 0, kc = 0, maxd = 0, nv0 = 0, nv1 = 0;
    uint32_t e_max = 0, neutral = 0, lds_entries = 0;
    bool uniform_cn = false;
    bool uniform_vn = false;
    uint32_t vn_affine[2][6] = {};
    std::vector<uint32_t> edge_w;
    std::vector<uint8_t> cn_deg;
    std::vector<uint8_t> cn_cnt;
    std::vector<Reg2VnBlock> vn_blocks;
    std::vector<uint32_t> vn_rank;
};

struct LayerStep
{
    uint32_t off;
    uint16_t count, degree;
};
struct LayerPlan
{
    bool ok = false;
    std::vector<LayerStep> steps;
    std::vector<uint16_t> vn;
    uint32_t slots = 0;
    std::vector<int> step_of_row;
};
LayerPlan build_layer_plan(const LdpcCode &code, const Plan &plan);

constexpr int kFusedVnSlots = 8;
constexpr int kFusedLeafCalls = 2;
constexpr int kFusedLaneRows = 44;
struct FusedCall
{
    uint32_t offs;
    uint32_t cnts;
    uint32_t cls;
    uint32_t pad;
};
struct FusedPlan
{
    bool ok = false;
    int n_slots = 0;
    int vnb = 0, cnl = 0;
    bool has_shortened = false;
    bool need_lambda = false;
    bool wide_exclusive = false;
    std::vector<FusedCall> leaf_calls;
    std::vector<FusedCall> calls;
    int calls_stride = 0;
    std::vector<uint32_t> vn_desc;
    uint32_t vn_prog[kDecodeWaves] = {0, 0, 0, 0};
    std::vector<uint32_t> vn_slot;
    std::vector<uint32_t> lane_tab;
    std::vector<uint32_t> edge_slot;
    std::vector<uint32_t> ho_map;
};
constexpr uint32_t kFusedCounted = 0x80000000u, kFusedNone = 0xFFFFFFFFu;
enum : uint32_t { kFusedVnNone = 0, kFusedVnPair = 1 , kFusedVn2 = 2 , kFusedVnWide = 3 , kFusedVnTable = 4 };
FusedPlan build_fused_plan(const LdpcCode &code, const Plan &plan);

Plan build_plan(const LdpcCode &code);
Reg2Plan build_reg2_plan(const LdpcCode &code, const Plan &plan, int nt, int kc, int maxd, int nv0, int nv1);
RegPlan build_reg_plan(const LdpcCode &code, const Plan &plan, int nt, int kc, int maxd, uint32_t lds_budget);

}
```

Measured before the change: 24.41 million.

## Balance fused CN/VN work across waves and pack per-wave descriptors for vector prefetch

The fused plan builder now deals check-node calls across waves using a joint cost model that includes each wave's variable-node share, and can split paired calls to cut the heaviest wave's load. A single-wave plan is kept when it is smaller. Per-wave call and VN descriptors are packed into one contiguous row that the kernel fetches as 16-byte scalar loads, prefetched before each barrier instead of reread from separate tables. The rest-call loop now runs for an explicit count rather than stopping at a zero sentinel. The goal is to reduce barrier wait caused by uneven waves and to cut scalar descriptor load latency, at the cost of a more complex planner and extra registers for the prefetched descriptors.

```diff
diff --git a/include/ldpc_amd.h b/include/ldpc_amd.h
--- a/include/ldpc_amd.h
+++ b/include/ldpc_amd.h
@@ -130,6 +130,8 @@
 void ldpc_hip_comm_destroy(ldpc_hip_comm *comm);
 int ldpc_hip_comm_allgather(ldpc_hip_comm *comm, const void *send, void *recv, uint64_t bytes);
 void ldpc_hip_fused_plan_info(const ldpc_hip_ctx *ctx, int64_t info[8]);
+int ldpc_hip_fused_plan_loads(const ldpc_hip_ctx *ctx, int separate, int64_t loads[4][8], int64_t *calls, int max_calls, int64_t *blocks,
+                              int max_blocks);
 int ldpc_hip_decode_stages(const ldpc_hip_ctx *ctx, decoder_param dec, int32_t stages[3]);
 int ldpc_hip_selftest_layer_plan(ldpc_hip_ctx *ctx, int32_t *step_of_row);
 int ldpc_hip_selftest_place(ldpc_hip_comm *comm, uint64_t nct, uint64_t pairs_before, uint64_t frame_pos, uint64_t cap,
diff --git a/libldpc_amd/binding.py b/libldpc_amd/binding.py
--- a/libldpc_amd/binding.py
+++ b/libldpc_amd/binding.py
@@ -96,6 +96,8 @@
     L.ldpc_hip_comm_allgather.argtypes = [vp, vp, vp, u64]
     L.ldpc_hip_fused_plan_info.restype = None
     L.ldpc_hip_fused_plan_info.argtypes = [vp, vp]
+    L.ldpc_hip_fused_plan_loads.restype = i32
+    L.ldpc_hip_fused_plan_loads.argtypes = [vp, i32, vp, vp, i32, vp, i32]
     L.ldpc_hip_decode_stages.restype = i32
     L.ldpc_hip_decode_stages.argtypes = [vp, decoder_param, vp]
     L.ldpc_hip_selftest_layer_plan.restype = i32
@@ -243,6 +245,17 @@
         self.lib.ldpc_hip_fused_plan_info(self.ctx, info)
         return dict(zip(("ok", "n_slots", "vnb", "cnl", "small", "calls_stride", "has_shortened", "table_entries"), [int(v) for v in info]))
 
+    def fused_plan_loads(self, separate=False):
+        loads, calls, blocks = np.zeros((4, 8), np.int64), np.zeros((256, 8), np.int64), np.zeros((64, 4), np.int64)
+        n = self.lib.ldpc_hip_fused_plan_loads(self.ctx, int(bool(separate)), _ptr(loads), _ptr(calls), len(calls), _ptr(blocks), len(blocks))
+        if n < 0:
+            return None
+        names = ("leaf_calls", "rest_calls", "cn_blocks", "vn_blocks", "cn_cost", "vn_cost", "total", "joint")
+        cnames = ("wave", "leaf", "off0", "cnt0", "off1", "cnt1", "cls")
+        return {"waves": [dict(zip(names, map(int, r))) for r in loads],
+                "calls": [dict(zip(cnames, map(int, r))) for r in calls[:n & 0xFFFF]],
+                "blocks": [dict(zip(("wave", "slot", "count", "degree"), map(int, r))) for r in blocks[:n >> 16]]}
+
     STAGES = ("whole", "ratio-first", "ratio-separate", "list-chain", "llr-redo", "handover-first", "handover-resume")
 
     def decode_stages(self, early_term=True, iterations=50, decoding="BP"):
diff --git a/libldpc_amd/csrc/api.cpp b/libldpc_amd/csrc/api.cpp
--- a/libldpc_amd/csrc/api.cpp
+++ b/libldpc_amd/csrc/api.cpp
@@ -618,6 +618,52 @@
     info[5] = f.calls_stride, info[6] = f.has_shortened ? 1 : 0, info[7] = static_cast<int64_t>(f.vn_slot.size());
 }
 
+int ldpc_hip_fused_plan_loads(const ldpc_hip_ctx *ctx, int separate, int64_t loads[4][8], int64_t *calls, int max_calls, int64_t *blocks, int max_blocks)
+{
+    FusedPlan other;
+    const FusedPlan *f = &ctx->eng->fused_plan();
+    if (separate && f->ok)
+    {
+        if (guarded([&] { other = build_fused_plan(ctx->eng->code(), ctx->eng->plan(), false); }) != 0)
+            return -1;
+        f = &other;
+    }
+    if (!f->ok)
+        return -1;
+    int n_calls = 0, n_blocks = 0;
+    for (int w = 0; w < kDecodeWaves; ++w)
+    {
+        const FusedPlan::WaveLoad &l = f->loads[w];
+        const int64_t row[8] = {l.leaf_calls, l.rest_calls, l.cn_blocks, l.vn_blocks, l.cn_cost, l.vn_cost, l.cn_cost + l.vn_cost, f->joint ? 1 : 0};
+        std::copy(row, row + 8, loads[w]);
+        auto put_call = [&](const FusedCall &c, int leaf) {
+            if (calls && n_calls < max_calls)
+            {
+                const int64_t r[8] = {w, leaf, c.offs & 0xFFFFu, c.cnts & 0xFFFFu, c.offs >> 16, c.cnts >> 16, c.cls, 0};
+                std::copy(r, r + 8, calls + 8 * static_cast<size_t>(n_calls));
+            }
+            ++n_calls;
+        };
+        for (int c = 0; c < l.leaf_calls; ++c)
+            put_call(f->leaf_calls[static_cast<size_t>(w) * kFusedLeafCalls + c], 1);
+        for (int c = 0; c < l.rest_calls; ++c)
+            put_call(f->calls[static_cast<size_t>(w) * f->calls_stride + c], 0);
+        for (int sw = 0; sw < kFusedVnSlots; ++sw)
+        {
+            const uint32_t kind = (f->vn_prog[w] >> (4 * sw)) & 0xFu, d0 = f->vn_desc[(static_cast<size_t>(w) * kFusedVnSlots + sw) * 4];
+            if (kind == kFusedVnNone)
+                continue;
+            if (blocks && n_blocks < max_blocks)
+            {
+                const int64_t r[4] = {w, sw, d0 & 0xFFFFu, d0 >> 16};
+                std::copy(r, r + 4, blocks + 4 * static_cast<size_t>(n_blocks));
+            }
+            ++n_blocks;
+        }
+    }
+    return n_calls > max_calls || n_blocks > max_blocks ? -2 : n_calls | (n_blocks << 16);
+}
+
 int ldpc_hip_decode_stages(const ldpc_hip_ctx *ctx, decoder_param dec, int32_t stages[3])
 {
     const StageSeq seq = ctx->eng->stages(to_params(dec));
diff --git a/libldpc_amd/csrc/engine.cpp b/libldpc_amd/csrc/engine.cpp
--- a/libldpc_amd/csrc/engine.cpp
+++ b/libldpc_amd/csrc/engine.cpp
@@ -630,6 +630,8 @@
         dev_fused_.vn_slot = static_cast<const uint32_t *>(up(f.vn_slot.data(), f.vn_slot.size() * 4));
         dev_fused_.lane_tab = static_cast<const uint32_t *>(up(f.lane_tab.data(), f.lane_tab.size() * 4));
         dev_fused_.ho_map = static_cast<const uint32_t *>(up(f.ho_map.data(), f.ho_map.size() * 4));
+        dev_fused_.wave_desc = static_cast<const uint32_t *>(up(f.wave_desc.data(), f.wave_desc.size() * 4));
+        dev_fused_.desc_stride = f.desc_stride;
     }
     if (code_->has_G())
     {
diff --git a/libldpc_amd/csrc/kernels.hpp b/libldpc_amd/csrc/kernels.hpp
--- a/libldpc_amd/csrc/kernels.hpp
+++ b/libldpc_amd/csrc/kernels.hpp
@@ -158,6 +158,8 @@
     const uint32_t *vn_slot;
     const uint32_t *lane_tab;
     const uint32_t *ho_map;
+    const uint32_t *wave_desc;
+    int desc_stride;
 };
 int launch_decode_fused(const DecodeArgs &a, const DevFusedPlan &f, Stage stage, void *stream);
 
diff --git a/libldpc_amd/csrc/kernels_fused.hip b/libldpc_amd/csrc/kernels_fused.hip
--- a/libldpc_amd/csrc/kernels_fused.hip
+++ b/libldpc_amd/csrc/kernels_fused.hip
@@ -43,6 +43,41 @@
 {
     t.hmax = max(max(t.hmax, hi_word(a)), hi_word(b));
     t.hmin = min(min(t.hmin, hi_word(a)), hi_word(b));
+}
+
+typedef uint32_t u32x4 __attribute__((ext_vector_type(4)));
+template <int CNL>
+struct CnDesc
+{
+    u32x4 leaf[CNL], rest0;
+};
+template <int VNB>
+struct VnDesc
+{
+    u32x4 head;
+    u32x4 d0[VNB / 4];
+};
+__device__ __forceinline__ u32x4 fetch4(const_as_ptr<uint32_t> p) { return *(const volatile u32x4 __attribute__((address_space(4))) *)(p); }
+template <int CNL>
+__device__ __forceinline__ CnDesc<CNL> fetch_cn(const_as_ptr<uint32_t> row)
+{
+    CnDesc<CNL> d;
+    if constexpr (CNL > 1)
+        d.leaf[1] = fetch4(row);
+    d.leaf[0] = fetch4(row + 4);
+    d.rest0 = fetch4(row + 8);
+    return d;
+}
+template <int VNB>
+__device__ __forceinline__ VnDesc<VNB> fetch_vn(const_as_ptr<uint32_t> vrow)
+{
+    static_assert(VNB % 4 == 0, "slots in fours");
+    VnDesc<VNB> d;
+    d.head = fetch4(vrow);
+#pragma unroll
+    for (int i = 0; i < VNB / 4; ++i)
+        d.d0[i] = fetch4(vrow + 4 + 4 * i);
+    return d;
 }
 
 template <int D, bool LEAF, unsigned FLIP, bool TWO, bool WANT_TOT, bool SHARED = true>
@@ -508,10 +543,19 @@
         }
         return my_val[w];
     };
+    const auto my_row = uniform_table(F.wave_desc + static_cast<uint32_t>(wave) * static_cast<uint32_t>(F.desc_stride));
+    const uint32_t vn_at = static_cast<uint32_t>(F.desc_stride) - 32u;
+    auto row_now = my_row;
+    auto fence_row = [&] {
+        row_now = my_row;
+        asm volatile("" : "+s"(row_now));
+    };
+    fence_row();
+    CnDesc<CNL> cn = fetch_cn<CNL>(row_now);
+    VnDesc<VNB> vn;
     __syncthreads();
 
-    const auto my_leaf_calls = uniform_table(reinterpret_cast<const uint32_t *>(F.leaf_calls + wave * kFusedLeafCalls));
-    const auto my_calls = uniform_table(reinterpret_cast<const uint32_t *>(F.calls + wave * F.calls_stride));
+    [[maybe_unused]] const auto my_calls = uniform_table(reinterpret_cast<const uint32_t *>(F.calls + wave * F.calls_stride));
     double *out_llr = WANT_LLR ? a.llr_out + frame * nc : nullptr;
     uint32_t leaf_bits = 0;
     uint32_t vn_bits = 0;
@@ -519,21 +563,12 @@
     uint32_t I = 0;
     uint32_t bad = 0, new_leaf_bits = 0, bits = 0;
     [[maybe_unused]] int32_t ho_key = 0;
-    auto leaf_calls_now = my_leaf_calls;
-    auto vdesc_now = my_vdesc;
-    uint32_t prog = vn_prog;
-    auto refresh_tables = [&] {
-        leaf_calls_now = my_leaf_calls;
-        vdesc_now = my_vdesc;
-        prog = vn_prog;
-        asm volatile("" : "+s"(leaf_calls_now), "+s"(vdesc_now), "+s"(prog));
-    };
     auto cn_pass = [&] {
         bad = 0, new_leaf_bits = 0;
 #pragma unroll
         for (int c = 0; c < CNL; ++c)
         {
-            const uint32_t offs = leaf_calls_now[4 * c], cnts = leaf_calls_now[4 * c + 1], cls = leaf_calls_now[4 * c + 2];
+            const uint32_t offs = cn.leaf[c][0], cnts = cn.leaf[c][1], cls = cn.leaf[c][2];
             const uint32_t cnt0 = cnts & 0xFFFFu;
             if (cnt0 == 0)
                 continue;
@@ -568,12 +603,13 @@
             if constexpr (WANT_LLR)
                 leaf_tot[2 * c] = tot0, leaf_tot[2 * c + 1] = tot1;
         }
-        for (int c = 0; c < F.calls_stride; ++c)
-        {
-            const uint32_t offs = my_calls[4 * c], cnts = my_calls[4 * c + 1], cls = my_calls[4 * c + 2];
+        const uint32_t n_rest = cn.leaf[0][3];
+        u32x4 call = cn.rest0;
+        for (uint32_t c = 0; c < n_rest; ++c)
+        {
+            const u32x4 next = fetch4(row_now + 12 + 4 * c);
+            const uint32_t offs = call[0], cnts = call[1], cls = call[2];
             const uint32_t cnt0 = cnts & 0xFFFFu;
-            if (cnt0 == 0)
-                break;
             const bool two = (cnts >> 16) != 0;
             uint32_t lb0, lb1;
             double tot0, tot1;
@@ -605,8 +641,14 @@
             }
 #undef LDPC_CLASS
             bad |= par;
+            call = next;
         }
     };
+    auto prefetch_vn = [&] {
+        fence_row();
+        vn = fetch_vn<VNB>(row_now + vn_at);
+    };
+    auto prefetch_cn = [&] { cn = fetch_cn<CNL>(row_now); };
     auto commit_leaves = [&] {
         leaf_bits = new_leaf_bits;
         if constexpr (WANT_LLR)
@@ -632,7 +674,7 @@
                 out_llr[tab[(24 + w) * kWaveSize] & 0x3FFFFFFFu] = llr;
         };
         auto one = [&](int w, uint32_t kind) {
-            const uint32_t d0 = vdesc_now[4 * w];
+            const uint32_t d0 = vn.d0[w / 4][w % 4];
             const int cnt = static_cast<int>(d0 & 0xFFFFu), deg = static_cast<int>(d0 >> 16);
             if (lane >= cnt)
                 return;
@@ -658,7 +700,7 @@
                     default: sg = 0; break;
                     }
                 else if constexpr (!EXCL)
-                    prod = vn_table(msg, F.vn_slot + vdesc_now[4 * w + 1], lane, cnt, deg, val_at(w), t, sg);
+                    prod = vn_table(msg, F.vn_slot + row_now[vn_at + 16 + w], lane, cnt, deg, val_at(w), t, sg);
                 else
                     sg = 0;
                 note_total(prod);
@@ -669,7 +711,7 @@
 #pragma unroll
         for (int w = 0; w < VNB; w += 2)
         {
-            const uint32_t k01 = (prog >> (4 * w)) & 0xFFu;
+            const uint32_t k01 = (vn.head[0] >> (4 * w)) & 0xFFu;
             if (k01 == (kFusedVnPair | (kFusedVnPair << 4)))
             {
                 uint32_t sga, sgb;
@@ -716,7 +758,6 @@
             }
             if (I == a.iterations)
                 break;
-            refresh_tables();
             if (any & 4)
             {
                 if (tid == 0)
@@ -765,8 +806,8 @@
                     }
                 };
                 for (int c = 0; c < CNL; ++c)
-                    if ((leaf_calls_now[4 * c + 1] & 0xFFFFu) != 0)
-                        ho_call(leaf_calls_now[4 * c], leaf_calls_now[4 * c + 1], leaf_calls_now[4 * c + 2], c);
+                    if ((cn.leaf[c][1] & 0xFFFFu) != 0)
+                        ho_call(cn.leaf[c][0], cn.leaf[c][1], cn.leaf[c][2], c);
                 for (int c = 0; c < F.calls_stride; ++c)
                 {
                     if ((my_calls[4 * c + 1] & 0xFFFFu) == 0)
@@ -777,9 +818,11 @@
             }
             cn_pass();
             commit_leaves();
+            prefetch_vn();
             __syncthreads();
             vn_pass();
             post_vote(I + 1);
+            prefetch_cn();
             __syncthreads();
             ++I;
         }
@@ -787,13 +830,13 @@
     else
     for (;;)
     {
-        refresh_tables();
         cn_pass();
         const int ph = I & 1;
         const bool esc = dm_box_escaped(t.hmax, t.hmin) || t.pmax >= DM_FUSED_P_HI;
         const int wave_vote = (__ballot((bad & 0x80000000u) != 0) != 0) | ((__ballot(esc) != 0) << 1);
         if (lane == 0)
             votes[ph][wave] = wave_vote;
+        prefetch_vn();
         __syncthreads();
         int any = 0;
 #pragma unroll
@@ -818,6 +861,7 @@
         commit_leaves();
 
         vn_pass();
+        prefetch_cn();
         __syncthreads();
         ++I;
     }
@@ -991,7 +1035,6 @@
         stage[n_stage + 1].x = 0.0;
     const uint32_t *tab = F.lane_tab + (static_cast<uint32_t>(wave) * kFusedLaneRows) * kWaveSize + lane;
     const auto my_vdesc = uniform_table(F.vn_desc + wave * kFusedVnSlots * 4);
-    const uint32_t vn_prog = F.vn_prog[wave];
     uint32_t my_idx[VNB], wide_idx[8], vn_entry[VNB], leaf_entry[2 * CNL];
 #pragma unroll
     for (int w = 0; w < VNB; ++w)
@@ -1046,24 +1089,23 @@
                 *at(msg, idx[p * cnt + lane]) = my_L[w];
         }
     }
+    const auto my_row = uniform_table(F.wave_desc + static_cast<uint32_t>(wave) * static_cast<uint32_t>(F.desc_stride));
+    const uint32_t vn_at = static_cast<uint32_t>(F.desc_stride) - 32u;
+    auto row_now = my_row;
+    asm volatile("" : "+s"(row_now));
+    CnDesc<CNL> cn = fetch_cn<CNL>(row_now);
     __syncthreads();
 
-    const auto my_leaf_calls = uniform_table(reinterpret_cast<const uint32_t *>(F.leaf_calls + wave * kFusedLeafCalls));
-    const auto my_calls = uniform_table(reinterpret_cast<const uint32_t *>(F.calls + wave * F.calls_stride));
     double *out_llr = WANT_LLR ? a.llr_out + frame * nc : nullptr;
     uint32_t leaf_bits = 0, vn_bits = 0;
     for (uint32_t I = 0; I < a.iterations; ++I)
     {
         const bool last = I + 1 == a.iterations;
-        auto leaf_calls_now = my_leaf_calls;
-        auto vdesc_now = my_vdesc;
-        uint32_t prog = vn_prog;
-        asm volatile("" : "+s"(leaf_calls_now), "+s"(vdesc_now), "+s"(prog));
         uint32_t lbits = 0;
 #pragma unroll
         for (int c = 0; c < CNL; ++c)
         {
-            const uint32_t offs = leaf_calls_now[4 * c], cnts = leaf_calls_now[4 * c + 1], cls = leaf_calls_now[4 * c + 2];
+            const uint32_t offs = cn.leaf[c][0], cnts = cn.leaf[c][1], cls = cn.leaf[c][2];
             const uint32_t cnt0 = cnts & 0xFFFFu;
             if (cnt0 == 0)
                 continue;
@@ -1096,12 +1138,13 @@
                 }
         }
         leaf_bits = lbits;
-        for (int c = 0; c < F.calls_stride; ++c)
-        {
-            const uint32_t offs = my_calls[4 * c], cnts = my_calls[4 * c + 1], cls = my_calls[4 * c + 2];
+        const uint32_t n_rest = cn.leaf[0][3];
+        u32x4 call = cn.rest0;
+        for (uint32_t c = 0; c < n_rest; ++c)
+        {
+            const u32x4 next = fetch4(row_now + 12 + 4 * c);
+            const uint32_t offs = call[0], cnts = call[1], cls = call[2];
             const uint32_t cnt0 = cnts & 0xFFFFu;
-            if (cnt0 == 0)
-                break;
             const bool two = (cnts >> 16) != 0;
             double d0 = 0.0, d1 = 0.0, d2 = 0.0, d3 = 0.0;
 #define LDPC_MS(D)                                                                                                        \
@@ -1119,7 +1162,11 @@
             default: break;
             }
 #undef LDPC_MS
-        }
+            call = next;
+        }
+        row_now = my_row;
+        asm volatile("" : "+s"(row_now));
+        const VnDesc<VNB> vn = fetch_vn<VNB>(row_now + vn_at);
         __syncthreads();
 
         uint32_t bits = 0;
@@ -1129,7 +1176,7 @@
                     out_llr[tab[(24 + w) * kWaveSize] & 0x3FFFFFFFu] = llr;
         };
         auto one = [&](int w, uint32_t kind) {
-            const uint32_t d0 = vdesc_now[4 * w];
+            const uint32_t d0 = vn.d0[w / 4][w % 4];
             const int cnt = static_cast<int>(d0 & 0xFFFFu), deg = static_cast<int>(d0 >> 16);
             if (lane >= cnt)
                 return;
@@ -1147,14 +1194,14 @@
                 default: break;
                 }
             else
-                out = vnms_table(msg, F.vn_slot + vdesc_now[4 * w + 1], lane, cnt, deg, my_L[w]);
+                out = vnms_table(msg, F.vn_slot + row_now[vn_at + 16 + w], lane, cnt, deg, my_L[w]);
             bits |= (out <= 0 ? 1u : 0u) << w;
             put_llr(w, out);
         };
 #pragma unroll
         for (int w = 0; w < VNB; w += 2)
         {
-            const uint32_t k01 = (prog >> (4 * w)) & 0xFFu;
+            const uint32_t k01 = (vn.head[0] >> (4 * w)) & 0xFFu;
             if (w + 1 < VNB && k01 == (kFusedVnPair | (kFusedVnPair << 4)))
             {
                 double oa, ob;
@@ -1171,6 +1218,7 @@
             }
         }
         vn_bits = bits;
+        cn = fetch_cn<CNL>(row_now);
         __syncthreads();
     }
 
diff --git a/libldpc_amd/csrc/plan.cpp b/libldpc_amd/csrc/plan.cpp
--- a/libldpc_amd/csrc/plan.cpp
+++ b/libldpc_amd/csrc/plan.cpp
@@ -5,6 +5,7 @@
 #include <algorithm>
 #include <cstdio>
 #include <cstdlib>
+#include <cstring>
 #include <map>
 #include <numeric>
 #include <stdexcept>
@@ -444,7 +445,20 @@
     return r;
 }
 
-FusedPlan build_fused_plan(const LdpcCode &code, const Plan &plan)
+namespace fused_cost
+{
+constexpr int kVn2Pair = 27, kVn2One = 17;
+constexpr int vn_wide(int degree) { return 5 + 6 * degree; }
+constexpr int vn_table(int degree) { return 10 + 9 * degree; }
+inline int cn_call(unsigned cls, bool pair)
+{
+    const int d = static_cast<int>(cls & 7u), leaf = static_cast<int>((cls >> 3) & 1u);
+    const int two = d == 2 ? 26 : (d == 3 ? (leaf ? 46 : 54) : (leaf ? 78 : 92));
+    return pair ? two : (two * 6 + 5) / 10;
+}
+}
+
+FusedPlan build_fused_plan(const LdpcCode &code, const Plan &plan, bool joint)
 {
     FusedPlan f;
     const SparseGF2 &H = code.H;
@@ -520,60 +534,6 @@
         calls.push_back(Call{static_cast<int>(b), pair ? static_cast<int>(b + 1) : -1, class_cost(blocks[b].cls) * (pair ? 2 : 1) + 4, leaf});
         b += pair ? 2 : 1;
     }
-    std::vector<std::vector<int>> w_leaf(W), w_rest(W);
-    std::vector<long> load(W, 0);
-    {
-        std::vector<int> order(calls.size());
-        std::iota(order.begin(), order.end(), 0);
-        std::stable_sort(order.begin(), order.end(), [&](int a, int b) { return calls[a].cost > calls[b].cost; });
-        int n_leaf = 0;
-        for (const Call &c : calls)
-            n_leaf += c.leaf;
-        const int leaf_cap = (n_leaf + W - 1) / W;
-        if (leaf_cap > kFusedLeafCalls)
-            return f;
-        for (int ci : order)
-            if (calls[ci].leaf)
-            {
-                int best = -1;
-                for (int w = 0; w < W; ++w)
-                    if (static_cast<int>(w_leaf[w].size()) < leaf_cap && (best < 0 || load[w] < load[best]))
-                        best = w;
-                w_leaf[best].push_back(ci);
-                load[best] += calls[ci].cost;
-            }
-        for (int ci : order)
-            if (!calls[ci].leaf)
-            {
-                const int w = static_cast<int>(std::min_element(load.begin(), load.end()) - load.begin());
-                w_rest[w].push_back(ci);
-                load[w] += calls[ci].cost;
-            }
-        f.cnl = leaf_cap;
-    }
-    auto describe = [&](const Call &c) {
-        const Block &b0 = blocks[c.b0];
-        FusedCall d{b0.off * 8u, static_cast<uint32_t>(b0.rows.size()), b0.cls, 0};
-        if (c.b1 >= 0)
-        {
-            d.offs |= (blocks[c.b1].off * 8u) << 16;
-            d.cnts |= static_cast<uint32_t>(blocks[c.b1].rows.size()) << 16;
-        }
-        return d;
-    };
-    f.leaf_calls.assign(static_cast<size_t>(W) * kFusedLeafCalls, FusedCall{0, 0, 0, 0});
-    f.calls_stride = 1;
-    for (int w = 0; w < W; ++w)
-        f.calls_stride = std::max(f.calls_stride, static_cast<int>(w_rest[w].size()) + 1);
-    f.calls.assign(static_cast<size_t>(W) * f.calls_stride, FusedCall{0, 0, 0, 0});
-    for (int w = 0; w < W; ++w)
-    {
-        for (size_t i = 0; i < w_leaf[w].size(); ++i)
-            f.leaf_calls[static_cast<size_t>(w) * kFusedLeafCalls + i] = describe(calls[w_leaf[w][i]]);
-        for (size_t i = 0; i < w_rest[w].size(); ++i)
-            f.calls[static_cast<size_t>(w) * f.calls_stride + i] = describe(calls[w_rest[w][i]]);
-    }
-
     std::vector<int> cols;
     for (int c = 0; c < H.cols; ++c)
         if (cdeg(c) >= 2)
@@ -689,6 +649,155 @@
                 tab[(24 + sw) * kWaveSize + l] = col_word[vb.cols[l]];
             }
         }
+    }
+    long vn_share[kDecodeWaves];
+    for (int w = 0; w < W; ++w)
+    {
+        vn_share[w] = 0;
+        int n_blocks = 0;
+        for (int sw = 0; sw < kFusedVnSlots; ++sw)
+        {
+            const uint32_t kind = (f.vn_prog[w] >> (4 * sw)) & 0xFu;
+            const int degree = static_cast<int>(f.vn_desc[(static_cast<size_t>(w) * kFusedVnSlots + sw) * 4] >> 16);
+            n_blocks += kind != kFusedVnNone;
+            if (kind == kFusedVnPair && sw % 2 == 0 && sw + 1 < kFusedVnSlots && ((f.vn_prog[w] >> (4 * (sw + 1))) & 0xFu) == kFusedVnPair)
+                vn_share[w] += fused_cost::kVn2Pair, ++n_blocks, ++sw;
+            else if (kind == kFusedVnPair || kind == kFusedVn2)
+                vn_share[w] += fused_cost::kVn2One;
+            else if (kind == kFusedVnWide)
+                vn_share[w] += fused_cost::vn_wide(degree);
+            else if (kind == kFusedVnTable)
+                vn_share[w] += fused_cost::vn_table(degree);
+        }
+        f.loads[w].vn_blocks = n_blocks;
+        f.loads[w].vn_cost = static_cast<int>(vn_share[w]);
+    }
+
+    std::vector<std::vector<int>> w_leaf(W), w_rest(W);
+    {
+        int n_leaf = 0;
+        for (const Call &c : calls)
+            n_leaf += c.leaf;
+        const int leaf_cap = (n_leaf + W - 1) / W;
+        if (leaf_cap > kFusedLeafCalls)
+            return f;
+        f.cnl = leaf_cap;
+        std::vector<int> order(calls.size());
+        std::iota(order.begin(), order.end(), 0);
+        if (!joint)
+        {
+            std::vector<long> load(W, 0);
+            std::stable_sort(order.begin(), order.end(), [&](int a, int b) { return calls[a].cost > calls[b].cost; });
+            for (int ci : order)
+                if (calls[ci].leaf)
+                {
+                    int best = -1;
+                    for (int w = 0; w < W; ++w)
+                        if (static_cast<int>(w_leaf[w].size()) < leaf_cap && (best < 0 || load[w] < load[best]))
+                            best = w;
+                    w_leaf[best].push_back(ci);
+                    load[best] += calls[ci].cost;
+                }
+            for (int ci : order)
+                if (!calls[ci].leaf)
+                {
+                    const int w = static_cast<int>(std::min_element(load.begin(), load.end()) - load.begin());
+                    w_rest[w].push_back(ci);
+                    load[w] += calls[ci].cost;
+                }
+        }
+        else
+        {
+            struct Dealing
+            {
+                std::vector<Call> calls;
+                std::vector<std::vector<int>> w_leaf, w_rest;
+                long heaviest = 0;
+            };
+            auto deal = [&](const std::vector<char> &split) {
+                Dealing d;
+                d.w_leaf.resize(W), d.w_rest.resize(W);
+                for (size_t ci = 0; ci < calls.size(); ++ci)
+                    if (split[ci])
+                        d.calls.push_back(Call{calls[ci].b0, -1, 0, false}), d.calls.push_back(Call{calls[ci].b1, -1, 0, false});
+                    else
+                        d.calls.push_back(calls[ci]);
+                std::vector<long> cn(W, 0);
+                auto measured = [&](int ci) { return fused_cost::cn_call(blocks[d.calls[ci].b0].cls, d.calls[ci].b1 >= 0); };
+                auto lighter = [&](int a, int b) {
+                    const long ta = cn[a] + vn_share[a], tb = cn[b] + vn_share[b];
+                    return ta != tb ? ta < tb : (cn[a] != cn[b] ? cn[a] < cn[b] : a < b);
+                };
+                std::vector<int> by_cost(d.calls.size());
+                std::iota(by_cost.begin(), by_cost.end(), 0);
+                std::stable_sort(by_cost.begin(), by_cost.end(), [&](int a, int b) { return measured(a) > measured(b); });
+                for (int leaf = 1; leaf >= 0; --leaf)
+                    for (int ci : by_cost)
+                        if (d.calls[ci].leaf == (leaf != 0))
+                        {
+                            int best = -1;
+                            for (int w = 0; w < W; ++w)
+                                if ((!leaf || static_cast<int>(d.w_leaf[w].size()) < leaf_cap) && (best < 0 || lighter(w, best)))
+                                    best = w;
+                            (leaf ? d.w_leaf : d.w_rest)[best].push_back(ci);
+                            cn[best] += measured(ci);
+                        }
+                for (int w = 0; w < W; ++w)
+                    d.heaviest = std::max(d.heaviest, cn[w] + vn_share[w]);
+                return d;
+            };
+            std::vector<char> split(calls.size(), 0);
+            Dealing best = deal(split);
+            std::stable_sort(order.begin(), order.end(), [&](int a, int b) { return calls[a].cost < calls[b].cost; });
+            for (int ci : order)
+                if (!calls[ci].leaf && calls[ci].b1 >= 0)
+                {
+                    split[ci] = 1;
+                    if (Dealing d = deal(split); d.heaviest < best.heaviest)
+                        best = std::move(d);
+                    else
+                        split[ci] = 0;
+                }
+            calls = std::move(best.calls), w_leaf = std::move(best.w_leaf), w_rest = std::move(best.w_rest);
+        }
+    }
+    auto describe = [&](const Call &c) {
+        const Block &b0 = blocks[c.b0];
+        FusedCall d{b0.off * 8u, static_cast<uint32_t>(b0.rows.size()), b0.cls, 0};
+        if (c.b1 >= 0)
+        {
+            d.offs |= (blocks[c.b1].off * 8u) << 16;
+            d.cnts |= static_cast<uint32_t>(blocks[c.b1].rows.size()) << 16;
+        }
+        return d;
+    };
+    f.leaf_calls.assign(static_cast<size_t>(W) * kFusedLeafCalls, FusedCall{0, 0, 0, 0});
+    f.calls_stride = 1;
+    for (int w = 0; w < W; ++w)
+        f.calls_stride = std::max(f.calls_stride, static_cast<int>(w_rest[w].size()) + 1);
+    f.calls.assign(static_cast<size_t>(W) * f.calls_stride, FusedCall{0, 0, 0, 0});
+    for (int w = 0; w < W; ++w)
+    {
+        FusedPlan::WaveLoad &ld = f.loads[w];
+        auto count = [&](const Call &c) {
+            ld.cn_blocks += c.b1 >= 0 ? 2 : 1;
+            ld.cn_cost += fused_cost::cn_call(blocks[c.b0].cls, c.b1 >= 0);
+        };
+        for (size_t i = 0; i < w_leaf[w].size(); ++i)
+        {
+            f.leaf_calls[static_cast<size_t>(w) * kFusedLeafCalls + i] = describe(calls[w_leaf[w][i]]);
+            count(calls[w_leaf[w][i]]);
+        }
+        for (size_t i = 0; i < w_rest[w].size(); ++i)
+        {
+            f.calls[static_cast<size_t>(w) * f.calls_stride + i] = describe(calls[w_rest[w][i]]);
+            count(calls[w_rest[w][i]]);
+        }
+        ld.leaf_calls = static_cast<int>(w_leaf[w].size()), ld.rest_calls = static_cast<int>(w_rest[w].size());
+    }
+    for (int w = 0; w < W; ++w)
+    {
+        uint32_t *tab = &f.lane_tab[static_cast<size_t>(w) * kFusedLaneRows * kWaveSize];
         for (size_t c = 0; c < w_leaf[w].size(); ++c)
             for (int h = 0; h < 2; ++h)
             {
@@ -706,6 +815,28 @@
                 }
             }
     }
+    f.desc_stride = kFusedDescStride(f.calls_stride);
+    f.wave_desc.assign(static_cast<size_t>(W) * f.desc_stride, 0);
+    for (int w = 0; w < W; ++w)
+    {
+        uint32_t *row = &f.wave_desc[static_cast<size_t>(w) * f.desc_stride];
+        for (int c = 0; c < kFusedLeafCalls; ++c)
+        {
+            const FusedCall &lc = f.leaf_calls[static_cast<size_t>(w) * kFusedLeafCalls + c];
+            uint32_t *d = row + (c == 0 ? 4 : 0);
+            d[0] = lc.offs, d[1] = lc.cnts, d[2] = lc.cls, d[3] = c == 0 ? static_cast<uint32_t>(w_rest[w].size()) : 0u;
+        }
+        static_assert(sizeof(FusedCall) == 16 && kFusedLeafCalls == 2, "row layout");
+        std::memcpy(row + 8, &f.calls[static_cast<size_t>(w) * f.calls_stride], static_cast<size_t>(f.calls_stride) * sizeof(FusedCall));
+        uint32_t *v = row + kFusedDescVn(f.calls_stride);
+        v[0] = f.vn_prog[w];
+        for (int sw = 0; sw < kFusedVnSlots; ++sw)
+        {
+            v[4 + sw] = f.vn_desc[(static_cast<size_t>(w) * kFusedVnSlots + sw) * 4];
+            v[16 + sw] = f.vn_desc[(static_cast<size_t>(w) * kFusedVnSlots + sw) * 4 + 1];
+        }
+    }
+    f.joint = joint;
     if (f.vn_slot.empty())
         f.vn_slot.push_back(0);
     f.wide_exclusive = true;
@@ -781,4 +912,13 @@
     return L;
 }
 
-}
+FusedPlan build_fused_plan(const LdpcCode &code, const Plan &plan)
+{
+    FusedPlan f = build_fused_plan(code, plan, true);
+    auto small = [](const FusedPlan &p) { return p.ok && p.cnl <= 1 && p.vnb <= 4 && p.wide_exclusive; };
+    if (FusedPlan solo = build_fused_plan(code, plan, false); solo.ok && (!f.ok || (small(solo) && !small(f))))
+        return solo;
+    return f;
+}
+
+}
diff --git a/libldpc_amd/csrc/plan.hpp b/libldpc_amd/csrc/plan.hpp
--- a/libldpc_amd/csrc/plan.hpp
+++ b/libldpc_amd/csrc/plan.hpp
@@ -153,10 +153,22 @@
     std::vector<uint32_t> lane_tab;
     std::vector<uint32_t> edge_slot;
     std::vector<uint32_t> ho_map;
+    std::vector<uint32_t> wave_desc;
+    int desc_stride = 0;
+    struct WaveLoad
+    {
+        int leaf_calls = 0, rest_calls = 0, cn_blocks = 0, vn_blocks = 0;
+        int cn_cost = 0, vn_cost = 0;
+    };
+    WaveLoad loads[kDecodeWaves];
+    bool joint = false;
 };
+constexpr int kFusedDescVn(int calls_stride) { return (8 + 4 * calls_stride + 15) / 16 * 16; }
+constexpr int kFusedDescStride(int calls_stride) { return kFusedDescVn(calls_stride) + 32; }
 constexpr uint32_t kFusedCounted = 0x80000000u, kFusedNone = 0xFFFFFFFFu;
 enum : uint32_t { kFusedVnNone = 0, kFusedVnPair = 1 , kFusedVn2 = 2 , kFusedVnWide = 3 , kFusedVnTable = 4 };
 FusedPlan build_fused_plan(const LdpcCode &code, const Plan &plan);
+FusedPlan build_fused_plan(const LdpcCode &code, const Plan &plan, bool joint);
 
 Plan build_plan(const LdpcCode &code);
 Reg2Plan build_reg2_plan(const LdpcCode &code, const Plan &plan, int nt, int kc, int maxd, int nv0, int nv1);
```

Result: slower. 23.25 million (-4.8%).
